# AdaptiveCity/deepdish

Measured on AMD Instinct MI355X. Metric: end-to-end frames/sec (detect+encode+track) at 640x480, higher is better.
Workload: dtype i8 (reference: uint8); encoder f16; 1 GPU; SSD-MobileNet-v1 uint8-quantised (300x300) + MARS-64x32x3 + deep_sort on synthetic 640x480 BGR frames, ~20 synthetic detections/frame (BASELINE.json configs[1]); streams_per_gpu=3072, worker_threads_per_gpu=2, parallelism=independent streams, 3072 per GPU in 2 worker groups, weights=seeded synthetic (seed 1234)

## Files before the change

### deepdish_amd/_lib.py

```python
import ctypes
import os
from ctypes import c_int, c_int64, c_double, c_float, c_void_p, c_char_p, POINTER

HERE = os.path.dirname(os.path.abspath(__file__))
LIB_PATH = os.environ.get('DD_LIB') or os.path.join(HERE, 'libdeepdish_hip.so')

P = c_void_p


class DeepDishHipError(RuntimeError):
    pass


SIGNATURES = {
    'dd_last_error': [],
    'dd_version': [],
    'dd_ctx_create': [c_int, POINTER(P)],
    'dd_ctx_destroy': [P],
    'dd_ctx_stream': [P, POINTER(P)],
    'dd_ctx_sync': [P],
    'dd_kf_initiate': [P, P, P, P, P, c_int, P],
    'dd_kf_predict': [P, P, P, P, c_int, P],
    'dd_kf_project': [P, P, P, P, c_int, P, P, P],
    'dd_kf_update': [P, P, P, P, P, c_int, P],
    'dd_kf_gate': [P, P, P, P, c_int, P, c_int, c_int, P, P],
    'dd_iou_cost': [P, P, P, c_int, P, c_int, P, P],
    'dd_cosine_nn_cost': [P, P, P, c_int, P, c_int, P, P],
    'dd_euclidean_nn_cost': [P, P, P, c_int, P, c_int, P, P],
    'dd_nms': [P, P, P, c_int, c_double, P, P, P],
    'dd_nms_ssd': [P, P, P, c_int, c_double, P, P, P],
    'dd_lsap_host': [P, c_int, c_int, P, P],
    'dd_pyset_difference_order_host': [P, c_int, P, c_int, P, POINTER(c_int)],
    'dd_tracker_create': [P, c_double, c_double, c_int, c_int, c_int, c_int, c_int, POINTER(P)],
    'dd_tracker_create_metric': [P, c_int, c_double, c_double, c_int, c_int, c_int, c_int, c_int, POINTER(P)],
    'dd_tracker_destroy': [P],
    'dd_tracker_predict': [P],
    'dd_tracker_update': [P, P, P, c_int, c_int],
    'dd_tracker_count': [P, c_int, POINTER(c_int)],
    'dd_tracker_read': [P, c_int, P, P, P],
    'dd_tracker_track_update': [P, c_int64, P, P, c_int],
    'dd_tracker_track_predict': [P, c_int64],
    'dd_tracker_track_set': [P, c_int64, c_int, c_int],
    'dd_tracker_remove': [P, P, c_int],
    'dd_tracker_next_id': [P, POINTER(c_int64)],
    'dd_tracker_last_cost': [P, P, P, c_int, POINTER(c_int), POINTER(c_int)],
    'dd_tracker_last_matches': [P, P, c_int, POINTER(c_int)],
    'dd_crop_resize': [P, P, c_int, c_int, P, c_int, c_int, c_int, P, P, P],
    'dd_crop_resize_f64': [P, P, c_int, c_int, P, c_int, c_int, c_int, P, P, P],
    'dd_fake_encode': [P, P, c_int, c_int, P, P],
    'dd_resize_lanczos': [P, P, c_int, c_int, c_int, c_int, P, c_int, c_int, P],
    'dd_resize_lanczos_batch': [P, P, c_int, c_int, c_int, c_int, c_int, P, c_int, c_int, P],
    'dd_resize_bilinear': [P, P, c_int, c_int, c_int, P, c_int, c_int, P],
    'dd_ingest_create': [P, c_int, c_int, c_int, c_int, c_int, c_int, c_int, P],
    'dd_ingest_destroy': [P],
    'dd_ingest_host_slot': [P, c_int, P, P],
    'dd_ingest_submit': [P, c_int],
    'dd_ingest_wait_uploaded': [P, c_int],
    'dd_ingest_acquire': [P, c_int, P, P],
    'dd_ingest_release': [P, c_int, P],
    'dd_mog2_create': [P, c_int, c_int, c_int, c_int, c_double, c_int, POINTER(P)],
    'dd_mog2_destroy': [P],
    'dd_mog2_state': [P, c_int, P, P, P, P],
    'dd_mog2_apply': [P, P, c_double, P, P, P],
    'dd_mask_box_count': [P, P, c_int, c_int, c_int, P, P, c_int, P, P],
    'dd_net_create': [P, P, c_int, P, c_int64, c_int, POINTER(P)],
    'dd_net_create_shared': [P, P, c_int, P, c_int64, c_int, POINTER(P)],
    'dd_net_activation_bytes': [P, POINTER(c_int64)],
    'dd_net_destroy': [P],
    'dd_net_forward': [P, P, c_int, P],
    'dd_net_output': [P, c_int, POINTER(P), POINTER(c_int), POINTER(c_int), POINTER(c_int), POINTER(c_int),
                      POINTER(c_int)],
    'dd_net_use_graph': [P, c_int],
    'dd_net_input_size': [P, POINTER(c_int), POINTER(c_int)],
    'dd_net_max_batch': [P, POINTER(c_int)],
    'dd_net_last_batch': [P, POINTER(c_int)],
    'dd_net_read': [P, c_int, c_int, P, c_int, P],
    'dd_net_profile': [P, c_int],
    'dd_net_profile_read': [P, P, c_int, POINTER(c_int)],
    'dd_net_op_launches': [P, P, c_int, POINTER(c_int)],
    'dd_ssd_postprocess': [P, P, P, c_int, c_int, c_int, c_float, c_float, P, P, P, P, P],
    'dd_ssd_decode': [P, P, P, c_int, c_int, c_float, P, P, P, P, c_int, P],
    'dd_ssd_postprocess_decoded': [P, P, P, P, P, c_int, c_int, c_float, c_float, P, P, P, P, c_int, P],
    'dd_ssd_regular_nms_decoded': [P, P, P, c_int, c_int, c_int, c_int, c_int, c_int, c_float, c_float, P, P, P, P, c_int, P],
    'dd_ssd_postprocess_regular': [P, P, P, c_int, c_int, c_int, c_int, c_float, c_float, P, P, P, P, c_int, P],
    'dd_ssd_postprocess_regular_u8': [P, P, P, c_int, P, P, P, c_int, c_int, c_int, c_int, c_float, c_float, P, P, P, P, c_int, P],
    'dd_net_ssd_heads_u8': [P, POINTER(P), POINTER(P), POINTER(c_int), POINTER(P), P, POINTER(c_int), POINTER(c_int)],
    'dd_net_ssd_decode': [P, P, c_int, c_float, c_int],
    'dd_net_ssd_decoded': [P, POINTER(P), POINTER(P), POINTER(P), POINTER(P)],
    'dd_net_ssd_decoded_read': [P, c_int, P, P, P, P],
    'dd_net_yolo_decode': [P, c_int],
    'dd_net_yolo_decoded': [P, P, P, P, P],
    'dd_net_yolo_decoded_read': [P, c_int, P, P, P],
    'dd_ssd_detections': [P, P, P, P, c_int, c_int, c_double, c_double, c_double, c_double, P, P, P, P, P],
    'dd_yolov5_decode': [P, P, c_int, c_int, c_float, c_float, c_float, P, P, P, c_int, P, P],
    'dd_pipeline_create': [P, c_int, c_int, c_int, P, P, c_int, c_int, P, c_char_p, c_char_p, c_double, c_double,
                           c_double, c_int, c_int, P, c_int, c_int, POINTER(P)],
    'dd_pipeline_destroy': [P],
    'dd_pipeline_detector_adaptor': [P, c_int],
    'dd_pipeline_ssd_options': [P, c_int, c_float, c_float],
    'dd_pipeline_ssd_regular_nms': [P, c_int],
    'dd_pipeline_detector_skip_frames': [P, c_int],
    'dd_pipeline_metric': [P, c_int],
    'dd_pipeline_step': [P, P, P, P, P, P],
    'dd_pipeline_step2': [P, P, P, P, P, P, P],
    'dd_pipeline_background_subtraction': [P, c_double, c_int],
    'dd_pipeline_motion_mask': [P, P, c_int, POINTER(ctypes.c_longlong)],
    'dd_pipeline_counts': [P, P],
    'dd_pipeline_tracker': [P, c_int, POINTER(P)],
    'dd_pipeline_stage_seconds': [P, P, POINTER(ctypes.c_longlong)],
    'dd_pipeline_stage_gpu_ms': [P, P, POINTER(ctypes.c_longlong)],
    'dd_pipeline_detector_stream': [P, POINTER(P)],
    'dd_pipeline_detections': [P, c_int, P, P, P, c_int, POINTER(c_int)],
    'dd_counts_accumulate': [P, P, P, c_int, P],
}
_RESTYPE = {'dd_last_error': c_char_p}

_lib = None
MISSING = []


def lib():
    global _lib
    if _lib is not None:
        return _lib
    if not os.path.exists(LIB_PATH):
        raise DeepDishHipError(
            'libdeepdish_hip.so is missing (%s): build it with `python -m deepdish_amd.build`; '
            'there is no CPU fallback' % LIB_PATH)
    try:
        import torch
    except ImportError:
        pass
    l = ctypes.CDLL(LIB_PATH)
    for name, args in SIGNATURES.items():
        try:
            fn = getattr(l, name)
        except AttributeError:
            MISSING.append(name)
            continue
        fn.argtypes = args
        fn.restype = _RESTYPE.get(name, c_int)
    _lib = l
    return l


def check(rc, what=''):
    if rc != 0:
        msg = lib().dd_last_error()
        raise DeepDishHipError('%s failed (%d): %s' % (what or 'libdeepdish_hip call', rc,
                                                      msg.decode() if msg else '?'))
```

### deepdish_amd/csrc/mars_pair.hip

```cpp
#include "mars_tail.h"

namespace {

typedef _Float16 h8 __attribute__((ext_vector_type(8)));
typedef float f4 __attribute__((ext_vector_type(4)));
typedef unsigned u4 __attribute__((ext_vector_type(4)));

__device__ __forceinline__ float elu(float v) {
    float e = __builtin_amdgcn_exp2f(v * 1.44269504088896340736f);
    e = __builtin_amdgcn_fmed3f(e, 0.f, 1.f);
    return __builtin_amdgcn_fmed3f(v, e - 1.f, 3.0e38f);
}

__device__ __forceinline__ void lds_fill16(const _Float16 *g, char *lds_wave_base) {
#if defined(__HIP_DEVICE_COMPILE__)
    __builtin_amdgcn_global_load_lds(g, lds_wave_base, 16, 0, 0);
#endif
}

__device__ __forceinline__ int frag_row(int a, int fr) { return (fr >> 2) * 8 + (a & 1) * 4 + (fr & 3); }

constexpr int PZ_B = 3072;
constexpr int PT64_B = 18 * 1024;
constexpr int PT32_B = 33 * 1024;
constexpr int PPLAIN_B = 16 * 1024;
constexpr int PRAW_B = 8 * 1024;
constexpr int pair_off_in(bool) { return PZ_B; }
constexpr int pair_off_h(bool first) { return PZ_B + 2 * (first ? PT32_B : PT64_B); }
constexpr int pair_off_res(bool first) { return pair_off_h(first) + 2 * PT64_B; }
constexpr int pair_off_raw(bool first) { return pair_off_res(first) + (first ? 2 : 3) * PPLAIN_B; }
constexpr int pair_off_const(bool first) { return pair_off_raw(first) + (first ? 2 * PRAW_B : 0); }
constexpr int pair_lds_bytes(bool first) { return pair_off_const(first) + 5 * 64 * 4; }

template <bool FIRST>
__global__ __launch_bounds__(512, 2) void mars_pair64_k(const MarsPairP P) {
    constexpr int OFF_IN = pair_off_in(FIRST), OFF_H = pair_off_h(FIRST), OFF_RES = pair_off_res(FIRST), OFF_RAW = pair_off_raw(FIRST),
                  OFF_C = pair_off_const(FIRST);
    constexpr int TIN_B = FIRST ? PT32_B : PT64_B, NRES = FIRST ? 2 : 3;
    extern __shared__ __attribute__((aligned(16))) char smem[];
    const int tid = threadIdx.x, lane = tid & 63;
    const int wave = __builtin_amdgcn_readfirstlane(tid >> 6);
    const int stage = wave >> 2, half = wave & 1, q = (wave >> 1) & 1;
    const int fr = lane & 15, fq = lane >> 4, j = fr >> 3, x = fr & 7;

    for (int i = tid * 16; i < OFF_C; i += 512 * 16) *reinterpret_cast<u4 *>(smem + i) = u4{0u, 0u, 0u, 0u};
    float *cst = reinterpret_cast<float *>(smem + OFF_C);
    if (tid < 64) {
        cst[tid] = P.bias_a[tid];
        cst[64 + tid] = P.bias_b[tid];
        cst[128 + tid] = P.aff2[tid];
        cst[192 + tid] = P.aff2[P.cout_pad + tid];
        cst[256 + tid] = (FIRST && P.bias_p) ? P.bias_p[tid] : 0.f;
    }
    __syncthreads();

    h8 wf[9][2][2];
    h8 wp[2];
    const bool a32 = FIRST && stage == 0;
    {
        const _Float16 *w = stage == 0 ? P.wa : P.wb;
        const int kpad = stage == 0 ? P.kpad_a : P.kpad_b;
#pragma unroll
        for (int t = 0; t < 9; ++t)
#pragma unroll
            for (int ks = 0; ks < 2; ++ks)
#pragma unroll
                for (int a = 0; a < 2; ++a) {
                    const size_t row = (size_t)(half * 32 + frag_row(a, fr)) * kpad;
                    wf[t][ks][a] = a32 ? *reinterpret_cast<const h8 *>(w + row + t * 32 + fq * 8)
                                       : *reinterpret_cast<const h8 *>(w + row + t * 64 + ks * 32 + fq * 8);
                }
#pragma unroll
        for (int a = 0; a < 2; ++a)
            wp[a] = FIRST ? *reinterpret_cast<const h8 *>(P.wp + (size_t)(half * 32 + frag_row(a, fr)) * P.kpad_p + fq * 8) : wf[0][0][a];
    }
#if defined(__HIP_DEVICE_COMPILE__)
#pragma unroll
    for (int t = 0; t < 9; ++t)
#pragma unroll
        for (int ks = 0; ks < 2; ++ks)
#pragma unroll
            for (int a = 0; a < 2; ++a) asm volatile("" ::"v"(wf[t][ks][a]));
    asm volatile("" ::"v"(wp[0]), "v"(wp[1]));
#endif

    const int n0 = blockIdx.x, nstep = gridDim.x;
    const int Kc = (P.n_img - n0 + nstep - 1) / nstep;

    const _Float16 *src[5];
    size_t stp[5];
    int n_dma;
    if constexpr (FIRST) {
        const int par = lane >> 5, pl = (lane >> 3) & 3, col = 2 * (lane & 7) + par;
#pragma unroll
        for (int h = 0; h < 4; ++h) {
            const int r = wave + 8 * h < 31 ? wave + 8 * h : 30;
            src[h] = col < 15 ? P.in + ((size_t)n0 * 31 + r) * 15 * P.cs_in + (size_t)col * P.cs_in + P.coff_in + pl * 8 : P.zero;
            stp[h] = col < 15 ? (size_t)nstep * 31 * 15 * P.cs_in : 0;
        }
        const int jr = lane >> 5, xx = lane & 7;
        src[4] = P.in2 + ((size_t)n0 * 31 + 2 * (2 * wave + jr)) * 15 * P.cs_in2 + (size_t)(2 * xx) * P.cs_in2 + P.coff_in2 + pl * 8;
        stp[4] = (size_t)nstep * 31 * 15 * P.cs_in2;
        n_dma = 5;
    } else {
        const int pl = lane >> 3, xx = lane & 7;
#pragma unroll
        for (int h = 0; h < 2; ++h) {
            src[h] = P.in + (((size_t)n0 * 16 + wave + 8 * h) * 8 + xx) * P.cs_in + P.coff_in + pl * 8;
            stp[h] = (size_t)nstep * 128 * P.cs_in;
            src[2 + h] = P.res + (((size_t)n0 * 16 + wave + 8 * h) * 8 + xx) * P.cs_res + P.coff_res + pl * 8;
            stp[2 + h] = (size_t)nstep * 128 * P.cs_res;
        }
        src[4] = P.zero; stp[4] = 0;
        n_dma = 4;
    }
    (void)n_dma;
    int dq = 0;
    auto issue = [&]() {
        char *T = smem + OFF_IN + (dq & 1) * TIN_B;
        if constexpr (FIRST) {
#pragma unroll
            for (int h = 0; h < 4; ++h) lds_fill16(src[h], T + ((wave + 8 * h < 31 ? wave + 8 * h : 30) + 1) * 1024);
            lds_fill16(src[4], smem + OFF_RAW + (dq & 1) * PRAW_B + wave * 1024);
        } else {
#pragma unroll
            for (int h = 0; h < 2; ++h) lds_fill16(src[h], T + (wave + 8 * h + 1) * 1024);
            const int rs = dq % 3;
#pragma unroll
            for (int h = 0; h < 2; ++h) lds_fill16(src[2 + h], smem + OFF_RES + rs * PPLAIN_B + (wave + 8 * h) * 1024);
        }
        ++dq;
        const bool more = dq < Kc;
#pragma unroll
        for (int h = 0; h < 5; ++h) src[h] += more ? stp[h] : 0;
    };

    const int co = half * 32 + fq * 8;
    const unsigned lo64 = (unsigned)((j * 64 + fq * 8 + x) * 16);
    const unsigned lo32 = (unsigned)((2 * j * 64 + fq * 8 + x) * 16);
    const f4 ba0 = *reinterpret_cast<const f4 *>(cst + (stage ? 64 : 0) + co), ba1 = *reinterpret_cast<const f4 *>(cst + (stage ? 64 : 0) + co + 4);

    issue();
    for (int c = 0; c <= Kc; ++c) {
#if defined(__HIP_DEVICE_COMPILE__)
        if (stage == 0 || c < 2) asm volatile("s_waitcnt vmcnt(0) lgkmcnt(0)" ::: "memory");
        else asm volatile("s_waitcnt vmcnt(8) lgkmcnt(0)" ::: "memory");
        __builtin_amdgcn_s_barrier();
        asm volatile("" ::: "memory");
#endif
        issue();
        const int cc = stage == 0 ? c : c - 1;
        if (cc < 0 || cc >= Kc) continue;
        const size_t n = (size_t)(n0 + cc * nstep);
#pragma unroll 1
        for (int f = 0; f < 4; ++f) {
            const int F = 4 * q + f;
            f4 acc[2] = {f4{0.f, 0.f, 0.f, 0.f}, f4{0.f, 0.f, 0.f, 0.f}};
            h8 X[4];
            if (a32) {
                const unsigned tb = (unsigned)(OFF_IN + (cc & 1) * PT32_B + 4 * F * 1024) + lo32;
                const unsigned bL = x == 0 ? ((tb + 512u - 16u) & 255u) : tb + 512u - 16u, bC = tb, bR = tb + 512u;
                const unsigned pb = (unsigned)(OFF_RAW + (cc & 1) * PRAW_B) + (unsigned)(((2 * F + j) * 32 + fq * 8 + x) * 16);
                f4 accp[2] = {f4{0.f, 0.f, 0.f, 0.f}, f4{0.f, 0.f, 0.f, 0.f}};
#if defined(__HIP_DEVICE_COMPILE__)
#define DD_RD(u_) do { if constexpr ((u_) < 9) { constexpr int dy_ = (u_) / 3, dx_ = (u_) - dy_ * 3;                                               \
                           asm volatile("ds_read_b128 %0, %1 offset:%2" : "=&v"(X[(u_) & 3]) : "v"(dx_ == 0 ? bL : dx_ == 1 ? bC : bR), "n"(dy_ * 1024) : "memory"); } \
                       else asm volatile("ds_read_b128 %0, %1" : "=&v"(X[(u_) & 3]) : "v"(pb) : "memory"); } while (0)
#define DD_UNIT(u_) do { if constexpr ((u_) + 3 < 10) DD_RD(((u_) + 3) % 10);                                                                      \
                         asm volatile("s_waitcnt lgkmcnt(%1)" : "+v"(X[(u_) & 3]) : "n"((u_) + 3 < 10 ? 3 : 9 - (u_)));                           \
                         if constexpr ((u_) < 9) { _Pragma("unroll") for (int a = 0; a < 2; ++a) acc[a] = __builtin_amdgcn_mfma_f32_16x16x32_f16(wf[(u_) % 9][0][a], X[(u_) & 3], acc[a], 0, 0, 0); } \
                         else { _Pragma("unroll") for (int a = 0; a < 2; ++a) accp[a] = __builtin_amdgcn_mfma_f32_16x16x32_f16(wp[a], X[(u_) & 3], accp[a], 0, 0, 0); } } while (0)
                DD_RD(0); DD_RD(1); DD_RD(2);
                DD_UNIT(0); DD_UNIT(1); DD_UNIT(2); DD_UNIT(3); DD_UNIT(4); DD_UNIT(5); DD_UNIT(6); DD_UNIT(7); DD_UNIT(8); DD_UNIT(9);
#undef DD_UNIT
#undef DD_RD
#endif
                const f4 c0 = *reinterpret_cast<const f4 *>(cst + 256 + co), c1 = *reinterpret_cast<const f4 *>(cst + 256 + co + 4);
                h8 sk;
#pragma unroll
                for (int i = 0; i < 4; ++i) { sk[i] = (_Float16)(accp[0][i] + c0[i]); sk[4 + i] = (_Float16)(accp[1][i] + c1[i]); }
                *reinterpret_cast<h8 *>(smem + OFF_RES + (cc & 1) * PPLAIN_B + ((2 * F + j) * 64 + (half * 4 + fq) * 8 + x) * 16) = sk;
            } else {
                const unsigned tb = (unsigned)((stage == 0 ? OFF_IN + (cc & 1) * PT64_B : OFF_H + (cc & 1) * PT64_B) + 2 * F * 1024) + lo64;
                const unsigned bL = x == 0 ? ((tb - 16u) & 255u) : tb - 16u, bC = tb, bR = x == 7 ? ((tb + 16u) & 255u) : tb + 16u;
#if defined(__HIP_DEVICE_COMPILE__)
#define DD_RD(u_) do { constexpr int t_ = (u_) >> 1, ks_ = (u_) & 1, dy_ = t_ / 3, dx_ = t_ - dy_ * 3;                                             \
                       asm volatile("ds_read_b128 %0, %1 offset:%2" : "=&v"(X[(u_) & 3]) : "v"(dx_ == 0 ? bL : dx_ == 1 ? bC : bR), "n"(dy_ * 1024 + ks_ * 512) : "memory"); } while (0)
#define DD_UNIT(u_) do { if constexpr ((u_) + 3 < 18) DD_RD(((u_) + 3) % 18);                                                                      \
                         asm volatile("s_waitcnt lgkmcnt(%1)" : "+v"(X[(u_) & 3]) : "n"((u_) + 3 < 18 ? 3 : 17 - (u_)));                          \
                         _Pragma("unroll") for (int a = 0; a < 2; ++a) acc[a] = __builtin_amdgcn_mfma_f32_16x16x32_f16(wf[(u_) >> 1][(u_) & 1][a], X[(u_) & 3], acc[a], 0, 0, 0); } while (0)
                DD_RD(0); DD_RD(1); DD_RD(2);
                DD_UNIT(0); DD_UNIT(1); DD_UNIT(2); DD_UNIT(3); DD_UNIT(4); DD_UNIT(5); DD_UNIT(6); DD_UNIT(7); DD_UNIT(8);
                DD_UNIT(9); DD_UNIT(10); DD_UNIT(11); DD_UNIT(12); DD_UNIT(13); DD_UNIT(14); DD_UNIT(15); DD_UNIT(16); DD_UNIT(17);
#undef DD_UNIT
#undef DD_RD
#endif
            }
            float v[8];
#pragma unroll
            for (int i = 0; i < 4; ++i) { v[i] = acc[0][i] + ba0[i]; v[4 + i] = acc[1][i] + ba1[i]; }
            if (stage == 0) {
                h8 o;
#pragma unroll
                for (int i = 0; i < 8; ++i) o[i] = (_Float16)elu(v[i]);
                *reinterpret_cast<h8 *>(smem + OFF_H + (cc & 1) * PT64_B + ((2 * F + j + 1) * 64 + (half * 4 + fq) * 8 + x) * 16) = o;
            } else {
                const int rs = FIRST ? (cc & 1) : cc % 3;
                const h8 rv = *reinterpret_cast<const h8 *>(smem + OFF_RES + rs * PPLAIN_B + ((2 * F + j) * 64 + (half * 4 + fq) * 8 + x) * 16);
#pragma unroll
                for (int i = 0; i < 8; ++i) v[i] += (float)rv[i];
                const size_t m = (n * 16 + 2 * F + j) * 8 + x;
                h8 o;
#pragma unroll
                for (int i = 0; i < 8; ++i) o[i] = (_Float16)v[i];
                *reinterpret_cast<h8 *>(P.out + m * P.cs_out + P.coff_out + co) = o;
                const f4 s0 = *reinterpret_cast<const f4 *>(cst + 128 + co), s1 = *reinterpret_cast<const f4 *>(cst + 128 + co + 4);
                const f4 t0 = *reinterpret_cast<const f4 *>(cst + 192 + co), t1 = *reinterpret_cast<const f4 *>(cst + 192 + co + 4);
                h8 o2;
#pragma unroll
                for (int i = 0; i < 4; ++i) { o2[i] = (_Float16)elu(s0[i] * v[i] + t0[i]); o2[4 + i] = (_Float16)elu(s1[i] * v[4 + i] + t1[i]); }
                *reinterpret_cast<h8 *>(P.out2 + m * P.cs_out2 + P.coff_out2 + co) = o2;
            }
        }
    }
#if defined(__HIP_DEVICE_COMPILE__)
    asm volatile("s_waitcnt vmcnt(0)" ::: "memory");
#endif
}

template <bool FIRST>
int launch_pair(hipStream_t s, int device, const MarsPairP &P) {
    constexpr int lds = pair_lds_bytes(FIRST);
    static_assert(lds <= 160 * 1024, "LDS budget");
    static DevOnce once;
    const int rc = once.run(device, [&]() -> int {
        DD_HIP(hipFuncSetAttribute(reinterpret_cast<const void *>(&mars_pair64_k<FIRST>), hipFuncAttributeMaxDynamicSharedMemorySize, lds));
        return DD_OK;
    });
    if (rc != DD_OK) return rc;
    const int n_cu = dd_cu_count(device);
    const int grid = P.n_img < n_cu ? P.n_img : n_cu;
    hipLaunchKernelGGL((mars_pair64_k<FIRST>), dim3(grid), dim3(512), lds, s, P);
    DD_LAUNCH_CHECK();
    return DD_OK;
}

}

int mars_pair64_launch(hipStream_t s, int device, const MarsPairP &P, bool first) {
    DD_REQUIRE(P.n_img > 0 && P.in && P.wa && P.wb && P.bias_a && P.bias_b && P.out && P.out2 && P.aff2 && P.zero && (first ? (P.in2 && P.wp) : P.res != nullptr), DD_E_ARG,
               "mars_pair64: bad argument");
    return first ? launch_pair<true>(s, device, P) : launch_pair<false>(s, device, P);
}
```

### deepdish_amd/csrc/mars_tail.h

```cpp
#pragma once
#include "common.h"

struct MarsWsP {
    const _Float16 *in;  int cs_in, coff_in;
    const _Float16 *in2; int cs_in2, coff_in2;
    const _Float16 *w;   int kpad;
    const _Float16 *w2;  int kpad2;
    const float *bias, *bias2;
    const _Float16 *res; int cs_res, coff_res;
    _Float16 *out;  int cs_out, coff_out;
    _Float16 *out2; int cs_out2, coff_out2;
    const float *aff2; int cout_pad;
    const _Float16 *zero;
    int n_img;
};

enum { MARS_WS_S1 = 0, MARS_WS_S1_RES = 1, MARS_WS_S2_PROJ = 2 };

int mars_ws128_launch(hipStream_t s, int device, const MarsWsP &P, int mode, int act, bool out2);

struct MarsPairP {
    const _Float16 *in;  int cs_in, coff_in;
    const _Float16 *in2; int cs_in2, coff_in2;
    const _Float16 *wa;  int kpad_a; const float *bias_a;
    const _Float16 *wp;  int kpad_p; const float *bias_p;
    const _Float16 *wb;  int kpad_b; const float *bias_b;
    const _Float16 *res; int cs_res, coff_res;
    _Float16 *out;  int cs_out, coff_out;
    _Float16 *out2; int cs_out2, coff_out2;
    const float *aff2; int cout_pad;
    const _Float16 *zero;
    int n_img;
};
int mars_pair64_launch(hipStream_t s, int device, const MarsPairP &P, bool first);
```

### deepdish_amd/csrc/mars_tail.hip

```cpp
#include "mars_tail.h"
#include <vector>

namespace {

typedef _Float16 h8 __attribute__((ext_vector_type(8)));
typedef float f4 __attribute__((ext_vector_type(4)));
typedef unsigned u4 __attribute__((ext_vector_type(4)));

enum { ACT_NONE = 0, ACT_ELU = 2 };

__device__ __forceinline__ float elu(float v) {
    float e = __builtin_amdgcn_exp2f(v * 1.44269504088896340736f);
    e = __builtin_amdgcn_fmed3f(e, 0.f, 1.f);
    return __builtin_amdgcn_fmed3f(v, e - 1.f, 3.0e38f);
}

__device__ __forceinline__ void lds_fill16(const _Float16 *g, char *lds_wave_base) {
#if defined(__HIP_DEVICE_COMPILE__)
    __builtin_amdgcn_global_load_lds(g, lds_wave_base, 16, 0, 0);
#endif
}

__device__ __forceinline__ int frag_row(int a, int fr) { return (fr >> 2) * 8 + (a & 1) * 4 + (fr & 3); }

// ... 1 lines not shown
__device__ unsigned long long dd_mars_stamps[256 * 8 * 8];
#define DD_STAMP(k) do { const unsigned long long t_ = __builtin_amdgcn_s_memtime(); st_acc[k] += t_ - st_last; st_last = t_; } while (0)
#else
#define DD_STAMP(k) do { } while (0)
#endif

constexpr int WS_LEAD = 2, WS_NB = WS_LEAD + 2, WS_NBR = WS_LEAD + 3;
constexpr int ws_tile_bytes(int mode) { return mode == MARS_WS_S2_PROJ ? 17 * 68 * 16 : 10 * 72 * 16; }
constexpr int ws_zero_bytes(int mode) { return mode == MARS_WS_S2_PROJ ? 0 : 7680; }
constexpr int WS_RES_BYTES = 8 * 72 * 16, WS_PRJ_BYTES = 4096;
constexpr int ws_xw_bytes(int mode) { return mode == MARS_WS_S2_PROJ ? 4096 : 2048; }
constexpr int ws_off_tiles(int mode) { return ws_zero_bytes(mode); }
constexpr int ws_off_aux(int mode) { return ws_off_tiles(mode) + WS_NB * ws_tile_bytes(mode); }
constexpr int ws_off_xchg(int mode) {
    return ws_off_aux(mode) + (mode == MARS_WS_S1_RES ? WS_NBR * WS_RES_BYTES : mode == MARS_WS_S2_PROJ ? WS_NB * WS_PRJ_BYTES : 0);
}
constexpr int ws_off_const(int mode) { return ws_off_xchg(mode) + 2 * 8 * ws_xw_bytes(mode); }
constexpr int ws_lds_bytes(int mode) { return ws_off_const(mode) + 3 * 128 * 4; }

template <int MODE, int ACT, bool OUT2>
__global__ __launch_bounds__(512, 2) void mars_ws128_k(const MarsWsP P) {
    constexpr bool S2 = MODE == MARS_WS_S2_PROJ, RES = MODE == MARS_WS_S1_RES;
    constexpr int LEAD = WS_LEAD, NB = WS_NB, NBR = WS_NBR;
    constexpr int TILE_B = ws_tile_bytes(MODE), XW_B = ws_xw_bytes(MODE);
    constexpr int OFF_T = ws_off_tiles(MODE), OFF_A = ws_off_aux(MODE), OFF_X = ws_off_xchg(MODE), OFF_C = ws_off_const(MODE);
    constexpr int KS = S2 ? 1 : 2, CIN = S2 ? 64 : 128;
    [[maybe_unused]] constexpr int N_DMA = S2 ? 3 : RES ? 2 : 1;
    [[maybe_unused]] constexpr int N_ST = S2 ? 2 : (RES && OUT2) ? 2 : 1;
    extern __shared__ __attribute__((aligned(16))) char smem[];
    const int tid = threadIdx.x, lane = tid & 63;
    const int wave = __builtin_amdgcn_readfirstlane(tid >> 6);
    const int cg = wave & 3, kh = wave >> 2;
    const int fr = lane & 15, fq = lane >> 4, yy = fr >> 2, x = fr & 3;

    for (int i = tid * 16; i < OFF_A; i += 512 * 16) *reinterpret_cast<u4 *>(smem + i) = u4{0u, 0u, 0u, 0u};
    float *cst = reinterpret_cast<float *>(smem + OFF_C);
    if (tid < 128) {
        cst[tid] = P.bias[tid];
        if constexpr (S2) cst[128 + tid] = P.bias2 ? P.bias2[tid] : 0.f;
        if constexpr (RES && OUT2) { cst[128 + tid] = P.aff2[tid]; cst[256 + tid] = P.aff2[P.cout_pad + tid]; }
    }
    __syncthreads();

    h8 wf[9][KS][2];
#pragma unroll
    for (int t = 0; t < 9; ++t)
#pragma unroll
        for (int ks = 0; ks < KS; ++ks)
#pragma unroll
            for (int a = 0; a < 2; ++a)
                wf[t][ks][a] = *reinterpret_cast<const h8 *>(P.w + (size_t)(cg * 32 + frag_row(a, fr)) * P.kpad + t * CIN + kh * (CIN / 2) + ks * 32 + fq * 8);
    h8 wp[2];
    if constexpr (S2) {
#pragma unroll
        for (int a = 0; a < 2; ++a) wp[a] = *reinterpret_cast<const h8 *>(P.w2 + (size_t)(cg * 32 + frag_row(a, fr)) * P.kpad2 + kh * 32 + fq * 8);
    }

#if defined(__HIP_DEVICE_COMPILE__)
#pragma unroll
    for (int t = 0; t < 9; ++t)
#pragma unroll
        for (int ks = 0; ks < KS; ++ks)
#pragma unroll
            for (int a = 0; a < 2; ++a) asm volatile("" ::"v"(wf[t][ks][a]));
    if constexpr (S2) asm volatile("" ::"v"(wp[0]), "v"(wp[1]));
#endif

    const int n0 = blockIdx.x, nstep = gridDim.x;
    const int Kc = (P.n_img - n0 + nstep - 1) / nstep;

    int dq = 0, dq_slot = 0, dq_rslot = 0;
    const _Float16 *src_a, *src_b, *src_c;
    size_t step_a, step_b, step_c;
    if constexpr (!S2) {
        src_a = P.in + (size_t)n0 * 32 * P.cs_in + ((wave * 4 + (lane & 3)) * P.cs_in + P.coff_in + (lane >> 2) * 8);
        src_b = RES ? P.res + (size_t)n0 * 32 * P.cs_res + ((wave * 4 + (lane & 3)) * P.cs_res + P.coff_res + (lane >> 2) * 8) : P.zero;
        src_c = P.zero;
        step_a = (size_t)nstep * 32 * P.cs_in; step_b = (size_t)nstep * 32 * P.cs_res; step_c = 0;
    } else {
        const int par = lane >> 5, pl = (lane >> 2) & 7, col = 2 * (lane & 3) + par;
        src_a = P.in + (size_t)n0 * 128 * P.cs_in + ((wave * 8 + col) * P.cs_in + P.coff_in + pl * 8);
        src_b = src_a + (size_t)64 * P.cs_in;
        const int ch = (wave & 3) * 64 + lane;
        src_c = P.in2 + (size_t)n0 * 128 * P.cs_in2 + ((2 * ((ch >> 2) & 7) * 8 + 2 * (ch & 3)) * P.cs_in2 + P.coff_in2 + (ch >> 5) * 8);
        step_a = step_b = (size_t)nstep * 128 * P.cs_in; step_c = (size_t)nstep * 128 * P.cs_in2;
    }
    auto issue = [&]() {
        char *T = smem + OFF_T + dq_slot * TILE_B;
        if constexpr (!S2) {
            lds_fill16(src_a, T + (wave + 1) * 72 * 16);
            if constexpr (RES) lds_fill16(src_b, smem + OFF_A + dq_rslot * WS_RES_BYTES + wave * 72 * 16);
        } else {
            lds_fill16(src_a, T + wave * 68 * 16);
            lds_fill16(src_b, T + (wave + 8) * 68 * 16);
            lds_fill16(src_c, smem + OFF_A + dq_slot * WS_PRJ_BYTES + (wave & 3) * 1024);
        }
        ++dq;
        const bool more = dq < Kc;
        src_a += more ? step_a : 0;
        if constexpr (RES || S2) src_b += more ? step_b : 0;
        if constexpr (S2) src_c += more ? step_c : 0;
        dq_slot = dq_slot + 1 == NB ? 0 : dq_slot + 1;
        dq_rslot = dq_rslot + 1 == NBR ? 0 : dq_rslot + 1;
    };

    const unsigned lo = S2 ? (unsigned)((2 * yy * 68 + (kh * 4 + fq) * 4 + x) * 16) : (unsigned)((yy * 72 + (kh * 8 + fq) * 4 + x) * 16);
    const unsigned lo_prj = (unsigned)(((kh * 4 + fq) * 32 + yy * 4 + x) * 16);
    const unsigned lo_res = (unsigned)(((4 * kh + yy) * 72 + (cg * 4 + fq) * 4 + x) * 16);
    const int co = cg * 32 + fq * 8;
    const f4 b0 = *reinterpret_cast<const f4 *>(cst + co), b1 = *reinterpret_cast<const f4 *>(cst + co + 4);

    f4 keep[S2 ? 4 : 2];
    int slot = 0, rslot_prev = 0, rslot = 0;

    auto epilogue = [&](int cprev) {
        const char *Xp = smem + OFF_X + ((cprev & 1) * 8 + (wave ^ 4)) * XW_B + lane * 16;
        const size_t n = (size_t)(n0 + cprev * nstep);
        const size_t m = (n * 8 + 4 * kh + yy) * 4 + x;
        float v[8];
        {
            const f4 o0 = *reinterpret_cast<const f4 *>(Xp), o1 = *reinterpret_cast<const f4 *>(Xp + 1024);
#pragma unroll
            for (int i = 0; i < 4; ++i) { v[i] = keep[0][i] + o0[i] + b0[i]; v[4 + i] = keep[1][i] + o1[i] + b1[i]; }
        }
        if constexpr (ACT == ACT_ELU) {
#pragma unroll
            for (int i = 0; i < 8; ++i) v[i] = elu(v[i]);
        }
        if constexpr (RES) {
            const h8 rv = *reinterpret_cast<const h8 *>(smem + OFF_A + rslot_prev * WS_RES_BYTES + lo_res);
#pragma unroll
            for (int i = 0; i < 8; ++i) v[i] += (float)rv[i];
        }
        h8 o;
#pragma unroll
        for (int i = 0; i < 8; ++i) o[i] = (_Float16)v[i];
        *reinterpret_cast<h8 *>(P.out + m * P.cs_out + P.coff_out + co) = o;
        if constexpr (RES && OUT2) {
            const f4 s0 = *reinterpret_cast<const f4 *>(cst + 128 + co), s1 = *reinterpret_cast<const f4 *>(cst + 128 + co + 4);
            const f4 t0 = *reinterpret_cast<const f4 *>(cst + 256 + co), t1 = *reinterpret_cast<const f4 *>(cst + 256 + co + 4);
            h8 o2;
#pragma unroll
            for (int i = 0; i < 4; ++i) { o2[i] = (_Float16)elu(s0[i] * v[i] + t0[i]); o2[4 + i] = (_Float16)elu(s1[i] * v[4 + i] + t1[i]); }
            *reinterpret_cast<h8 *>(P.out2 + m * P.cs_out2 + P.coff_out2 + co) = o2;
        }
        if constexpr (S2) {
            const f4 o0 = *reinterpret_cast<const f4 *>(Xp + 2048), o1 = *reinterpret_cast<const f4 *>(Xp + 3072);
            const f4 c0 = *reinterpret_cast<const f4 *>(cst + 128 + co), c1 = *reinterpret_cast<const f4 *>(cst + 128 + co + 4);
            h8 o2;
#pragma unroll
            for (int i = 0; i < 4; ++i) { o2[i] = (_Float16)(keep[2][i] + o0[i] + c0[i]); o2[4 + i] = (_Float16)(keep[3][i] + o1[i] + c1[i]); }
            *reinterpret_cast<h8 *>(P.out2 + m * P.cs_out2 + P.coff_out2 + co) = o2;
        }
    };

#ifdef DD_MARS_STAMPS
    unsigned long long st_acc[8] = {0, 0, 0, 0, 0, 0, 0, 0}, st_last = __builtin_amdgcn_s_memtime();
    const unsigned long long st_begin = st_last;
#endif
    static_assert(LEAD == 2, "the counted waits below are written for two crops of look-ahead");
    for (int ci = 0; ci < LEAD; ++ci) issue();
    DD_STAMP(0);
    for (int c = 0; c <= Kc; ++c) {
#if defined(__HIP_DEVICE_COMPILE__)
        if (kh == 0 || c == 0) {
            if (c <= 1) asm volatile("s_waitcnt vmcnt(%0) lgkmcnt(0)" ::"i"(N_DMA) : "memory");
            else if (c == 2) asm volatile("s_waitcnt vmcnt(%0) lgkmcnt(0)" ::"i"(N_DMA + N_ST) : "memory");
            else asm volatile("s_waitcnt vmcnt(%0) lgkmcnt(0)" ::"i"(N_DMA + 2 * N_ST) : "memory");
// ... 66 lines not shown
#endif
            DD_STAMP(3);
            issue();
            DD_STAMP(1);
            if (c > 0) epilogue(c - 1);
            DD_STAMP(4);
#pragma unroll
            for (int i = 0; i < (S2 ? 4 : 2); ++i) keep[i] = kn[i];
        } else {
            issue();
            DD_STAMP(1);
            if (c > 0) epilogue(c - 1);
            DD_STAMP(4);
#if defined(__HIP_DEVICE_COMPILE__)
            if (c == 0) asm volatile("s_waitcnt vmcnt(%0) lgkmcnt(0)" ::"i"(N_DMA) : "memory");
            else if (c == 1) asm volatile("s_waitcnt vmcnt(%0) lgkmcnt(0)" ::"i"(N_DMA + N_ST) : "memory");
            else asm volatile("s_waitcnt vmcnt(%0) lgkmcnt(0)" ::"i"(N_DMA + 2 * N_ST) : "memory");
            __builtin_amdgcn_s_barrier();
            asm volatile("" ::: "memory");
#endif
            DD_STAMP(3);
            if (c < Kc) compute(keep);
            DD_STAMP(5);
        }
        slot = slot + 1 == NB ? 0 : slot + 1;
        rslot_prev = rslot;
        rslot = rslot + 1 == NBR ? 0 : rslot + 1;
    }
#if defined(__HIP_DEVICE_COMPILE__)
    asm volatile("s_waitcnt vmcnt(0)" ::: "memory");
#endif
#ifdef DD_MARS_STAMPS
    if (lane == 0) {
        unsigned long long *d = dd_mars_stamps + ((size_t)blockIdx.x * 8 + wave) * 8;
        for (int k = 0; k < 6; ++k) d[k] = st_acc[k];
        d[6] = __builtin_amdgcn_s_memtime() - st_begin;
        d[7] = (unsigned long long)Kc;
    }
#endif
}

template <int MODE, int ACT, bool OUT2>
int launch_one(hipStream_t s, int device, const MarsWsP &P) {
    constexpr int lds = ws_lds_bytes(MODE);
    static_assert(lds <= 160 * 1024, "LDS budget");
    static DevOnce once;
    const int rc = once.run(device, [&]() -> int {
        DD_HIP(hipFuncSetAttribute(reinterpret_cast<const void *>(&mars_ws128_k<MODE, ACT, OUT2>), hipFuncAttributeMaxDynamicSharedMemorySize, lds));
        return DD_OK;
    });
    if (rc != DD_OK) return rc;
    const int n_cu = dd_cu_count(device);
    const int grid = P.n_img < n_cu ? P.n_img : n_cu;
    hipLaunchKernelGGL((mars_ws128_k<MODE, ACT, OUT2>), dim3(grid), dim3(512), lds, s, P);
    DD_LAUNCH_CHECK();
#ifdef DD_MARS_STAMPS
    {
        static std::vector<unsigned long long> h(256 * 8 * 8);
        DD_HIP(hipStreamSynchronize(s));
        DD_HIP(hipMemcpyFromSymbol(h.data(), HIP_SYMBOL(dd_mars_stamps), h.size() * 8));
        for (int half = 0; half < 2; ++half) {
            double a[7] = {0, 0, 0, 0, 0, 0, 0};
            int nw = 0;
            for (int b = 0; b < grid; ++b)
                for (int w = half * 4; w < half * 4 + 4; ++w, ++nw) {
                    const unsigned long long *d = h.data() + ((size_t)b * 8 + w) * 8;
                    for (int k = 0; k < 7; ++k) a[k] += (double)d[k] / (double)(k == 0 || k == 6 ? 1 : d[7] + 1);
                }
            fprintf(stderr, "mars_ws128_k<%d,%d,%d> K half %d: prologue DMAs %.0f | per step: issue %.0f, wait %.0f, barrier %.0f, epilogue %.0f, compute %.0f | loop total %.0f cycles, %d steps\n",
                    MODE, ACT, (int)OUT2, half, a[0] / nw, a[1] / nw, a[2] / nw, a[3] / nw, a[4] / nw, a[5] / nw, a[6] / nw, (int)h[7] + 1);
        }
    }
#endif
    return DD_OK;
}

}

int mars_ws128_launch(hipStream_t s, int device, const MarsWsP &P, int mode, int act, bool out2) {
    DD_REQUIRE(P.n_img > 0 && P.in && P.w && P.bias && P.out && P.zero, DD_E_ARG, "mars_ws128: bad argument");
    DD_REQUIRE((long long)P.n_img * 128 * (P.cs_in > P.cs_out ? P.cs_in : P.cs_out) < (1ll << 40), DD_E_CAPACITY, "mars_ws128: batch of %d", P.n_img);
    if (mode == MARS_WS_S2_PROJ) {
        DD_REQUIRE(P.in2 && P.w2 && P.out2 && act == ACT_ELU, DD_E_ARG, "mars_ws128: stride-2 form needs the projection operands and ELU");
        return launch_one<MARS_WS_S2_PROJ, ACT_ELU, false>(s, device, P);
    }
    if (mode == MARS_WS_S1) {
        DD_REQUIRE(!P.res && !P.out2, DD_E_ARG, "mars_ws128: plain form with a residual or a second output");
        return act == ACT_ELU ? launch_one<MARS_WS_S1, ACT_ELU, false>(s, device, P) : launch_one<MARS_WS_S1, ACT_NONE, false>(s, device, P);
    }
    DD_REQUIRE(mode == MARS_WS_S1_RES && P.res && act == ACT_NONE && (!out2 || (P.out2 && P.aff2)), DD_E_ARG, "mars_ws128: residual form");
    return out2 ? launch_one<MARS_WS_S1_RES, ACT_NONE, true>(s, device, P) : launch_one<MARS_WS_S1_RES, ACT_NONE, false>(s, device, P);
}
```

### deepdish_amd/csrc/net_priv.h

```cpp
#pragma once
#include <map>
#include <utility>
#include <vector>
#include "common.h"

struct TensorDesc { int buf, h, w, c, cs, coff, dtype, pad; };

struct dd_net {
    dd_ctx *ctx = nullptr;
    int max_batch = 0;
    std::vector<int32_t> prog;
    std::vector<TensorDesc> tensors;
    std::vector<int64_t> buf_elems;
    std::vector<void *> bufs;
    std::vector<int> buf_dtype;
    int n_ops = 0, ops_off = 0;
    void *arena = nullptr;
    int64_t arena_bytes = 0;
    char *d_weights = nullptr;
    int64_t weight_bytes = 0;
    int in_h = 0, in_w = 0, out_tensor = -1;
    bool profile = false;
    int last_batch = 0;
    DevBuf slab;
    bool ssd_dec = false, yolo_dec = false;
    int dec_anchors = 0; float dec_thr = 0.f;
    float *d_anchors = nullptr, *dec_boxes = nullptr, *dec_score = nullptr, *dec_keys = nullptr; int *dec_cls = nullptr;
    bool slab_moved = false;
    _Float16 *d_zero = nullptr;
    bool use_glds = true;
    bool use_rw = true;
    int tile_mode = 0;
    std::vector<hipEvent_t> events;
    std::vector<int32_t> op_launch;
    struct GraphEntry { int calls = 0; hipGraph_t graph = nullptr; hipGraphExec_t exec = nullptr; };
    bool use_graph = false;
    std::map<std::pair<const void *, int>, GraphEntry> graphs;
};

int netq_run_op(dd_net *net, int op_index, const int32_t *o, const uint8_t *input, int nimg, hipStream_t s, int *handled);
int netq_run_front(dd_net *net, const int32_t *o0, const int32_t *o1, const int32_t *o2, const uint8_t *input, int nimg, hipStream_t s, int *ran);
int netq_run_mid(dd_net *net, const int32_t *o3, const int32_t *o4, int nimg, hipStream_t s, int *ran);
int netq_prepare(dd_net *net);
```

### deepdish_amd/csrc/nets.hip

```cpp
#include <algorithm>
#include <cmath>
#include <cstdlib>
#include <map>
#include <string>
#include "common.h"
#include "ssd_dev.h"
#include "net_priv.h"
#include "mars_tail.h"

namespace {

typedef _Float16 h8 __attribute__((ext_vector_type(8)));
typedef _Float16 h4 __attribute__((ext_vector_type(4)));
typedef float f4 __attribute__((ext_vector_type(4)));

enum { OP_INPUT = 1, OP_CONV = 2, OP_DWCONV = 3, OP_MAXPOOL = 4, OP_UPSAMPLE = 5, OP_FC = 6, OP_L2NORM = 7, OP_STEM = 8, OP_DWPW = 9 };
enum { ACT_NONE = 0, ACT_RELU6 = 1, ACT_ELU = 2, ACT_SILU = 3, ACT_RELU = 4, ACT_SIGMOID = 5 };
enum { EPI_F16 = 0, EPI_F32 = 1, EPI_SSD_HEAD = 2, EPI_YOLO = 3 };
enum { OPK_DEFAULT = 0, OPK_FOLDED = 1, OPK_POOL_ROWS = 2, OPK_POOL_ROWS_STEM = 3, OPK_RES_UNIT = 4, OPK_SSD_FRONT = 5, OPK_C64_ROWS = 6, OPK_S2_ROWS = 7, OPK_CONV_WS = 8, OPK_WS_DW = 9, OPK_DWPW_ROWS = 10, OPK_SSD_HEAD_DEC = 11, OPK_RES_PAIR = 12, OPK_YOLO_HEAD_DEC = 13, OPK_MARS_WS = 14, OPK_FOLDED_PREV = 15, OPK_MARS_PAIR = 16, OPK_C64_STRIPS = 18, OPK_Q_FRONT = 19, OPK_Q_MID = 20, OPK_STEM_WIDE = 23 };
enum { DT_F16 = 0, DT_F32 = 1, DT_U8 = 2 };

constexpr int OP_WORDS = 48;
constexpr int TENSOR_WORDS = 8;

// ... 83 lines not shown
        const int n = m / hw, p = m - n * hw;
        const int A = P.p[5];
        float *dst = static_cast<float *>(P.out) + ((size_t)n * P.p[1] + P.p[2] + (size_t)p * A) * P.p[3];
#pragma unroll
        for (int r = 0; r < 4; ++r)
            if (co + r < P.cout) dst[co + r] = v[r];
        return;
    }
    if (P.res) {
        const h4 rv = *reinterpret_cast<const h4 *>(P.res + (size_t)m * P.cs_res + P.coff_res + co);
#pragma unroll
        for (int r = 0; r < 4; ++r) v[r] += (float)rv[r];
    }
    if (P.epi == EPI_F32) {
        if (P.post_aff) {
            const f4 sc = *reinterpret_cast<const f4 *>(P.aff2 + co);
            const f4 sh = *reinterpret_cast<const f4 *>(P.aff2 + P.cout_pad + co);
#pragma unroll
            for (int r = 0; r < 4; ++r) v[r] = sc[r] * v[r] + sh[r];
        }
#pragma unroll
        for (int r = 0; r < 4; ++r)
            if (co + r >= P.cout) v[r] = 0.f;
        *reinterpret_cast<f4 *>(static_cast<float *>(P.out) + (size_t)m * P.cs_out + P.coff_out + co) = f4{v[0], v[1], v[2], v[3]};
        return;
    }
#pragma unroll
    for (int r = 0; r < 4; ++r)
        if (co + r >= P.cout) v[r] = 0.f;
    {
        h4 o;
#pragma unroll
        for (int r = 0; r < 4; ++r) o[r] = (_Float16)v[r];
        *reinterpret_cast<h4 *>(static_cast<_Float16 *>(P.out) + (size_t)m * P.cs_out + P.coff_out + co) = o;
    }
    if (P.out2) {
        const f4 sc = *reinterpret_cast<const f4 *>(P.aff2 + co);
        const f4 sh = *reinterpret_cast<const f4 *>(P.aff2 + P.cout_pad + co);
        h4 o;
#pragma unroll
        for (int r = 0; r < 4; ++r) {
            const float t = co + r < P.cout ? apply_act(sc[r] * v[r] + sh[r], ACT_ELU) : 0.f;
            o[r] = (_Float16)t;
        }
        *reinterpret_cast<h4 *>(P.out2 + (size_t)m * P.cs_out2 + P.coff_out2 + co) = o;
    }
}

typedef unsigned u4v_t __attribute__((ext_vector_type(4)));
template <int HI>
__device__ __forceinline__ float fma_mix_f16(unsigned x, unsigned w, float acc) {
#if defined(__HIP_DEVICE_COMPILE__)
    if (HI) asm("v_fma_mix_f32 %0, %1, %2, %0 op_sel:[1,1,0] op_sel_hi:[1,1,0]" : "+v"(acc) : "v"(x), "v"(w));
    else asm("v_fma_mix_f32 %0, %1, %2, %0 op_sel:[0,0,0] op_sel_hi:[1,1,0]" : "+v"(acc) : "v"(x), "v"(w));
#endif
    return acc;
}
__device__ __forceinline__ void dw_tap(float (&acc)[8], const h8 &x, const h8 &w) {
    const u4v_t xv = __builtin_bit_cast(u4v_t, x), wv = __builtin_bit_cast(u4v_t, w);
#pragma unroll
    for (int i = 0; i < 8; ++i)
        acc[i] = (i & 1) ? fma_mix_f16<1>(xv[i >> 1], wv[i >> 1], acc[i]) : fma_mix_f16<0>(xv[i >> 1], wv[i >> 1], acc[i]);
}

struct Epi8 { f4 b0, b1, s0, s1, t0, t1; };

__device__ __forceinline__ Epi8 epi8_load(const ConvP &P, int co) {
    Epi8 E;
    E.b0 = *reinterpret_cast<const f4 *>(P.bias + co);
    E.b1 = *reinterpret_cast<const f4 *>(P.bias + co + 4);
    E.s0 = E.s1 = E.t0 = E.t1 = f4{0.f, 0.f, 0.f, 0.f};
    if (P.out2) {
        E.s0 = *reinterpret_cast<const f4 *>(P.aff2 + co);
        E.s1 = *reinterpret_cast<const f4 *>(P.aff2 + co + 4);
        E.t0 = *reinterpret_cast<const f4 *>(P.aff2 + P.cout_pad + co);
        E.t1 = *reinterpret_cast<const f4 *>(P.aff2 + P.cout_pad + co + 4);
    }
    return E;
}

#ifndef DD_EPI_NT
#define DD_EPI_NT true
#endif
template <int ACT = -1, bool BIAS = true, int EF = -1, bool NT = DD_EPI_NT, bool TAIL = true>
__device__ __forceinline__ void conv_epilogue_f16x8(const ConvP &P, const Epi8 &E, int m, int co, float v[8], const h8 *res_pre = nullptr) {
    const int act = ACT < 0 ? P.act : ACT;
    const bool has_res = EF < 0 ? P.res != nullptr : EF >= 1, has_out2 = EF < 0 ? P.out2 != nullptr : EF == 1;
#pragma unroll
    for (int r = 0; r < 4; ++r) {
        v[r] = apply_act(BIAS ? v[r] + E.b0[r] : v[r], act);
        v[4 + r] = apply_act(BIAS ? v[4 + r] + E.b1[r] : v[4 + r], act);
    }
    if (has_res) {
        const h8 rv = res_pre ? *res_pre : *reinterpret_cast<const h8 *>(P.res + (size_t)m * P.cs_res + P.coff_res + co);
#pragma unroll
        for (int r = 0; r < 8; ++r) v[r] += (float)rv[r];
    }
    const bool tail = TAIL && co + 8 > P.cout;
    h8 o;
#pragma unroll
    for (int r = 0; r < 8; ++r) o[r] = (_Float16)v[r];
    if (tail) {
#pragma unroll
        for (int r = 0; r < 8; ++r)
            if (co + r >= P.cout) o[r] = (_Float16)0.f;
    }
    h8 *dst = reinterpret_cast<h8 *>(static_cast<_Float16 *>(P.out) + (size_t)m * P.cs_out + P.coff_out + co);
    if constexpr (NT) __builtin_nontemporal_store(o, dst);
    else *dst = o;
    if (has_out2) {
        h8 o2;
#pragma unroll
        for (int r = 0; r < 8; ++r) {
            const float sc = r < 4 ? E.s0[r] : E.s1[r - 4], sh = r < 4 ? E.t0[r] : E.t1[r - 4];
            o2[r] = (_Float16)apply_act(sc * v[r] + sh, ACT_ELU);
        }
        if (tail) {
#pragma unroll
            for (int r = 0; r < 8; ++r)
                if (co + r >= P.cout) o2[r] = (_Float16)0.f;
        }
        *reinterpret_cast<h8 *>(P.out2 + (size_t)m * P.cs_out2 + P.coff_out2 + co) = o2;
    }
}

template <int ACT = -1>
__device__ __forceinline__ void conv_epilogue_f16x8(const ConvP &P, int m, int co, float v[8]) {
    const Epi8 E = epi8_load(P, co);
    conv_epilogue_f16x8<ACT>(P, E, m, co, v);
}

template <int ACT, int BM, int BN, int T>
__device__ __forceinline__ void conv_finish_rows(const ConvP &P, const float *ot, int m0, int n0) {
    constexpr int OROW = BN + 4, G = BN / 8;
    static_assert(T % G == 0, "a thread keeps its channel group over the row loop");
    const int g = threadIdx.x % G, co = n0 + g * 8;
    if (co >= P.cout_pad) return;
    const Epi8 E = epi8_load(P, co);
    for (int pl = threadIdx.x / G; pl < BM; pl += T / G) {
        const int m = m0 + pl;
        if (m >= P.m) break;
        const f4 lo = *reinterpret_cast<const f4 *>(ot + pl * OROW + g * 8);
        const f4 hi = *reinterpret_cast<const f4 *>(ot + pl * OROW + g * 8 + 4);
        float v[8] = {lo[0], lo[1], lo[2], lo[3], hi[0], hi[1], hi[2], hi[3]};
        conv_epilogue_f16x8<ACT>(P, E, m, co, v);
    }
}

template <int WM, int WN, int MI, int NI>
__device__ __forceinline__ void conv_finish(const ConvP &P, f4 (&acc)[NI][MI], _Float16 *lds, int m0, int n0, int hw) {
    constexpr int T = WM * WN * 64;
    constexpr int BM = WM * MI * 16, BN = WN * NI * 16;
    const int tid = threadIdx.x, lane = tid & 63, wave = tid >> 6;
    const int wm = wave / WN, wn = wave % WN;
    const int fr = lane & 15, fq = lane >> 4;
    if (P.epi == EPI_F16 && P.splitk == 1) {
        constexpr int OROW = BN + 4;
        float *ot = reinterpret_cast<float *>(lds);
#pragma unroll
        for (int b = 0; b < MI; ++b)
#pragma unroll
            for (int a = 0; a < NI; ++a)
                *reinterpret_cast<f4 *>(ot + ((wm * MI + b) * 16 + fr) * OROW + (wn * NI + a) * 16 + fq * 4) = acc[a][b];
        __syncthreads();
        switch (P.act) {
            case ACT_NONE: conv_finish_rows<ACT_NONE, BM, BN, T>(P, ot, m0, n0); break;
            case ACT_RELU6: conv_finish_rows<ACT_RELU6, BM, BN, T>(P, ot, m0, n0); break;
            case ACT_ELU: conv_finish_rows<ACT_ELU, BM, BN, T>(P, ot, m0, n0); break;
            case ACT_SILU: conv_finish_rows<ACT_SILU, BM, BN, T>(P, ot, m0, n0); break;
            default: conv_finish_rows<-1, BM, BN, T>(P, ot, m0, n0);
        }
        return;
    }
    if (P.epi == EPI_SSD_HEAD && P.splitk == 1) {
        constexpr int OROW = BN + 4;
        float *ot = reinterpret_cast<float *>(lds);
#pragma unroll
        for (int b = 0; b < MI; ++b)
#pragma unroll
            for (int a = 0; a < NI; ++a)
                *reinterpret_cast<f4 *>(ot + ((wm * MI + b) * 16 + fr) * OROW + (wn * NI + a) * 16 + fq * 4) = acc[a][b];
        __syncthreads();
        const int A = P.p[5];
        typedef float f4u __attribute__((ext_vector_type(4), aligned(4)));
        constexpr int LPP = BN / 4, PPW = 64 / LPP;
        const int lc = (lane % LPP) * 4, lp = lane / LPP;
        const int ch = n0 + lc;
        const int nlive = min(4, max(0, P.cout - ch));
        f4 bias = f4{0.f, 0.f, 0.f, 0.f};
        for (int q = 0; q < nlive; ++q) bias[q] = P.bias[ch + q];
        for (int pl = wave * PPW + lp; pl < BM; pl += WM * WN * PPW) {
            const int m = m0 + pl;
// ... 1183 lines not shown
            fill_pre(2 * r + 3); fill_pre(2 * r + 4);
            if constexpr (RAW_SEP) { fill_raw(2 * r + 1); fill_raw(2 * r + 2); }
            auto conv2 = [&](const _Float16 *ringp, int slot0, int mask, const h8 (&w)[9][2], f4 (&acc)[2][2]) {
                h8 X[2][3];
                auto rd = [&](int i, h8 (&x)[3]) {
                    const _Float16 *rs = ringp + ((slot0 + i) & mask) * RU_SLOT + offC;
                    x[0] = *reinterpret_cast<const h8 *>(rs - 8);
                    x[1] = *reinterpret_cast<const h8 *>(rs);
                    x[2] = *reinterpret_cast<const h8 *>(rs + 8);
                };
                rd(0, X[0]);
#pragma unroll
                for (int i = 0; i < 4; ++i) {
                    h8 (&x)[3] = X[i & 1];
#if defined(__HIP_DEVICE_COMPILE__)
                    asm volatile("" : "+v"(x[0]), "+v"(x[1]), "+v"(x[2]));
                    __builtin_amdgcn_sched_barrier(0);
#endif
                    if (i + 1 < 4) rd(i + 1, X[(i + 1) & 1]);
#if defined(__HIP_DEVICE_COMPILE__)
                    __builtin_amdgcn_sched_barrier(0);
#endif
#pragma unroll
                    for (int dx = 0; dx < 3; ++dx)
#pragma unroll
                        for (int cr = 0; cr < 2; ++cr) {
                            const int dy = i - cr;
                            if (dy < 0 || dy > 2) continue;
#pragma unroll
                            for (int a = 0; a < 2; ++a)
                                acc[cr][a] = __builtin_amdgcn_mfma_f32_16x16x32_f16(w[dy * 3 + dx][a], x[dx], acc[cr][a], 0, 0, 0);
                        }
#if defined(__HIP_DEVICE_COMPILE__)
                    __builtin_amdgcn_sched_barrier(0);
#endif
                }
            };
            {
                f4 acc[2][2] = {{bA0, bA1}, {bA0, bA1}};
                conv2(pre, 2 * r, RU_PRE_SLOTS - 1, wA, acc);
#pragma unroll
                for (int cr = 0; cr < 2; ++cr) {
                    const int y = 2 * r + cr;
                    const bool live = y < H && fr < W;
                    h8 o;
#pragma unroll
                    for (int q = 0; q < 4; ++q) {
                        o[q] = (_Float16)apply_act(acc[cr][0][q], actA);
                        o[4 + q] = (_Float16)apply_act(acc[cr][1][q], actA);
                    }
                    u4v_t ou = __builtin_bit_cast(u4v_t, o);
                    ou &= live ? 0xFFFFFFFFu : 0u;
                    *reinterpret_cast<u4v_t *>(h1 + (y & (RU_H1_SLOTS - 1)) * RU_SLOT + offC) = ou;
                }
            }
            {
                f4 acc[2][2] = {{EB.b0, EB.b1}, {EB.b0, EB.b1}};
                conv2(h1, 2 * r - 2, RU_H1_SLOTS - 1, wB, acc);
                h8 rv0 = RAW_SEP ? *reinterpret_cast<const h8 *>(rawr + ((2 * r - 1) & (RU_RAW_SLOTS - 1)) * RU_SLOT + offC)
                                 : *reinterpret_cast<const h8 *>(pre + ((2 * r) & (RU_PRE_SLOTS - 1)) * RU_SLOT + offC);
#if defined(__HIP_DEVICE_COMPILE__)
                asm volatile("s_waitcnt vmcnt(0)" ::: "memory");
#endif
#pragma unroll
                for (int cr = 0; cr < 2; ++cr) {
                    const int y = 2 * r - 1 + cr;
                    if (cr == 1) rv0 = RAW_SEP ? *reinterpret_cast<const h8 *>(rawr + (y & (RU_RAW_SLOTS - 1)) * RU_SLOT + offC)
                                               : *reinterpret_cast<const h8 *>(pre + ((y + 1) & (RU_PRE_SLOTS - 1)) * RU_SLOT + offC);
                    if ((unsigned)y >= (unsigned)H || fr >= W) continue;
                    float o[8];
#pragma unroll
                    for (int q = 0; q < 4; ++q) { o[q] = acc[cr][0][q]; o[4 + q] = acc[cr][1][q]; }
                    conv_epilogue_f16x8<ACT_NONE, false, 1, true, false>(PB, EB, (n * H + y) * W + fr, fq * 8, o, &rv0);
                }
            }
        }
    }
}

constexpr int RP_X_SLOTS = 8;
constexpr int rp_pair_halves() { return 6 * 8 + (RU_PRE_SLOTS + 2 * RU_H1_SLOTS + 2 * RP_X_SLOTS) * RU_SLOT; }

template <int ACT_A>
__global__ __launch_bounds__(512, 2) void res_pair_rows_k(const ConvP P1A, const ConvP P1B, const ConvP P2A, const ConvP P2B, const int n_img) {
    extern __shared__ __attribute__((aligned(16))) _Float16 lds[];
    const int tid = threadIdx.x, lane = tid & 63;
    const int wave = __builtin_amdgcn_readfirstlane(tid >> 6);
    const int pair = wave & 3, role = wave >> 2;
    const int fr = lane & 15, fq = lane >> 4;
    _Float16 *pbase = lds + (size_t)pair * rp_pair_halves();
    _Float16 *pre = pbase + 8;
    _Float16 *h1a = pre + RU_PRE_SLOTS * RU_SLOT + 8;
    _Float16 *xo = h1a + RU_H1_SLOTS * RU_SLOT + 8;
    _Float16 *xo2 = xo + RP_X_SLOTS * RU_SLOT + 8;
    _Float16 *h1b = xo2 + RP_X_SLOTS * RU_SLOT + 8;
    const h8 zero8 = {(_Float16)0.f, (_Float16)0.f, (_Float16)0.f, (_Float16)0.f, (_Float16)0.f, (_Float16)0.f, (_Float16)0.f, (_Float16)0.f};
    for (int i = (role * 64 + lane) * 8; i < rp_pair_halves(); i += 128 * 8) *reinterpret_cast<h8 *>(pbase + i) = zero8;

    const _Float16 *wa_p = role ? P2A.w : P1A.w, *wb_p = role ? P2B.w : P1B.w;
    const int kpa = role ? P2A.kpad : P1A.kpad, kpb = role ? P2B.kpad : P1B.kpad;
    h8 wA[9][2], wB[9][2];
#pragma unroll
    for (int t = 0; t < 9; ++t)
#pragma unroll
        for (int a = 0; a < 2; ++a) {
            wA[t][a] = *reinterpret_cast<const h8 *>(wa_p + (size_t)rw_weight_row(a, fr) * kpa + t * 32 + fq * 8);
            wB[t][a] = *reinterpret_cast<const h8 *>(wb_p + (size_t)rw_weight_row(a, fr) * kpb + t * 32 + fq * 8);
        }
    const float *ba_p = role ? P2A.bias : P1A.bias, *bb_p = role ? P2B.bias : P1B.bias, *af_p = role ? P2B.aff2 : P1B.aff2;
    const int cpad = role ? P2B.cout_pad : P1B.cout_pad;
    const f4 bA0 = *reinterpret_cast<const f4 *>(ba_p + fq * 8), bA1 = *reinterpret_cast<const f4 *>(ba_p + fq * 8 + 4);
    Epi8 EB;
    EB.b0 = *reinterpret_cast<const f4 *>(bb_p + fq * 8); EB.b1 = *reinterpret_cast<const f4 *>(bb_p + fq * 8 + 4);
    EB.s0 = *reinterpret_cast<const f4 *>(af_p + fq * 8); EB.s1 = *reinterpret_cast<const f4 *>(af_p + fq * 8 + 4);
    EB.t0 = *reinterpret_cast<const f4 *>(af_p + cpad + fq * 8); EB.t1 = *reinterpret_cast<const f4 *>(af_p + cpad + fq * 8 + 4);
    const int H = P1A.H, W = P1A.W;
    const int offC = (fq * 16 + fr) * 8;
    const int actA = ACT_A < 0 ? P1A.act : ACT_A;
    _Float16 *inr = role ? xo2 : pre, *h1r = role ? h1b : h1a, *resr = role ? xo : pre;

    const int n0 = blockIdx.x * 4 + pair, nstep = gridDim.x * 4;
    const int K = n0 < n_img ? (n_img - n0 + nstep - 1) / nstep : 0;
    const int base4 = blockIdx.x * 4;
    const int Kmax = base4 < n_img ? (n_img - base4 + nstep - 1) / nstep : 0;
    const int GA = 16 * K, Gall = 16 * Kmax + 2;
    auto fill_pre = [&](int s) {
        const int kk = (s + 1) >> 5, y = ((s + 1) & 31) - 1;
        const bool ok = kk < K && y >= 0 && fr < W;
        const _Float16 *src = P1A.in + ((size_t)(n0 + (ok ? kk : 0) * nstep) * H * W + (size_t)(ok ? y : 0) * W + fr) * P1A.cs_in + P1A.coff_in + fq * 8;
        lds_fill16(ok ? src : P1A.zero, pre + ((s + 1) & (RU_PRE_SLOTS - 1)) * RU_SLOT);
    };
#if defined(__HIP_DEVICE_COMPILE__)
    asm volatile("s_waitcnt lgkmcnt(0)" ::: "memory");
    __builtin_amdgcn_s_barrier();
    asm volatile("" ::: "memory");
#endif
    if (role == 0 && K > 0) { fill_pre(-1); fill_pre(0); fill_pre(1); fill_pre(2); fill_pre(3); fill_pre(4); }
#if defined(__HIP_DEVICE_COMPILE__)
    asm volatile("s_waitcnt vmcnt(0)" ::: "memory");
#endif
    auto conv2 = [&](const _Float16 *ringp, int slot0, int mask, const h8 (&w)[9][2], f4 (&acc)[2][2]) {
        h8 X[2][3];
        auto rd = [&](int i, h8 (&x)[3]) {
            const _Float16 *rs = ringp + ((slot0 + i) & mask) * RU_SLOT + offC;
            x[0] = *reinterpret_cast<const h8 *>(rs - 8);
            x[1] = *reinterpret_cast<const h8 *>(rs);
            x[2] = *reinterpret_cast<const h8 *>(rs + 8);
        };
        rd(0, X[0]);
#pragma unroll
        for (int i = 0; i < 4; ++i) {
            h8 (&x)[3] = X[i & 1];
#if defined(__HIP_DEVICE_COMPILE__)
            asm volatile("" : "+v"(x[0]), "+v"(x[1]), "+v"(x[2]));
            __builtin_amdgcn_sched_barrier(0);
#endif
            if (i + 1 < 4) rd(i + 1, X[(i + 1) & 1]);
#if defined(__HIP_DEVICE_COMPILE__)
            __builtin_amdgcn_sched_barrier(0);
#endif
#pragma unroll
            for (int dx = 0; dx < 3; ++dx)
#pragma unroll
                for (int cr = 0; cr < 2; ++cr) {
                    const int dy = i - cr;
                    if (dy < 0 || dy > 2) continue;
#pragma unroll
                    for (int a = 0; a < 2; ++a)
                        acc[cr][a] = __builtin_amdgcn_mfma_f32_16x16x32_f16(w[dy * 3 + dx][a], x[dx], acc[cr][a], 0, 0, 0);
                }
#if defined(__HIP_DEVICE_COMPILE__)
            __builtin_amdgcn_sched_barrier(0);
#endif
        }
    };
    f4 accC[2][2];
    int grC = -1;
    auto b_store = [&]() {
#pragma unroll
        for (int cr = 0; cr < 2; ++cr) {
            const int s = 2 * grC - 1 + cr;
            const int kk = (s + 1) >> 5, y = ((s + 1) & 31) - 1;
            if (y < 0 || fr >= W) continue;
            float o[8];
#pragma unroll
            for (int q = 0; q < 4; ++q) { o[q] = accC[cr][0][q]; o[4 + q] = accC[cr][1][q]; }
            const h8 rv = *reinterpret_cast<const h8 *>(resr + ((s + 1) & (RU_PRE_SLOTS - 1)) * RU_SLOT + offC);
            conv_epilogue_f16x8<ACT_NONE, false, 1, true, false>(P2B, EB, ((n0 + kk * nstep) * H + y) * W + fr, fq * 8, o, &rv);
        }
    };
    for (int g = 0; g < Gall; ++g) {
        const int gr = role ? g - 2 : g;
        const bool active = role ? (gr >= 0 && gr < GA) : (K > 0 && gr <= GA);
        if (grC >= 0) { b_store(); grC = -1; }
        if (active) {
            if (role == 0) { fill_pre(2 * gr + 5); fill_pre(2 * gr + 6); }
            {
                f4 acc[2][2] = {{bA0, bA1}, {bA0, bA1}};
                conv2(inr, 2 * gr, RU_PRE_SLOTS - 1, wA, acc);
#pragma unroll
                for (int cr = 0; cr < 2; ++cr) {
                    const int s = 2 * gr + cr;
                    const bool live = ((s + 1) & 31) != 0 && fr < W;
                    h8 o;
#pragma unroll
                    for (int q = 0; q < 4; ++q) {
                        o[q] = (_Float16)apply_act(acc[cr][0][q], actA);
                        o[4 + q] = (_Float16)apply_act(acc[cr][1][q], actA);
                    }
                    u4v_t ou = __builtin_bit_cast(u4v_t, o);
                    ou &= live ? 0xFFFFFFFFu : 0u;
                    *reinterpret_cast<u4v_t *>(h1r + (s & (RU_H1_SLOTS - 1)) * RU_SLOT + offC) = ou;
                }
            }
            {
                f4 acc[2][2] = {{EB.b0, EB.b1}, {EB.b0, EB.b1}};
                conv2(h1r, 2 * gr - 2, RU_H1_SLOTS - 1, wB, acc);
                h8 rv[2];
#pragma unroll
                for (int cr = 0; cr < 2; ++cr) rv[cr] = *reinterpret_cast<const h8 *>(resr + ((2 * gr + cr) & (RU_PRE_SLOTS - 1)) * RU_SLOT + offC);
                if (role == 0) {
#pragma unroll
                    for (int cr = 0; cr < 2; ++cr) {
                        const int s = 2 * gr - 1 + cr;
                        const bool live = ((s + 1) & 31) != 0 && fr < W;
                        float v[8];
#pragma unroll
                        for (int q = 0; q < 4; ++q) { v[q] = acc[cr][0][q]; v[4 + q] = acc[cr][1][q]; }
#pragma unroll
                        for (int q = 0; q < 8; ++q) v[q] += (float)rv[cr][q];
                        h8 o, o2;
#pragma unroll
                        for (int q = 0; q < 8; ++q) o[q] = (_Float16)v[q];
#pragma unroll
                        for (int q = 0; q < 8; ++q) {
                            const float sc = q < 4 ? EB.s0[q] : EB.s1[q - 4], sh = q < 4 ? EB.t0[q] : EB.t1[q - 4];
                            o2[q] = (_Float16)apply_act(sc * v[q] + sh, ACT_ELU);
                        }
                        u4v_t ou = __builtin_bit_cast(u4v_t, o), ou2 = __builtin_bit_cast(u4v_t, o2);
                        ou &= live ? 0xFFFFFFFFu : 0u;
                        ou2 &= live ? 0xFFFFFFFFu : 0u;
                        *reinterpret_cast<u4v_t *>(xo + ((s + 1) & (RP_X_SLOTS - 1)) * RU_SLOT + offC) = ou;
                        *reinterpret_cast<u4v_t *>(xo2 + ((s + 1) & (RP_X_SLOTS - 1)) * RU_SLOT + offC) = ou2;
                    }
#if defined(__HIP_DEVICE_COMPILE__)
                    asm volatile("s_waitcnt vmcnt(2)" ::: "memory");
#endif
                } else {
#pragma unroll
                    for (int cr = 0; cr < 2; ++cr) { accC[cr][0] = acc[cr][0]; accC[cr][1] = acc[cr][1]; }
                    grC = gr;
                }
            }
        }
#if defined(__HIP_DEVICE_COMPILE__)
        asm volatile("s_waitcnt lgkmcnt(0)" ::: "memory");
        __builtin_amdgcn_s_barrier();
        asm volatile("" ::: "memory");
#endif
    }
    if (grC >= 0) b_store();
#if defined(__HIP_DEVICE_COMPILE__)
    asm volatile("s_waitcnt vmcnt(0)" ::: "memory");
#endif
}

constexpr int C64_PITCH = 704, C64_SLOTS = 11, C64_RES_SLOTS = 4, C64_LEAD = 3;
constexpr int c64_wave_halves() { return C64_SLOTS * C64_PITCH + C64_RES_SLOTS * 512; }

template <int ACT, int EF, bool STRIP = false>
__global__ __launch_bounds__(256, 2) void conv3x3_c64_rows_k(const ConvP P, const int n_img) {
// ... 1725 lines not shown
            const int split = force_split > 0 ? force_split : nimg >= 1536 ? 1 : nimg >= 768 ? 2 : 4;
            const int n_units = nimg * split;
            const int grid = std::min(dd_ceil_div(n_units, 4), 2 * 256);
            if (stem) hipLaunchKernelGGL((conv3x3_pool_rows_k<ACT_ELU, true>), dim3((unsigned)grid), dim3(256), ring_bytes, s, P, n_units, split | (dbg << 8));
            else hipLaunchKernelGGL((conv3x3_pool_rows_k<ACT_ELU, false>), dim3((unsigned)grid), dim3(256), ring_bytes, s, P, n_units, split | (dbg << 8));
            DD_LAUNCH_CHECK();
            return DD_OK;
        }
    } else {
        spatial_tile(P.ho, P.wo, 1, RW_MAX_PATCH, P);
    }
    const int npix = (P.th + 2) * (P.tw + 2);
    DD_REQUIRE(npix <= RW_MAX_PATCH, DD_E_ARG, "conv3x3_rw: patch of %d pixels", npix);
    DD_REQUIRE(pool || !P.src8 || (P.tw == 32 && P.act == ACT_SILU && !P.res && !P.out2), DD_E_ARG, "conv3x3_rw: an input op was folded into a launch that cannot take it");
    const size_t lds_bytes = (size_t)4 * ((npix * 16 + 255) & ~255) + (pool ? (size_t)P.th * P.tw * 32 * sizeof(_Float16) : 0);
    const int total = nimg * P.tiles_x * P.tiles_y;
    const int grid = std::min(total, 2 * 256);
    if (pool) {
        static DevOnce once;
        const int rc = once.run(device, [&]() -> int {
            DD_HIP(hipFuncSetAttribute(reinterpret_cast<const void *>(&conv3x3_rw_k<2, 32, ACT_ELU, true>),
                                       hipFuncAttributeMaxDynamicSharedMemorySize, (int)lds_bytes));
            return DD_OK;
        });
        if (rc != DD_OK) return rc;
    }
    if (pool) {
        hipLaunchKernelGGL((conv3x3_rw_k<2, 32, ACT_ELU, true>), dim3((unsigned)grid), dim3(256), lds_bytes, s, P, total);
        DD_LAUNCH_CHECK();
        return DD_OK;
    }
#define DD_RW(TW_, ACT_, EF_) hipLaunchKernelGGL((conv3x3_rw_k<2, TW_, ACT_, false, EF_>), dim3((unsigned)grid), dim3(256), lds_bytes, s, P, total)
    const int ef = (!P.res && !P.out2) ? 0 : (P.res && P.out2) ? 1 : -1;
    if (P.tw == 32 && P.act == ACT_ELU && ef == 0) DD_RW(32, ACT_ELU, 0);
    else if (P.tw == 32 && P.act == ACT_SILU && P.src8 && ef == 0)
        hipLaunchKernelGGL((conv3x3_rw_k<2, 32, ACT_SILU, false, 0, true>), dim3((unsigned)grid), dim3(256), lds_bytes, s, P, total);
    else if (P.tw == 32 && P.act == ACT_SILU) DD_RW(32, ACT_SILU, -1);
    else if (P.tw == 15 && P.act == ACT_ELU && ef == 0) DD_RW(15, ACT_ELU, 0);
    else if (P.tw == 15 && P.act == ACT_NONE && ef == 1) DD_RW(15, ACT_NONE, 1);
    else DD_RW(0, -1, -1);
#undef DD_RW
    DD_LAUNCH_CHECK();
    return DD_OK;
}

bool res_unit_fusable(const ConvP &A, const ConvP &B, int nimg) {
    static const bool off = getenv("DD_RES_UNIT_UNFUSED") && atoi(getenv("DD_RES_UNIT_UNFUSED")) != 0;
    static const int min_img = getenv("DD_RES_UNIT_MIN") ? atoi(getenv("DD_RES_UNIT_MIN")) : 512;
    auto plain = [](const ConvP &P) {
        return P.kh == 3 && P.kw == 3 && P.stride == 1 && P.pad_t == 1 && P.pad_l == 1 && P.cin == 32 && P.cout == 32 && P.cout_pad == 32 &&
               P.epi == EPI_F16 && P.W == 15 && P.wo == 15 && P.H == P.ho && P.splitk <= 1;
    };
    return !off && nimg >= min_img && plain(A) && plain(B) && A.act == ACT_ELU && !A.res && !A.out2 && !A.coff_out &&
           B.act == ACT_NONE && B.res && B.out2 && B.in == static_cast<const _Float16 *>(A.out) && !B.coff_in && B.cs_in == A.cs_out && B.H == A.H;
}

int launch_res_unit(hipStream_t s, const ConvP &A, const ConvP &B, int nimg, int device) {
    const bool raw_sep = !(B.res == A.in && B.cs_res == A.cs_in && B.coff_res == A.coff_in);
    const size_t lds_bytes = (size_t)4 * ru_wave_halves(raw_sep) * sizeof(_Float16);
    static DevOnce once;
    const int rc = once.run(device, [&]() -> int {
        DD_HIP(hipFuncSetAttribute(reinterpret_cast<const void *>(&res_unit_rows_k<ACT_ELU, true>),
                                   hipFuncAttributeMaxDynamicSharedMemorySize, (int)(4 * ru_wave_halves(true) * sizeof(_Float16))));
        return DD_OK;
    });
    if (rc != DD_OK) return rc;
    const int grid = std::min(dd_ceil_div(nimg, 4), 2 * 256);
    if (raw_sep) hipLaunchKernelGGL((res_unit_rows_k<ACT_ELU, true>), dim3((unsigned)grid), dim3(256), lds_bytes, s, A, B, nimg);
    else hipLaunchKernelGGL((res_unit_rows_k<ACT_ELU, false>), dim3((unsigned)grid), dim3(256), lds_bytes, s, A, B, nimg);
    DD_LAUNCH_CHECK();
    return DD_OK;
}

bool res_pair_fusable(const ConvP &A1, const ConvP &B1, const ConvP &A2, const ConvP &B2, int nimg) {
    static const bool off = getenv("DD_RES_PAIR_OFF") && atoi(getenv("DD_RES_PAIR_OFF")) != 0;
    static const int min_img = getenv("DD_RES_PAIR_MIN") ? atoi(getenv("DD_RES_PAIR_MIN")) : 1024;
    return !off && nimg >= min_img && A1.H == 31 && A1.W == 15 &&
           B1.res == A1.in && B1.cs_res == A1.cs_in && B1.coff_res == A1.coff_in &&
           A2.in == static_cast<const _Float16 *>(B1.out2) && A2.cs_in == B1.cs_out2 && !A2.coff_in && !B1.coff_out2 &&
           B2.res == static_cast<const _Float16 *>(B1.out) && B2.cs_res == B1.cs_out && B2.coff_res == B1.coff_out &&
           A2.H == A1.H && A2.W == A1.W && A1.act == ACT_ELU && A2.act == ACT_ELU;
}

int launch_res_pair(hipStream_t s, const ConvP &A1, const ConvP &B1, const ConvP &A2, const ConvP &B2, int nimg, int device) {
    constexpr size_t lds_bytes = (size_t)4 * rp_pair_halves() * sizeof(_Float16);
    static DevOnce once;
    const int rc = once.run(device, [&]() -> int {
        DD_HIP(hipFuncSetAttribute(reinterpret_cast<const void *>(&res_pair_rows_k<ACT_ELU>), hipFuncAttributeMaxDynamicSharedMemorySize, (int)lds_bytes));
        return DD_OK;
    });
    if (rc != DD_OK) return rc;
    const int grid = std::min(dd_ceil_div(nimg, 4), 256);
    hipLaunchKernelGGL((res_pair_rows_k<ACT_ELU>), dim3((unsigned)grid), dim3(512), lds_bytes, s, A1, B1, A2, B2, nimg);
    DD_LAUNCH_CHECK();
    return DD_OK;
}

bool s2_rows_eligible(const ConvP &P, int nimg, int max_batch) {
    static const bool off = getenv("DD_S2_ROWS_OFF") && atoi(getenv("DD_S2_ROWS_OFF")) != 0;
    static const int min_img = getenv("DD_S2_ROWS_MIN") ? atoi(getenv("DD_S2_ROWS_MIN")) : 512;
    return !off && nimg >= min_img && P.kh == 3 && P.kw == 3 && P.stride == 2 && P.pad_t == 1 && P.pad_l == 1 && P.cin == 32 && P.cout == 64 &&
           P.cout_pad == 64 && P.kpad >= 288 && P.epi == EPI_F16 && P.W == 15 && P.H == 31 && P.ho == 16 && P.wo == 8 && P.splitk <= 1 &&
           P.act == ACT_ELU && !P.res && !P.out2 && (long long)dd_ceil_div(max_batch * P.ho * P.wo, 64) >= 256;
}

int launch_conv3x3_s2_rows(hipStream_t s, const ConvP &P, int nimg, int device) {
    constexpr size_t lds_bytes = (size_t)4 * S2_SLOTS * S2_PITCH * sizeof(_Float16);
    static DevOnce once;
    const int rc = once.run(device, [&]() -> int {
        DD_HIP(hipFuncSetAttribute(reinterpret_cast<const void *>(&conv3x3_s2_rows_k<ACT_ELU>), hipFuncAttributeMaxDynamicSharedMemorySize, (int)lds_bytes));
        return DD_OK;
    });
    if (rc != DD_OK) return rc;
    const int grid = std::min(dd_ceil_div(nimg, 4), 2 * 256);
    hipLaunchKernelGGL((conv3x3_s2_rows_k<ACT_ELU>), dim3((unsigned)grid), dim3(256), lds_bytes, s, P, nimg);
    DD_LAUNCH_CHECK();
    return DD_OK;
}

bool c64_strips_eligible(const ConvP &P, int nimg, int max_batch) {
    static const bool off = getenv("DD_C64_STRIPS_OFF") && atoi(getenv("DD_C64_STRIPS_OFF")) != 0;
    static const int min_items = getenv("DD_C64_STRIPS_MIN") ? atoi(getenv("DD_C64_STRIPS_MIN")) : 1024;
    return !off && P.kh == 3 && P.kw == 3 && P.stride == 1 && P.pad_t == 1 && P.pad_l == 1 && P.cin == 64 && P.cout == 64 &&
           P.cout_pad == 64 && P.kpad == 576 && P.epi == EPI_F16 && P.W > 8 && P.W % 8 == 0 && P.wo == P.W && P.H == P.ho && P.H % 2 == 0 &&
           P.splitk <= 1 && P.act == ACT_SILU && !P.out2 && (!P.res || (P.cs_res % 8 == 0 && P.coff_res % 8 == 0)) &&
           P.cs_in % 8 == 0 && P.coff_in % 8 == 0 && (long long)nimg * (P.W >> 3) >= min_items &&
           (long long)dd_ceil_div(max_batch * P.ho * P.wo, 64) >= 256;
}

int launch_conv3x3_c64_strips(hipStream_t s, const ConvP &P, int nimg, int device) {
    constexpr size_t lds_bytes = (size_t)4 * c64_wave_halves() * sizeof(_Float16);
    static DevOnce once;
    const int rc = once.run(device, [&]() -> int {
        DD_HIP(hipFuncSetAttribute(reinterpret_cast<const void *>(&conv3x3_c64_rows_k<ACT_SILU, 0, true>), hipFuncAttributeMaxDynamicSharedMemorySize, (int)lds_bytes));
        DD_HIP(hipFuncSetAttribute(reinterpret_cast<const void *>(&conv3x3_c64_rows_k<ACT_SILU, 2, true>), hipFuncAttributeMaxDynamicSharedMemorySize, (int)lds_bytes));
        return DD_OK;
    });
    if (rc != DD_OK) return rc;
    const long long items = (long long)nimg * (P.W >> 3);
    DD_REQUIRE(items * P.H * 8 < (1LL << 31), DD_E_CAPACITY, "conv3x3_c64 strips: %lld items exceed 32-bit pixel indexing", items);
    const int grid = (int)std::min<long long>((items + 1) / 2, 2 * 256);
    if (P.res) hipLaunchKernelGGL((conv3x3_c64_rows_k<ACT_SILU, 2, true>), dim3((unsigned)grid), dim3(256), lds_bytes, s, P, (int)items);
    else hipLaunchKernelGGL((conv3x3_c64_rows_k<ACT_SILU, 0, true>), dim3((unsigned)grid), dim3(256), lds_bytes, s, P, (int)items);
    DD_LAUNCH_CHECK();
    return DD_OK;
}

bool c64_rows_eligible(const ConvP &P, int nimg, int max_batch) {
    static const bool off = getenv("DD_C64_ROWS_OFF") && atoi(getenv("DD_C64_ROWS_OFF")) != 0;
    static const int min_img = getenv("DD_C64_ROWS_MIN") ? atoi(getenv("DD_C64_ROWS_MIN")) : 512;
    return !off && nimg >= min_img && P.kh == 3 && P.kw == 3 && P.stride == 1 && P.pad_t == 1 && P.pad_l == 1 && P.cin == 64 && P.cout == 64 &&
           P.cout_pad == 64 && P.kpad == 576 && P.epi == EPI_F16 && P.W == 8 && P.wo == 8 && P.H == P.ho && P.H % 2 == 0 && P.splitk <= 1 &&
           ((P.act == ACT_ELU && !P.res && !P.out2) || (P.act == ACT_NONE && P.res && P.out2 && P.cs_res % 8 == 0 && P.coff_res % 8 == 0)) &&
           (long long)dd_ceil_div(max_batch * P.ho * P.wo, 64) >= 256;
}

int launch_conv3x3_c64_rows(hipStream_t s, const ConvP &P, int nimg, int device) {
    constexpr size_t lds_bytes = (size_t)4 * c64_wave_halves() * sizeof(_Float16);
    static DevOnce once;
    const int rc = once.run(device, [&]() -> int {
        DD_HIP(hipFuncSetAttribute(reinterpret_cast<const void *>(&conv3x3_c64_rows_k<ACT_ELU, 0>), hipFuncAttributeMaxDynamicSharedMemorySize, (int)lds_bytes));
        DD_HIP(hipFuncSetAttribute(reinterpret_cast<const void *>(&conv3x3_c64_rows_k<ACT_NONE, 1>), hipFuncAttributeMaxDynamicSharedMemorySize, (int)lds_bytes));
        return DD_OK;
    });
    if (rc != DD_OK) return rc;
    const int grid = std::min(dd_ceil_div(nimg, 2), 2 * 256);
    if (P.res) hipLaunchKernelGGL((conv3x3_c64_rows_k<ACT_NONE, 1>), dim3((unsigned)grid), dim3(256), lds_bytes, s, P, nimg);
    else hipLaunchKernelGGL((conv3x3_c64_rows_k<ACT_ELU, 0>), dim3((unsigned)grid), dim3(256), lds_bytes, s, P, nimg);
    DD_LAUNCH_CHECK();
    return DD_OK;
}

bool ssd_front_fusable(const ConvP &S, const ConvP &P, int nimg) {
    static const bool off = getenv("DD_SSD_FRONT_UNFUSED") && atoi(getenv("DD_SSD_FRONT_UNFUSED")) != 0;
    static const int min_img = getenv("DD_SSD_FRONT_MIN") ? atoi(getenv("DD_SSD_FRONT_MIN")) : 16;
    return !off && nimg >= min_img && S.stride == 2 && S.cout == 32 && S.cout_pad == 32 && S.act == ACT_RELU6 && (S.W * 3) % 4 == 0 &&
// ... 221 lines not shown
        DD_HIP(hipFuncSetAttribute(reinterpret_cast<const void *>(&dwpw_big_k<STRIDE, -1, -1>),
                                   hipFuncAttributeMaxDynamicSharedMemorySize, 160 * 1024));
        return DD_OK;
    });
    if (rc != DD_OK) return rc;
    const dim3 grid((unsigned)(dd_ceil_div(P.total_quads, DWB_BM / 2) * (P.cout_pad / DWB_BN)));
    if (relu6) hipLaunchKernelGGL((dwpw_big_k<STRIDE, ACT_RELU6, ACT_RELU6>), grid, dim3(512), lds_bytes, s, P);
    else hipLaunchKernelGGL((dwpw_big_k<STRIDE, -1, -1>), grid, dim3(512), lds_bytes, s, P);
    DD_LAUNCH_CHECK();
    return DD_OK;
}


bool mars_ws_on() {
    static const bool on = !(getenv("DD_MARS_WS") && atoi(getenv("DD_MARS_WS")) == 0);
    return on;
}
bool mars_ws_s1_eligible(const ConvP &P) {
    return mars_ws_on() && P.kh == 3 && P.kw == 3 && P.stride == 1 && P.pad_t == 1 && P.pad_l == 1 && P.H == 8 && P.W == 4 && P.ho == 8 && P.wo == 4 &&
           P.cin == 128 && P.cout == 128 && P.cout_pad == 128 && P.kpad >= 1152 && P.epi == EPI_F16 && P.cs_in % 8 == 0 && P.coff_in % 8 == 0 &&
           P.cs_out % 8 == 0 && P.coff_out % 8 == 0 &&
           ((P.act == ACT_ELU && !P.res && !P.out2) || (P.act == ACT_NONE && P.res && P.cs_res % 8 == 0 && P.coff_res % 8 == 0 && (!P.out2 || (P.cs_out2 % 8 == 0 && P.coff_out2 % 8 == 0))));
}
bool mars_ws_s2_eligible(const ConvP &P) {
    return mars_ws_on() && P.kh == 3 && P.kw == 3 && P.stride == 2 && P.pad_t == 0 && P.pad_l == 0 && P.H == 16 && P.W == 8 && P.ho == 8 && P.wo == 4 &&
           P.cin == 64 && P.cout == 128 && P.cout_pad == 128 && P.kpad >= 576 && P.epi == EPI_F16 && P.act == ACT_ELU && !P.res && !P.out2 &&
           P.cs_in % 8 == 0 && P.coff_in % 8 == 0 && P.cs_out % 8 == 0 && P.coff_out % 8 == 0;
}
bool mars_proj_follows(const dd_net *net, int i, const ConvP &P) {
    const int32_t *q = net->prog.data() + net->ops_off + (size_t)(i + 1) * OP_WORDS;
    if (q[0] != OP_CONV || q[5] != 1 || q[6] != 1 || q[7] != 2 || q[8] != 0 || q[9] != 0 || q[10] != 64 || q[11] != 128 || q[12] != 128 ||
        q[14] != ACT_NONE || q[15] != EPI_F16 || q[3] >= 0 || q[4] >= 0 || q[13] < 64 || q[1] < 0 || q[2] < 0) return false;
    const TensorDesc &qs = net->tensors[q[1]], &qd = net->tensors[q[2]];
    return qs.h == 16 && qs.w == 8 && qd.h == 8 && qd.w == 4 && qs.cs % 8 == 0 && qs.coff % 8 == 0 && qd.cs % 8 == 0 && qd.coff % 8 == 0 && qd.dtype == DT_F16;
}
int mars_pair_match(const dd_net *net, int i, int nimg, MarsPairP &Q, bool &first) {
    void *const *bufs = net->bufs.data();
    static const bool off = getenv("DD_MARS_PAIR") && atoi(getenv("DD_MARS_PAIR")) == 0;
    static const int min_crops = getenv("DD_MARS_PAIR_MIN") ? atoi(getenv("DD_MARS_PAIR_MIN")) : 256;
    if (off || nimg < min_crops) return 0;
    auto op = [&](int k) { return net->prog.data() + net->ops_off + (size_t)k * OP_WORDS; };
    auto W = [&](const int32_t *o, int word) { return net->d_weights + (size_t)(uint32_t)o[word]; };
    auto conv3 = [&](const int32_t *o, int stride, int cin, int act) {
        return o[0] == OP_CONV && o[5] == 3 && o[6] == 3 && o[7] == stride && o[10] == cin && o[11] == 64 && o[12] == 64 && o[14] == act && o[15] == EPI_F16 &&
               o[8] == 1 && o[9] == 1 && o[13] >= 9 * cin && o[1] >= 0 && o[2] >= 0 && !o[29];
    };
    auto t16x8 = [&](int t, int c) { const TensorDesc &d = net->tensors[t]; return d.h == 16 && d.w == 8 && d.c == c && d.cs % 8 == 0 && d.coff % 8 == 0 && d.dtype == DT_F16; };
    auto t31x15 = [&](int t) { const TensorDesc &d = net->tensors[t]; return d.h == 31 && d.w == 15 && d.c == 32 && d.cs % 8 == 0 && d.coff % 8 == 0 && d.dtype == DT_F16; };
    memset(&Q, 0, sizeof(Q));
    const int32_t *a = op(i);
    int nb;
    if (i + 2 < net->n_ops && a[30] == 3 && conv3(a, 2, 32, ACT_ELU) && a[3] < 0 && a[4] < 0 && t31x15(a[1]) && t16x8(a[2], 64)) {
        const int32_t *p = op(i + 1);
        if (!(p[30] == 4 && p[0] == OP_CONV && p[5] == 1 && p[6] == 1 && p[7] == 2 && p[8] == 0 && p[9] == 0 && p[10] == 32 && p[11] == 64 && p[12] == 64 &&
              p[14] == ACT_NONE && p[15] == EPI_F16 && p[3] < 0 && p[4] < 0 && p[13] >= 32 && p[1] >= 0 && p[2] >= 0 && t31x15(p[1]) && t16x8(p[2], 64))) return 0;
        first = true; nb = i + 2;
        const TensorDesc &ti = net->tensors[a[1]], &tr = net->tensors[p[1]];
        Q.in = reinterpret_cast<const _Float16 *>(bufs[ti.buf]); Q.cs_in = ti.cs; Q.coff_in = ti.coff;
        Q.in2 = reinterpret_cast<const _Float16 *>(bufs[tr.buf]); Q.cs_in2 = tr.cs; Q.coff_in2 = tr.coff;
        Q.wp = reinterpret_cast<const _Float16 *>(W(p, 16)); Q.kpad_p = p[13]; Q.bias_p = reinterpret_cast<const float *>(W(p, 17));
        const int32_t *b = op(nb);
        if (b[3] != p[2]) return 0;
    } else if (i + 1 < net->n_ops && a[30] == 4 && conv3(a, 1, 64, ACT_ELU) && a[3] < 0 && a[4] < 0 && t16x8(a[1], 64) && t16x8(a[2], 64)) {
        first = false; nb = i + 1;
        const TensorDesc &ti = net->tensors[a[1]];
        Q.in = reinterpret_cast<const _Float16 *>(bufs[ti.buf]); Q.cs_in = ti.cs; Q.coff_in = ti.coff;
        const int32_t *b = op(nb);
        if (b[3] < 0 || !t16x8(b[3], 64)) return 0;
        const TensorDesc &tr = net->tensors[b[3]];
        Q.res = reinterpret_cast<const _Float16 *>(bufs[tr.buf]); Q.cs_res = tr.cs; Q.coff_res = tr.coff;
    } else return 0;
    const int32_t *b = op(nb);
    if (!(conv3(b, 1, 64, ACT_NONE) && b[1] == a[2] && b[3] >= 0 && b[4] >= 0 && b[19] && t16x8(b[2], 64) && t16x8(b[4], 64))) return 0;
    Q.wa = reinterpret_cast<const _Float16 *>(W(a, 16)); Q.kpad_a = a[13]; Q.bias_a = reinterpret_cast<const float *>(W(a, 17));
    Q.wb = reinterpret_cast<const _Float16 *>(W(b, 16)); Q.kpad_b = b[13]; Q.bias_b = reinterpret_cast<const float *>(W(b, 17));
    const TensorDesc &to = net->tensors[b[2]], &t2 = net->tensors[b[4]];
    Q.out = reinterpret_cast<_Float16 *>(bufs[to.buf]); Q.cs_out = to.cs; Q.coff_out = to.coff;
    Q.out2 = reinterpret_cast<_Float16 *>(bufs[t2.buf]); Q.cs_out2 = t2.cs; Q.coff_out2 = t2.coff;
    Q.aff2 = reinterpret_cast<const float *>(W(b, 18)); Q.cout_pad = b[12];
    Q.zero = net->d_zero; Q.n_img = nimg;
    return nb - i + 1;
}

MarsWsP mars_ws_params(const ConvP &P, int nimg) {
    MarsWsP Q;
    memset(&Q, 0, sizeof(Q));
    Q.in = P.in; Q.cs_in = P.cs_in; Q.coff_in = P.coff_in;
    Q.w = P.w; Q.kpad = P.kpad; Q.bias = P.bias;
    Q.res = P.res; Q.cs_res = P.cs_res; Q.coff_res = P.coff_res;
    Q.out = static_cast<_Float16 *>(P.out); Q.cs_out = P.cs_out; Q.coff_out = P.coff_out;
    Q.out2 = P.out2; Q.cs_out2 = P.cs_out2; Q.coff_out2 = P.coff_out2; Q.aff2 = P.aff2; Q.cout_pad = P.cout_pad;
    Q.zero = P.zero; Q.n_img = nimg;
    return Q;
}

}

extern "C" {

static int net_create(dd_ctx *ctx, const int32_t *program_host, int n_words, const void *weights_host,
                      int64_t n_weight_bytes, int max_batch, dd_net **out, bool share);
int dd_net_destroy(dd_net *n);

int dd_net_create(dd_ctx *ctx, const int32_t *program_host, int n_words, const void *weights_host,
                  int64_t n_weight_bytes, int max_batch, dd_net **out) {
    return net_create(ctx, program_host, n_words, weights_host, n_weight_bytes, max_batch, out, false);
}

int dd_net_create_shared(dd_ctx *ctx, const int32_t *program_host, int n_words, const void *weights_host,
                         int64_t n_weight_bytes, int max_batch, dd_net **out) {
    return net_create(ctx, program_host, n_words, weights_host, n_weight_bytes, max_batch, out, true);
}

static int net_create(dd_ctx *ctx, const int32_t *program_host, int n_words, const void *weights_host,
                      int64_t n_weight_bytes, int max_batch, dd_net **out, bool share) {
    DD_REQUIRE(ctx && program_host && weights_host && out && max_batch > 0 && n_words >= 8, DD_E_ARG,
               "dd_net_create: bad argument");
    DD_REQUIRE(program_host[0] == 0x314E4444, DD_E_ARG, "dd_net_create: bad program magic");
    const int nt = program_host[1], nb = program_host[2], no = program_host[3];
    DD_REQUIRE(n_words == 8 + nt * TENSOR_WORDS + nb * 2 + no * OP_WORDS, DD_E_ARG, "dd_net_create: program size mismatch");
    dd_net *n = new dd_net();
    struct Guard { dd_net *n; ~Guard() { if (n) (void)dd_net_destroy(n); } } guard{n};
    n->ctx = ctx;
    n->max_batch = max_batch;
    n->prog.assign(program_host, program_host + n_words);
    n->in_h = program_host[4];
    n->in_w = program_host[5];
    n->out_tensor = program_host[6];
    const int32_t *p = program_host + 8;
    for (int i = 0; i < nt; ++i, p += TENSOR_WORDS) n->tensors.push_back(TensorDesc{p[0], p[1], p[2], p[3], p[4], p[5], p[6], p[7]});
    DD_HIP(hipSetDevice(ctx->device));
    if (share) {
        const int32_t *ops = p + (size_t)nb * 2;
        std::vector<int> first(nb, -1), last(nb, -1);
        for (int t = 0; t < nt; ++t) DD_REQUIRE(n->tensors[t].buf >= 0 && n->tensors[t].buf < nb, DD_E_ARG, "dd_net_create_shared: tensor %d names buffer %d of %d", t, n->tensors[t].buf, nb);
        for (int i = 0; i < no; ++i)
            DD_REQUIRE((ops + (size_t)i * OP_WORDS)[0] < 16, DD_E_ARG, "dd_net_create_shared: uint8 programs keep one buffer per tensor (their borders are set once)");
        std::vector<int> gs(no), ge(no);
        for (int i = 0; i < no;) {
            int j = i;
            while (j + 1 < no && (ops + (size_t)j * OP_WORDS)[30] != 0) ++j;
            for (int k = i; k <= j; ++k) { gs[k] = i; ge[k] = j; }
            i = j + 1;
        }
        auto touch2 = [&](int t, int i) {
            if (t < 0 || t >= nt) return;
            const int b = n->tensors[t].buf;
            first[b] = first[b] < 0 ? gs[i] : std::min(first[b], gs[i]);
            last[b] = std::max(last[b], ge[i]);
        };
        for (int i = 0; i < no; ++i) {
            const int32_t *o = ops + (size_t)i * OP_WORDS;
            touch2(o[1], i); touch2(o[2], i); touch2(o[3], i); touch2(o[4], i);
        }
        if (n->out_tensor >= 0) last[n->tensors[n->out_tensor].buf] = no;
        std::vector<size_t> bytes(nb), off(nb, 0);
        size_t arena = 0;
        std::vector<int> order(nb);
        for (int b = 0; b < nb; ++b) { order[b] = b; bytes[b] = ((size_t)p[2 * b] * max_batch * dtype_size(p[2 * b + 1] & 0xff) + 256 + 255) & ~(size_t)255; }
        std::stable_sort(order.begin(), order.end(), [&](int a, int b) { return first[a] < first[b]; });
        std::vector<int> placed;
        for (int b : order) {
            if (first[b] < 0) { first[b] = 0; last[b] = no; }
            size_t at = 0;
            for (bool moved = true; moved;) {
                moved = false;
// ... 78 lines not shown

int dd_net_input_size(dd_net *n, int *h_host, int *w_host) {
    DD_REQUIRE(n && h_host && w_host, DD_E_ARG, "dd_net_input_size: NULL argument");
    *h_host = n->in_h; *w_host = n->in_w;
    return DD_OK;
}

int dd_net_max_batch(dd_net *n, int *out_host) {
    DD_REQUIRE(n && out_host, DD_E_ARG, "dd_net_max_batch: NULL argument");
    *out_host = n->max_batch;
    return DD_OK;
}

int dd_net_output(dd_net *n, int tensor, void **dev_ptr, int *h, int *w, int *c, int *cs, int *dtype) {
    DD_REQUIRE(n, DD_E_ARG, "dd_net_output: NULL net");
    const int t = tensor < 0 ? n->out_tensor : tensor;
    DD_REQUIRE(t >= 0 && t < (int)n->tensors.size(), DD_E_ARG, "dd_net_output: tensor %d out of range", t);
    const TensorDesc &d = n->tensors[t];
    if (dev_ptr) *dev_ptr = static_cast<char *>(n->bufs[d.buf]) + (size_t)d.coff * dtype_size(d.dtype);
    if (h) *h = d.h;
    if (w) *w = d.w;
    if (c) *c = d.c;
    if (cs) *cs = d.cs;
    if (dtype) *dtype = d.dtype;
    return DD_OK;
}

int dd_net_profile(dd_net *n, int enable) {
    DD_REQUIRE(n, DD_E_ARG, "dd_net_profile: NULL net");
    DD_DEVICE(n->ctx);
    if (enable && n->events.empty()) {
        n->events.resize(n->n_ops + 2);
        for (auto &e : n->events) DD_HIP(hipEventCreate(&e));
    }
    n->profile = enable != 0;
    return DD_OK;
}

int dd_net_profile_read(dd_net *n, float *ms_host, int cap, int *n_ops_host) {
    DD_REQUIRE(n && ms_host && n_ops_host, DD_E_ARG, "dd_net_profile_read: NULL argument");
    DD_DEVICE(n->ctx);
    DD_REQUIRE(n->profile && !n->events.empty(), DD_E_STATE, "dd_net_profile_read: profiling is off");
    DD_REQUIRE(cap >= n->n_ops, DD_E_ARG, "dd_net_profile_read: cap %d < %d ops", cap, n->n_ops);
    DD_HIP(hipEventSynchronize(n->events[n->n_ops + 1]));
    float empty = 0.f;
    DD_HIP(hipEventElapsedTime(&empty, n->events[n->n_ops], n->events[n->n_ops + 1]));
    for (int i = 0; i < n->n_ops; ++i) {
        DD_HIP(hipEventElapsedTime(&ms_host[i], n->events[i], n->events[i + 1]));
        ms_host[i] = ms_host[i] > empty ? ms_host[i] - empty : 0.f;
    }
    *n_ops_host = n->n_ops;
    return DD_OK;
}

int dd_net_op_launches(dd_net *n, int32_t *codes_host, int cap, int *n_ops_host) {
    DD_REQUIRE(n && codes_host && n_ops_host, DD_E_ARG, "dd_net_op_launches: NULL argument");
    DD_REQUIRE(cap >= n->n_ops, DD_E_ARG, "dd_net_op_launches: cap %d < %d ops", cap, n->n_ops);
    for (int i = 0; i < n->n_ops; ++i) codes_host[i] = i < (int)n->op_launch.size() ? n->op_launch[i] : OPK_DEFAULT;
    *n_ops_host = n->n_ops;
    return DD_OK;
}

int dd_net_read(dd_net *n, int tensor, int n_img, void *dst, int dst_on_device, void *stream) {
    DD_REQUIRE(n && dst && n_img >= 0 && n_img <= n->max_batch, DD_E_ARG, "dd_net_read: bad argument");
    DD_DEVICE(n->ctx);
    const int t = tensor < 0 ? n->out_tensor : tensor;
    DD_REQUIRE(t >= 0 && t < (int)n->tensors.size(), DD_E_ARG, "dd_net_read: tensor %d out of range", t);
    const TensorDesc &d = n->tensors[t];
    DD_REQUIRE(!n->arena || t == n->out_tensor, DD_E_STATE, "dd_net_read: tensor %d of an engine whose buffers share memory by lifetime "
               "(dd_net_create_shared): only the output tensor outlives the forward", t);
    DD_REQUIRE(d.coff == 0, DD_E_ARG, "dd_net_read: tensor %d is a channel slice", t);
    for (int i = 0; i < n->n_ops && i < (int)n->op_launch.size(); ++i) {
        const int32_t *o = n->prog.data() + n->ops_off + (size_t)i * OP_WORDS;
        DD_REQUIRE(!(o[2] == t && n->op_launch[i] == OPK_SSD_HEAD_DEC), DD_E_STATE,
                   "dd_net_read: tensor %d (the SSD head matrix) was not written: the head layers decoded in their epilogue "
                   "(dd_net_ssd_decode); read dd_net_ssd_decoded instead", t);
        DD_REQUIRE(!(o[2] == t && n->op_launch[i] == OPK_YOLO_HEAD_DEC), DD_E_STATE,
                   "dd_net_read: tensor %d (the Detect matrix) was not written: the head layers reduced their rows in their epilogue "
                   "(dd_net_yolo_decode); read dd_net_yolo_decoded instead", t);
        DD_REQUIRE(!((o[2] == t || o[4] == t) && n->op_launch[i] == OPK_FOLDED), DD_E_STATE,
                   "dd_net_read: tensor %d was not written by the last forward (op %d ran inside the next op's launch at this batch "
                   "size and its output stayed on chip); run a smaller batch or a program compiled without the fusion flags", t, i);
    }
    hipStream_t s = dd_pick_stream(n->ctx, stream);
    const size_t bytes = d.pad ? (size_t)n_img * (d.h + 2) * (d.w + 2) * d.cs
                               : (size_t)n_img * d.h * d.w * d.cs * dtype_size(d.dtype);
    if (!bytes) return DD_OK;
    DD_HIP(hipMemcpyAsync(dst, n->bufs[d.buf], bytes, dst_on_device ? hipMemcpyDeviceToDevice : hipMemcpyDeviceToHost, s));
    if (!dst_on_device) DD_HIP(hipStreamSynchronize(s));
    return DD_OK;
}

static int net_run_ops(dd_net *net, const uint8_t *input, int nimg, hipStream_t s);

int dd_net_use_graph(dd_net *net, int enable) {
    DD_REQUIRE(net, DD_E_ARG, "dd_net_use_graph: NULL net");
    DD_DEVICE(net->ctx);
    net->use_graph = enable != 0;
    if (!net->use_graph) net_drop_graphs(net);
    return DD_OK;
}

int dd_net_ssd_decode(dd_net *net, const float *anchors_host, int n_anchors, float score_thr, int enable) {
    DD_REQUIRE(net, DD_E_ARG, "dd_net_ssd_decode: NULL net");
    DD_DEVICE(net->ctx);
    net_drop_graphs(net);
    if (!enable) { net->ssd_dec = false; return DD_OK; }
    DD_REQUIRE(anchors_host && n_anchors > 0, DD_E_ARG, "dd_net_ssd_decode: anchors missing");
    int heads = 0;
    for (int i = 0; i < net->n_ops; ++i) {
        const int32_t *o = net->prog.data() + net->ops_off + (size_t)i * OP_WORDS;
        if (o[0] == OP_CONV && o[15] == EPI_SSD_HEAD) {
            DD_REQUIRE(o[18] && o[21] == n_anchors && 4 + o[20] <= 96, DD_E_ARG,
                       "dd_net_ssd_decode: head op %d has no per-anchor weight copy, or %d anchors / %d classes do not fit", i, o[21], o[20]);
            ++heads;
        }
        if (o[0] == 20) {
            DD_REQUIRE(o[21] == n_anchors, DD_E_ARG, "dd_net_ssd_decode: the program decodes %d anchors, %d given", o[21], n_anchors);
            ++heads;
        }
    }
    DD_REQUIRE(heads > 0, DD_E_ARG, "dd_net_ssd_decode: the program has no SSD head");
    if (net->dec_anchors != n_anchors) {
        for (void *q : {(void *)net->d_anchors, (void *)net->dec_boxes, (void *)net->dec_score, (void *)net->dec_keys, (void *)net->dec_cls}) (void)hipFree(q);
        net->d_anchors = net->dec_boxes = net->dec_score = net->dec_keys = nullptr; net->dec_cls = nullptr; net->dec_anchors = 0;
        const size_t per = (size_t)net->max_batch * n_anchors;
        DD_HIP(hipMalloc(&net->d_anchors, (size_t)n_anchors * 4 * sizeof(float)));
        DD_HIP(hipMalloc(&net->dec_boxes, per * 4 * sizeof(float)));
        DD_HIP(hipMalloc(&net->dec_score, per * sizeof(float)));
        DD_HIP(hipMalloc(&net->dec_keys, per * sizeof(float)));
        DD_HIP(hipMalloc(&net->dec_cls, per * sizeof(int)));
        net->dec_anchors = n_anchors;
    }
    DD_HIP(hipMemcpy(net->d_anchors, anchors_host, (size_t)n_anchors * 4 * sizeof(float), hipMemcpyHostToDevice));
    net->dec_thr = score_thr;
    net->ssd_dec = true;
    return DD_OK;
}

int dd_net_yolo_decode(dd_net *net, int enable) {
    DD_REQUIRE(net, DD_E_ARG, "dd_net_yolo_decode: NULL net");
    DD_DEVICE(net->ctx);
    net_drop_graphs(net);
    if (!enable) { net->yolo_dec = false; return DD_OK; }
    DD_REQUIRE(!net->ssd_dec, DD_E_STATE, "dd_net_yolo_decode: the SSD decode is on for this network");
    int heads = 0, rows = 0;
    for (int i = 0; i < net->n_ops; ++i) {
        const int32_t *o = net->prog.data() + net->ops_off + (size_t)i * OP_WORDS;
        if (o[0] == OP_CONV && o[15] == EPI_YOLO) {
            DD_REQUIRE(o[18] && !o[19] && o[20] >= 6 && o[20] <= 96, DD_E_ARG,
                       "dd_net_yolo_decode: head op %d has no per-anchor weight copy, or %d columns per row do not fit", i, o[20]);
            DD_REQUIRE(rows == 0 || rows == o[21], DD_E_ARG, "dd_net_yolo_decode: heads disagree on the rows per image");
            rows = o[21];
            ++heads;
        }
    }
    DD_REQUIRE(heads > 0 && rows > 0, DD_E_ARG, "dd_net_yolo_decode: the program has no YOLOv5 Detect head");
    if (net->dec_anchors != rows || !net->dec_boxes) {
        for (void *q : {(void *)net->d_anchors, (void *)net->dec_boxes, (void *)net->dec_score, (void *)net->dec_keys, (void *)net->dec_cls}) (void)hipFree(q);
        net->d_anchors = net->dec_boxes = net->dec_score = net->dec_keys = nullptr; net->dec_cls = nullptr; net->dec_anchors = 0;
        const size_t per = (size_t)net->max_batch * rows;
        DD_HIP(hipMalloc(&net->dec_boxes, per * 4 * sizeof(float)));
        DD_HIP(hipMalloc(&net->dec_score, per * sizeof(float)));
        DD_HIP(hipMalloc(&net->dec_cls, per * sizeof(int)));
        net->dec_anchors = rows;
    }
    net->yolo_dec = true;
    return DD_OK;
}

int dd_net_yolo_decoded(dd_net *net, float **boxes, float **conf, int **classes, int *rows) {
    DD_REQUIRE(net && net->yolo_dec, DD_E_STATE, "dd_net_yolo_decoded: dd_net_yolo_decode is off");
    if (boxes) *boxes = net->dec_boxes;
    if (conf) *conf = net->dec_score;
    if (classes) *classes = net->dec_cls;
    if (rows) *rows = net->dec_anchors;
    return DD_OK;
}

int dd_net_yolo_decoded_read(dd_net *net, int n, float *boxes_host, float *conf_host, int *classes_host) {
    DD_REQUIRE(net && net->yolo_dec && n >= 0 && n <= net->max_batch, DD_E_STATE, "dd_net_yolo_decoded_read: decode is off or n out of range");
    DD_DEVICE(net->ctx);
    DD_HIP(hipStreamSynchronize(net->ctx->stream));
    const size_t per = (size_t)n * net->dec_anchors;
    if (boxes_host) DD_HIP(hipMemcpy(boxes_host, net->dec_boxes, per * 4 * sizeof(float), hipMemcpyDeviceToHost));
    if (conf_host) DD_HIP(hipMemcpy(conf_host, net->dec_score, per * sizeof(float), hipMemcpyDeviceToHost));
    if (classes_host) DD_HIP(hipMemcpy(classes_host, net->dec_cls, per * sizeof(int), hipMemcpyDeviceToHost));
    return DD_OK;
}


int dd_net_ssd_decoded(dd_net *net, float **boxes, float **scores, int **classes, float **keys) {
    DD_REQUIRE(net && net->ssd_dec, DD_E_STATE, "dd_net_ssd_decoded: dd_net_ssd_decode is off");
    if (boxes) *boxes = net->dec_boxes;
    if (scores) *scores = net->dec_score;
    if (classes) *classes = net->dec_cls;
    if (keys) *keys = net->dec_keys;
    return DD_OK;
}

int dd_net_ssd_heads_u8(dd_net *net, const uint8_t **box_q, const uint8_t **cls_q, int *cls_stride, const uint8_t **lut, float *quant4_host,
                        int *n_anchors, int *n_classes) {
    DD_REQUIRE(net && box_q && cls_q && cls_stride && lut && quant4_host && n_anchors && n_classes, DD_E_ARG, "dd_net_ssd_heads_u8: NULL argument");
    DD_REQUIRE(!net->arena, DD_E_STATE, "dd_net_ssd_heads_u8: the engine's buffers share memory by lifetime (dd_net_create_shared): the head "
               "tensors do not outlive the forward");
    for (int i = 0; i < net->n_ops; ++i) {
        const int32_t *o = net->prog.data() + net->ops_off + (size_t)i * OP_WORDS;
        if (o[0] != 20) continue;
        DD_REQUIRE(o[1] >= 0 && o[1] < (int)net->tensors.size() && o[3] >= 0 && o[3] < (int)net->tensors.size(), DD_E_ARG, "dd_net_ssd_heads_u8: head tensors out of range");
        const TensorDesc &tb = net->tensors[o[1]], &tc = net->tensors[o[3]];
        DD_REQUIRE(tb.cs == 4 && tb.h == o[21] && tc.h == o[21] && tb.w == 1 && tc.w == 1 && o[20] <= tc.cs && !tb.pad && !tc.pad && !tb.coff && !tc.coff, DD_E_ARG,
                   "dd_net_ssd_heads_u8: head tensors of %d anchors are not [anchors][4] / [anchors][>= %d] bytes", o[21], o[20]);
        *box_q = static_cast<const uint8_t *>(net->bufs[tb.buf]); *cls_q = static_cast<const uint8_t *>(net->bufs[tc.buf]);
        *cls_stride = tc.cs; *n_anchors = o[21]; *n_classes = o[20];
        *lut = reinterpret_cast<const uint8_t *>(net->d_weights + (size_t)(uint32_t)o[16]);
        const float *of = reinterpret_cast<const float *>(o);
        for (int q = 0; q < 4; ++q) quant4_host[q] = of[32 + q];
        return DD_OK;
    }
    DD_REQUIRE(false, DD_E_ARG, "dd_net_ssd_heads_u8: the program has no uint8 SSD head");
}

int dd_net_ssd_decoded_read(dd_net *net, int n, float *boxes_host, float *scores_host, int *classes_host, float *keys_host) {
    DD_REQUIRE(net && net->ssd_dec && n >= 0 && n <= net->max_batch, DD_E_STATE, "dd_net_ssd_decoded_read: decode is off or n out of range");
    DD_DEVICE(net->ctx);
    hipStream_t s = net->ctx->stream;
    DD_HIP(hipStreamSynchronize(s));
    const size_t per = (size_t)n * net->dec_anchors;
    if (!per) return DD_OK;
    if (boxes_host) DD_HIP(hipMemcpy(boxes_host, net->dec_boxes, per * 4 * sizeof(float), hipMemcpyDeviceToHost));
    if (scores_host) DD_HIP(hipMemcpy(scores_host, net->dec_score, per * sizeof(float), hipMemcpyDeviceToHost));
    if (classes_host) DD_HIP(hipMemcpy(classes_host, net->dec_cls, per * sizeof(int), hipMemcpyDeviceToHost));
    if (keys_host) DD_HIP(hipMemcpy(keys_host, net->dec_keys, per * sizeof(float), hipMemcpyDeviceToHost));
    return DD_OK;
}

int dd_net_forward(dd_net *net, const uint8_t *input, int nimg, void *stream) {
    DD_REQUIRE(net && input && nimg >= 0, DD_E_ARG, "dd_net_forward: bad argument");
    DD_DEVICE(net->ctx);
    DD_REQUIRE(nimg <= net->max_batch, DD_E_CAPACITY, "dd_net_forward: batch %d > max_batch %d", nimg, net->max_batch);
    if (nimg == 0) return DD_OK;
    net->last_batch = nimg;
    hipStream_t s = dd_pick_stream(net->ctx, stream);
    auto eager = [&]() -> int {
        const int rc = net_run_ops(net, input, nimg, s);
        if (net->slab_moved) { net->slab_moved = false; net_drop_graphs(net); }
        return rc;
    };
    if (!net->use_graph || net->profile) return eager();
    if (net->graphs.size() > 256) net_drop_graphs(net);
    dd_net::GraphEntry &g = net->graphs[std::make_pair(static_cast<const void *>(input), nimg)];
    if (g.exec) { DD_HIP(hipGraphLaunch(g.exec, s)); return DD_OK; }
    if (g.calls++ == 0) return eager();
    DD_HIP(hipStreamBeginCapture(s, hipStreamCaptureModeThreadLocal));
    const int rc = net_run_ops(net, input, nimg, s);
    hipGraph_t graph = nullptr;
    const hipError_t e = hipStreamEndCapture(s, &graph);
    if (rc != DD_OK) { if (graph) (void)hipGraphDestroy(graph); return rc; }
    DD_HIP(e);
    g.graph = graph;
    DD_HIP(hipGraphInstantiate(&g.exec, graph, nullptr, nullptr, 0));
    DD_HIP(hipGraphLaunch(g.exec, s));
    return DD_OK;
}

static int net_run_ops(dd_net *net, const uint8_t *input, int nimg, hipStream_t s) {
    auto base = [&](int t) -> char * {
        const TensorDesc &d = net->tensors[t];
        return static_cast<char *>(net->bufs[d.buf]);
    };
    net->op_launch.assign((size_t)net->n_ops, OPK_DEFAULT);
    ConvP stem_p;
    bool stem_pending = false;
    bool wide_pending = false, wide_ready = false;
    bool input_pending = false;
    float input_mean = 0.f, input_scale = 1.f;
    int input_op = -1;
    ConvP unit_a;
    bool unit_pending = false;
    ConvP pw_p;
    bool pw_pending = false;
    bool proj_done = false;
    MarsPairP pair64;
    bool pair64_first = false;
    int pair_left = 0;
    ConvP pair_a, pair_b;
    bool pair_pending = false;
    int pair_op = -1;
    auto flush_pair = [&]() -> int {
        pair_pending = false;
        net->op_launch[pair_op] = OPK_RES_UNIT;
        return launch_res_unit(s, pair_a, pair_b, nimg, net->ctx->device);
    };
    auto run_ws = [&](ConvP &P) { return P.cin == 256 ? launch_conv_ws<4>(s, P, net->ctx->device) : launch_conv_ws<8>(s, P, net->ctx->device); };
    int first_op = 0;
    bool mid_on = false;
    {
        static const int chunk_env = getenv("DD_Q_FRONT_CHUNK") ? atoi(getenv("DD_Q_FRONT_CHUNK")) : 0;
        auto opw = [&](int k) { return net->prog.data() + net->ops_off + (size_t)k * OP_WORDS; };
        const char *front_env = getenv("DD_Q_FRONT"), *front_min_env = getenv("DD_Q_FRONT_MIN");
        const int front_min = front_min_env ? atoi(front_min_env) : 24;
        {
            const char *mid_env = getenv("DD_Q_MID");
            mid_on = !(mid_env && atoi(mid_env) == 0) && nimg >= front_min;
        }
        if (!(front_env && atoi(front_env) == 0) && chunk_env <= 0 && nimg >= front_min && net->n_ops > 3 && opw(0)[0] == 16 && opw(1)[0] == 19 && opw(2)[0] == 19) {
            if (net->profile) for (int k = 0; k < 3; ++k) DD_HIP(hipEventRecord(net->events[k], s));
            int ran = 0;
            const int rc = netq_run_front(net, opw(0), opw(1), opw(2), input, nimg, s, &ran);
            if (rc != DD_OK) return rc;
            if (ran) { first_op = 3; net->op_launch[0] = OPK_FOLDED; net->op_launch[1] = OPK_FOLDED; net->op_launch[2] = OPK_Q_FRONT; }
        }
        if (first_op == 0 && chunk_env > 0 && nimg > chunk_env && net->n_ops > 3 && opw(0)[0] == 16 && opw(1)[0] == 19 && opw(2)[0] == 19 && opw(1)[1] == opw(0)[2] && opw(2)[1] == opw(1)[2]) {
            const TensorDesc &t2 = net->tensors[opw(2)[2]];
            const size_t img_out = (size_t)(t2.h + 2) * (t2.w + 2) * t2.cs;
            void *&out_buf = net->bufs[t2.buf];
            void *const out_base = out_buf;
            if (net->profile) for (int k = 0; k < 3; ++k) DD_HIP(hipEventRecord(net->events[k], s));
            for (int c0 = 0; c0 < nimg; c0 += chunk_env) {
                const int nc = std::min(chunk_env, nimg - c0);
                out_buf = static_cast<char *>(out_base) + (size_t)c0 * img_out;
                for (int k = 0; k < 3; ++k) {
                    int handled = 0;
                    const int rc = netq_run_op(net, k, opw(k), input + (size_t)c0 * net->in_h * net->in_w * 3, nc, s, &handled);
                    if (rc != DD_OK || !handled) { out_buf = out_base; return rc != DD_OK ? rc : DD_E_ARG; }
                }
            }
            out_buf = out_base;
            first_op = 3;
        }
    }
    for (int i = first_op; i < net->n_ops; ++i) {
        if (net->profile) DD_HIP(hipEventRecord(net->events[i], s));
        const int32_t *o = net->prog.data() + net->ops_off + (size_t)i * OP_WORDS;
        const float *of = reinterpret_cast<const float *>(o);
        const int kind = o[0], src = o[1], dst = o[2], res = o[3], dst2 = o[4];
        const TensorDesc *ts = src >= 0 ? &net->tensors[src] : nullptr;
        const TensorDesc *td = dst >= 0 ? &net->tensors[dst] : nullptr;
        DD_REQUIRE(!input_pending || (kind == OP_CONV && i == input_op + 1), DD_E_STATE, "dd_net_forward: input op %d was folded into an op that did not take it", input_op);
        if (mid_on && kind == 19 && i + 1 < net->n_ops && net->prog[net->ops_off + (size_t)(i + 1) * OP_WORDS] == 19) {
            const int32_t *o4 = net->prog.data() + net->ops_off + (size_t)(i + 1) * OP_WORDS;
            if (net->profile) DD_HIP(hipEventRecord(net->events[i + 1], s));
            int ran = 0;
            const int rc = netq_run_mid(net, o, o4, nimg, s, &ran);
            if (rc != DD_OK) return rc;
            if (ran) { net->op_launch[i] = OPK_FOLDED; net->op_launch[i + 1] = OPK_Q_MID; ++i; continue; }
        }
        DD_REQUIRE((!wide_pending || kind == OP_CONV) && (!wide_ready || kind == OP_MAXPOOL), DD_E_STATE, "dd_net_forward: op %d does not take the first layer folded into it", i);
        if (pair_pending && kind != OP_CONV) { const int rc = flush_pair(); if (rc != DD_OK) return rc; }
        if (pw_pending && kind != OP_DWCONV) {
            pw_pending = false; net->op_launch[i - 1] = OPK_CONV_WS;
            const int rc = run_ws(pw_p);
            if (rc != DD_OK) return rc;
        }
        if (unit_pending && kind != OP_CONV) {
            unit_pending = false; net->op_launch[i - 1] = OPK_DEFAULT;
            const int rc = launch_conv3x3_rw(s, unit_a, nimg, false, net->ctx->device);
            if (rc != DD_OK) return rc;
        }
        if (stem_pending && !(kind == OP_CONV && o[29]) && kind != OP_DWPW) {
            stem_pending = false; net->op_launch[i - 1] = OPK_DEFAULT;
            const int rc = launch_stem(s, stem_p, nimg);
            if (rc != DD_OK) return rc;
        }
        switch (kind) {
            case OP_INPUT: {
                const int s2d = o[5];
                const int m = nimg * td->h * td->w;
                if (s2d && o[30] && !o[6] && td->cs == 32 && !td->coff && i + 1 < net->n_ops && net->use_rw) {
                    const int32_t *q = net->prog.data() + net->ops_off + (size_t)(i + 1) * OP_WORDS;
                    static const bool off = getenv("DD_FOCUS_UNFUSED") && atoi(getenv("DD_FOCUS_UNFUSED")) != 0;
                    if (!off && q[0] == OP_CONV && q[1] == dst && q[5] == 3 && q[6] == 3 && q[7] == 1 && q[8] == 1 && q[9] == 1 && q[10] == 32 &&
                        q[12] == 32 && q[14] == ACT_SILU && q[15] == EPI_F16 && q[3] < 0 && q[4] < 0 && !q[29] && td->w % 32 == 0) {
                        input_pending = true; input_mean = of[32]; input_scale = of[33]; input_op = i;
                        net->op_launch[i] = OPK_FOLDED;
                        break;
                    }
                }
                if (s2d && td->cs >= 16 && td->cs % 8 == 0) {
                    const int cpp = td->cs / 8;
                    DD_REQUIRE((long long)m * cpp < (1ll << 31), DD_E_CAPACITY, "dd_net_forward: %d x %d input chunks", m, cpp);
                    hipLaunchKernelGGL(input_s2d_chunks_k, dim3(dd_ceil_div(m * cpp, 256)), dim3(256), 0, s, input, net->in_h, net->in_w, o[6],
                                       of[32], of[33], m * cpp, cpp, reinterpret_cast<_Float16 *>(base(dst)) + td->coff, td->cs);
                } else
                hipLaunchKernelGGL(input_k, dim3(dd_ceil_div(m, 256)), dim3(256), 0, s, input, net->in_h, net->in_w, o[6],
                                   of[32], of[33], s2d, m, reinterpret_cast<_Float16 *>(base(dst)) + td->coff, td->cs);
                DD_LAUNCH_CHECK();
                break;
            }
            case OP_CONV: {
#define DD_NO_PENDING() DD_REQUIRE(!unit_pending && !pair_pending && !stem_pending && !pw_pending && !input_pending, DD_E_STATE, \
                                   "dd_net_forward: op %d is folded into a neighbouring launch while an earlier op's launch is still held back", i)
                if (proj_done) { DD_NO_PENDING(); proj_done = false; net->op_launch[i] = OPK_FOLDED_PREV; break; }
                if (pair_left > 0) {
                    DD_NO_PENDING();
                    if (--pair_left > 0) { net->op_launch[i] = OPK_FOLDED; break; }
                    const int rc = mars_pair64_launch(s, net->ctx->device, pair64, pair64_first);
                    if (rc != DD_OK) return rc;
                    net->op_launch[i] = OPK_MARS_PAIR;
                    break;
                }
                if (o[30] == 3 || o[30] == 4) {
                    const int n_ops = mars_pair_match(net, i, nimg, pair64, pair64_first);
                    if (n_ops) { DD_NO_PENDING(); pair_left = n_ops - 1; net->op_launch[i] = OPK_FOLDED; break; }
                }
#undef DD_NO_PENDING
                ConvP P;
                memset(&P, 0, sizeof(P));
                P.in = reinterpret_cast<const _Float16 *>(base(src)); P.H = ts->h; P.W = ts->w; P.cs_in = ts->cs;
                P.coff_in = ts->coff; P.cin = o[10];
                P.kh = o[5]; P.kw = o[6]; P.stride = o[7]; P.pad_t = o[8]; P.pad_l = o[9];
                P.cout = o[11]; P.cout_pad = o[12]; P.kpad = o[13]; P.act = o[14]; P.epi = o[15];
                P.w = reinterpret_cast<const _Float16 *>(net->d_weights + (size_t)(uint32_t)o[16]);
                P.bias = reinterpret_cast<const float *>(net->d_weights + (size_t)(uint32_t)o[17]);
                P.ho = o[26]; P.wo = o[27]; P.m = nimg * P.ho * P.wo;
                P.out = base(dst); P.cs_out = td->cs; P.coff_out = td->coff;
                if (res >= 0) {
                    const TensorDesc &tr = net->tensors[res];
                    P.res = reinterpret_cast<const _Float16 *>(base(res)); P.cs_res = tr.cs; P.coff_res = tr.coff;
                }
                if (dst2 >= 0) {
                    const TensorDesc &t2 = net->tensors[dst2];
                    P.out2 = reinterpret_cast<_Float16 *>(base(dst2)); P.cs_out2 = t2.cs; P.coff_out2 = t2.coff;
                    P.aff2 = reinterpret_cast<const float *>(net->d_weights + (size_t)(uint32_t)o[18]);
                }
                if (dst2 < 0 && o[19]) {
                    P.aff2 = reinterpret_cast<const float *>(net->d_weights + (size_t)(uint32_t)o[18]);
                    P.post_aff = 1;
                }
                for (int q = 0; q < 6; ++q) P.p[q] = o[20 + q];
                for (int q = 0; q < 8; ++q) P.f[q] = of[32 + q];
                int rc;
                DD_REQUIRE(!o[29] || (net->use_rw && P.kh == 3 && P.stride == 1 && P.cin == 32 && P.cout_pad == 32), DD_E_ARG,
                           "dd_net_forward: fused pooling is only built for the 3x3 32->32 kernel");
                if (unit_pending) {
                    unit_pending = false;
                    if (res_unit_fusable(unit_a, P, nimg)) {
                        P.zero = net->d_zero;
                        if (pair_pending) {
                            if (res_pair_fusable(pair_a, pair_b, unit_a, P, nimg)) {
                                pair_pending = false;
                                rc = launch_res_pair(s, pair_a, pair_b, unit_a, P, nimg, net->ctx->device);
                                if (rc != DD_OK) return rc;
                                net->op_launch[i] = OPK_RES_PAIR;
                                break;
                            }
                            if ((rc = flush_pair()) != DD_OK) return rc;
                        }
                        if (o[30] == 2 && i + 2 < net->n_ops) {
                            pair_a = unit_a; pair_b = P; pair_pending = true; pair_op = i;
                            net->op_launch[i] = OPK_FOLDED;
                            break;
                        }
                        rc = launch_res_unit(s, unit_a, P, nimg, net->ctx->device);
                        if (rc != DD_OK) return rc;
                        net->op_launch[i] = OPK_RES_UNIT;
                        break;
                    }
                    if (pair_pending && (rc = flush_pair()) != DD_OK) return rc;
                    net->op_launch[i - 1] = OPK_DEFAULT;
                    rc = launch_conv3x3_rw(s, unit_a, nimg, false, net->ctx->device);
                    if (rc != DD_OK) return rc;
                }
                if (pair_pending) {
                    const bool next_a = net->use_rw && P.kh == 3 && P.kw == 3 && P.stride == 1 && P.cin == 32 && P.cout_pad == 32 && P.epi == EPI_F16 &&
                                        P.pad_t == 1 && P.pad_l == 1 && o[30] && !o[29] && i + 1 < net->n_ops && nimg >= 160 && !P.res && !P.out2 &&
                                        P.in == static_cast<const _Float16 *>(pair_b.out2);
                    if (!next_a && (rc = flush_pair()) != DD_OK) return rc;
                }
                if (P.epi == EPI_YOLO && net->yolo_dec && o[18] && !o[19]) {
                    DD_REQUIRE(P.p[1] == net->dec_anchors, DD_E_ARG, "dd_net_forward: head of %d rows, decode set up for %d", P.p[1], net->dec_anchors);
                    P.w = reinterpret_cast<const _Float16 *>(net->d_weights + (size_t)(uint32_t)o[18]);
                    P.bias = reinterpret_cast<const float *>(net->d_weights + (size_t)(uint32_t)o[31]);
                    P.zero = net->d_zero;
                    P.dec_boxes = net->dec_boxes; P.dec_score = net->dec_score; P.dec_cls = net->dec_cls;
                    rc = launch_yolo_head_dec(s, P);
                    if (rc != DD_OK) return rc;
                    net->op_launch[i] = OPK_YOLO_HEAD_DEC;
                    break;
                }
                if (P.epi == EPI_SSD_HEAD && net->ssd_dec && o[18] && !o[19]) {
                    DD_REQUIRE(P.p[1] == net->dec_anchors, DD_E_ARG, "dd_net_forward: head of %d anchors, decode set up for %d", P.p[1], net->dec_anchors);
                    P.w = reinterpret_cast<const _Float16 *>(net->d_weights + (size_t)(uint32_t)o[18]);
                    P.bias = reinterpret_cast<const float *>(net->d_weights + (size_t)(uint32_t)o[31]);
                    P.zero = net->d_zero;
                    P.anchors = net->d_anchors; P.dec_boxes = net->dec_boxes; P.dec_score = net->dec_score; P.dec_keys = net->dec_keys;
                    P.dec_cls = net->dec_cls; P.dec_thr = net->dec_thr;
                    rc = launch_ssd_head_dec(s, P);
                    if (rc != DD_OK) return rc;
                    net->op_launch[i] = OPK_SSD_HEAD_DEC;
                    break;
                }
                const bool bk32 = o[28] == 32;
                const bool glds = !bk32 && net->use_glds;
                P.zero = net->d_zero;
                if (net->use_rw && P.kh == 3 && P.kw == 3 && P.stride == 1 && P.cin == 32 && P.cout_pad == 32 &&
                    P.epi == EPI_F16 && P.pad_t == 1 && P.pad_l == 1) {
                    if (input_pending) { input_pending = false; P.src8 = input; P.in_mean = input_mean; P.in_scale = input_scale; }
                    if (o[29]) { P.p[0] = td->h; P.p[1] = td->w; }
                    if (wide_pending) {
                        wide_pending = false;
                        const int32_t *r = o + OP_WORDS;
                        const TensorDesc &tp = net->tensors[r[2]];
                        P.src8 = stem_p.src8; P.in_mean = stem_p.in_mean; P.in_scale = stem_p.in_scale;
                        P.dw_w = stem_p.w; P.dw_bias = stem_p.bias; P.dw_act = stem_p.act;
                        P.out = base(r[2]); P.cs_out = tp.cs; P.coff_out = tp.coff; P.p[0] = tp.h; P.p[1] = tp.w;
                        stem_p = P; wide_ready = true; net->op_launch[i] = OPK_FOLDED;
                        break;
                    }
                    if (stem_pending) {
                        stem_pending = false;
                        if (o[29] && pool_rows_fusable(P, nimg) && stem_p.out == static_cast<const void *>(P.in) && !P.coff_in) {
                            P.src8 = stem_p.src8; P.in_mean = stem_p.in_mean; P.in_scale = stem_p.in_scale;
                            P.dw_w = stem_p.w; P.dw_bias = stem_p.bias; P.dw_act = stem_p.act;
                        } else {
                            net->op_launch[i - 1] = OPK_DEFAULT;
                            rc = launch_stem(s, stem_p, nimg);
                            if (rc != DD_OK) return rc;
                        }
                    }
                    if (o[30] && !o[29] && i + 1 < net->n_ops && nimg >= 160 && !P.res && !P.out2) {
                        if (pair_pending && P.in != static_cast<const _Float16 *>(pair_b.out2) && (rc = flush_pair()) != DD_OK) return rc;
                        unit_a = P; unit_pending = true;
                        net->op_launch[i] = OPK_FOLDED;
                        break;
                    }
                    if (o[29] && pool_rows_fusable(P, nimg)) net->op_launch[i] = P.src8 ? OPK_POOL_ROWS_STEM : OPK_POOL_ROWS;
                    rc = launch_conv3x3_rw(s, P, nimg, o[29] != 0, net->ctx->device);
                } else if (mars_ws_s1_eligible(P)) {
                    const MarsWsP Q = mars_ws_params(P, nimg);
                    net->op_launch[i] = OPK_MARS_WS;
                    rc = mars_ws128_launch(s, net->ctx->device, Q, P.res ? MARS_WS_S1_RES : MARS_WS_S1, P.act, P.out2 != nullptr);
                } else if (o[30] == 3 && i + 1 < net->n_ops && mars_ws_s2_eligible(P) && mars_proj_follows(net, i, P)) {
                    const int32_t *q = net->prog.data() + net->ops_off + (size_t)(i + 1) * OP_WORDS;
                    const TensorDesc &qs = net->tensors[q[1]], &qd = net->tensors[q[2]];
                    MarsWsP Q = mars_ws_params(P, nimg);
                    Q.in2 = reinterpret_cast<const _Float16 *>(base(q[1])); Q.cs_in2 = qs.cs; Q.coff_in2 = qs.coff;
                    Q.w2 = reinterpret_cast<const _Float16 *>(net->d_weights + (size_t)(uint32_t)q[16]); Q.kpad2 = q[13];
                    Q.bias2 = reinterpret_cast<const float *>(net->d_weights + (size_t)(uint32_t)q[17]);
                    Q.out2 = reinterpret_cast<_Float16 *>(base(q[2])); Q.cs_out2 = qd.cs; Q.coff_out2 = qd.coff;
                    net->op_launch[i] = OPK_MARS_WS;
                    rc = mars_ws128_launch(s, net->ctx->device, Q, MARS_WS_S2_PROJ, P.act, false);
                    proj_done = true;
                } else if (s2_rows_eligible(P, nimg, net->max_batch)) {
                    net->op_launch[i] = OPK_S2_ROWS;
                    rc = launch_conv3x3_s2_rows(s, P, nimg, net->ctx->device);
                } else if (c64_rows_eligible(P, nimg, net->max_batch)) {
                    net->op_launch[i] = OPK_C64_ROWS;
                    rc = launch_conv3x3_c64_rows(s, P, nimg, net->ctx->device);
                } else if (c64_strips_eligible(P, nimg, net->max_batch)) {
                    net->op_launch[i] = OPK_C64_STRIPS;
                    rc = launch_conv3x3_c64_strips(s, P, nimg, net->ctx->device);
                } else if (ws_eligible(P) && o[30] && i + 1 < net->n_ops && P.act == ACT_RELU6) {
                    pw_p = P; pw_pending = true; net->op_launch[i] = OPK_FOLDED;
                    break;
                } else if (ws_eligible(P)) {
                    net->op_launch[i] = OPK_CONV_WS;
                    rc = P.cin == 256 ? launch_conv_ws<4>(s, P, net->ctx->device) : launch_conv_ws<8>(s, P, net->ctx->device);
                } else if (P.cout_pad <= 32) {
                    rc = bk32 ? launch_conv<4, 1, 1, 2, 32, false>(s, P, net->slab, net->max_batch, net->ctx->device, &net->slab_moved)
                       : (glds && P.m >= 16384) ? launch_conv<4, 1, 2, 2, 64, true>(s, P, net->slab, net->max_batch, net->ctx->device, &net->slab_moved)
                       : glds ? launch_conv<4, 1, 1, 2, 64, true>(s, P, net->slab, net->max_batch, net->ctx->device, &net->slab_moved)
                              : launch_conv<4, 1, 1, 2, 64, false>(s, P, net->slab, net->max_batch, net->ctx->device, &net->slab_moved);
                } else if (glds && net->tile_mode != 1 && P.m >= 16384 && P.cout_pad >= 128) {
                    const int gy128 = dd_ceil_div(P.cout_pad, 128);
                    const int c128 = dd_ceil_div(dd_ceil_div(P.m, 128) * gy128, 512) * 128;
                    const int c192 = dd_ceil_div(dd_ceil_div(P.m, 192) * gy128, 512) * 192;
                    if (P.epi == EPI_F16 && c192 <= c128 && net->tile_mode != 2)
                        rc = launch_conv<4, 2, 3, 4, 64, true>(s, P, net->slab, net->max_batch, net->ctx->device, &net->slab_moved);
                    else
                        rc = launch_conv<4, 2, 2, 4, 64, true>(s, P, net->slab, net->max_batch, net->ctx->device, &net->slab_moved);
                } else if (glds && net->tile_mode != 1 && P.m >= 16384 && P.cout_pad == 64) {
                    rc = launch_conv<4, 2, 2, 2, 64, true>(s, P, net->slab, net->max_batch, net->ctx->device, &net->slab_moved);
                } else if (glds && net->tile_mode != 1 && P.m >= 4096 && P.cout_pad >= 128) {
                    rc = launch_conv<2, 2, 2, 4, 64, true>(s, P, net->slab, net->max_batch, net->ctx->device, &net->slab_moved);
                } else {
                    rc = bk32 ? launch_conv<2, 2, 2, 2, 32, false>(s, P, net->slab, net->max_batch, net->ctx->device, &net->slab_moved)
                       : glds ? launch_conv<2, 2, 2, 2, 64, true>(s, P, net->slab, net->max_batch, net->ctx->device, &net->slab_moved)
                              : launch_conv<2, 2, 2, 2, 64, false>(s, P, net->slab, net->max_batch, net->ctx->device, &net->slab_moved);
                }
                if (rc != DD_OK) return rc;
                break;
            }
            case OP_STEM: {
                ConvP P;
                memset(&P, 0, sizeof(P));
                P.src8 = input; P.H = net->in_h; P.W = net->in_w; P.in_mean = of[32]; P.in_scale = of[33];
                P.zero = net->d_zero;
                P.kh = P.kw = 3; P.stride = o[7]; P.pad_t = o[8]; P.pad_l = o[9];
                P.cout = o[11]; P.cout_pad = o[12]; P.act = o[14]; P.epi = EPI_F16; P.splitk = 1;
                DD_REQUIRE(P.cout_pad == 32 && (P.stride == 1 || P.stride == 2), DD_E_ARG, "dd_net_forward: stem needs 32 output channels, stride 1 or 2");
                P.w = reinterpret_cast<const _Float16 *>(net->d_weights + (size_t)(uint32_t)o[16]);
                P.bias = reinterpret_cast<const float *>(net->d_weights + (size_t)(uint32_t)o[17]);
                P.ho = td->h; P.wo = td->w; P.m = nimg * P.ho * P.wo;
                P.out = base(dst); P.cs_out = td->cs; P.coff_out = td->coff;
                static const bool unfused = getenv("DD_STEM_UNFUSED") && atoi(getenv("DD_STEM_UNFUSED")) != 0;
                if (o[30] && !unfused && i + 1 < net->n_ops && P.stride == 1 && P.pad_t == 1 && P.pad_l == 1 && P.cout == 32 && P.act == ACT_ELU &&
                    P.W == 32 && (reinterpret_cast<uintptr_t>(input) & 3) == 0) {
                    stem_p = P; stem_pending = true; net->op_launch[i] = OPK_FOLDED;
                    break;
                }
                auto sole_reader = [&](int t, int reader) {
                    if (t < 0 || t == net->out_tensor) return false;
                    for (int k = 0; k < net->n_ops; ++k) {
                        const int32_t *w = net->prog.data() + net->ops_off + (size_t)k * OP_WORDS;
                        for (int a : {w[1], w[3]})
                            if (k != reader && a >= 0 && net->tensors[a].buf == net->tensors[t].buf) return false;
                    }
                    return true;
                };
                const char *wide_env = getenv("DD_STEM_WIDE"), *wide_min_env = getenv("DD_STEM_WIDE_MIN");
                const bool wide_off = wide_env ? atoi(wide_env) == 0 : !STEM_WIDE_DEFAULT;
                const int wide_min = wide_min_env ? atoi(wide_min_env) : STEM_WIDE_MIN_CROPS;
                if (o[30] && !wide_off && nimg >= wide_min && i + 2 < net->n_ops && net->use_rw && stem_wide_geometry(P.H, P.W) && P.stride == 1 &&
                    P.pad_t == 1 && P.pad_l == 1 && P.cout == 32 && P.act == ACT_ELU && !td->coff && (reinterpret_cast<uintptr_t>(input) & 3) == 0) {
                    const int32_t *q = o + OP_WORDS, *r = o + 2 * OP_WORDS;
                    if (q[0] == OP_CONV && q[1] == dst && q[5] == 3 && q[6] == 3 && q[7] == 1 && q[8] == 1 && q[9] == 1 && q[10] == 32 && q[11] == 32 && q[12] == 32 &&
                        q[14] == ACT_ELU && q[15] == EPI_F16 && q[3] < 0 && q[4] < 0 && !q[29] && !q[30] &&
                        r[0] == OP_MAXPOOL && r[1] == q[2] && r[5] == 3 && r[6] <= 1 && r[7] == 2 && r[8] == 0 && r[2] >= 0 && sole_reader(q[2], i + 2) &&
                        net->tensors[r[2]].h == P.H / 2 - 1 && net->tensors[r[2]].w == P.W / 2 - 1 && net->tensors[r[2]].c == 32) {
                        stem_p = P; wide_pending = true; net->op_launch[i] = OPK_FOLDED;
                        break;
                    }
// ... 149 lines not shown
```

### deepdish_amd/engine.py

```python
import ctypes
import numpy as np
import torch

from ._lib import lib, check, P
from .runtime import default_context, ptr
from . import nets


class Net:
    def __init__(self, program, max_batch, context=None, shared=False):
        self.ctx = context or default_context()
        self.program = program
        self.max_batch = int(max_batch)
        words, blob = program.serialize()
        self._words = words
        blob_arr = np.frombuffer(blob, dtype=np.uint8)
        h = P()
        create = lib().dd_net_create_shared if shared else lib().dd_net_create
        check(create(self.ctx.handle, ptr(words), len(words), ptr(blob_arr), len(blob), self.max_batch, ctypes.byref(h)), 'dd_net_create')
        self._h = h
        t = program.tensors[program.out_tensor]
        self.out_shape = (t['h'], t['w'], t['cs'])
        self.out_dtype = {nets.DT_F16: torch.float16, nets.DT_F32: torch.float32, nets.DT_U8: torch.uint8}[t['dtype']]
        self.weight_bytes = len(blob)

    def __del__(self):
        try:
            if self._h:
                lib().dd_net_destroy(self._h)
                self._h = None
        except Exception:
            pass

    def activation_bytes(self):
        v = ctypes.c_int64()
        check(lib().dd_net_activation_bytes(self._h, ctypes.byref(v)), 'dd_net_activation_bytes')
        return v.value

    def use_graph(self, enable=True):
        check(lib().dd_net_use_graph(self._h, int(bool(enable))), 'dd_net_use_graph')

    def ssd_decode(self, anchors, score_thr, enable=True):
        if not enable:
            check(lib().dd_net_ssd_decode(self._h, None, 0, 0.0, 0), 'dd_net_ssd_decode')
            self._dec_anchors = 0
            return
        a = np.ascontiguousarray(anchors, dtype=np.float32)
        check(lib().dd_net_ssd_decode(self._h, ptr(a), len(a), float(score_thr), int(bool(enable))), 'dd_net_ssd_decode')
        self._dec_anchors = len(a) if enable else 0

    def ssd_heads_u8(self):
        box, cls, lut = P(), P(), P()
        stride, na, nc = ctypes.c_int(), ctypes.c_int(), ctypes.c_int()
        quant = np.zeros(4, np.float32)
        check(lib().dd_net_ssd_heads_u8(self._h, ctypes.byref(box), ctypes.byref(cls), ctypes.byref(stride), ctypes.byref(lut), ptr(quant),
                                        ctypes.byref(na), ctypes.byref(nc)), 'dd_net_ssd_heads_u8')
        return dict(box=box.value, cls=cls.value, lut=lut.value, cls_stride=stride.value, n_anchors=na.value, n_classes=nc.value, quant=quant)

    def ssd_decoded(self, n=None):
        n = self._last_n if n is None else n
        A = self._dec_anchors
        out = (np.zeros((n, A, 4), np.float32), np.zeros((n, A), np.float32), np.zeros((n, A), np.int32), np.zeros((n, A), np.float32))
        check(lib().dd_net_ssd_decoded_read(self._h, n, *[ptr(o) for o in out]), 'dd_net_ssd_decoded_read')
        return out

    def yolo_decode(self, enable=True):
        check(lib().dd_net_yolo_decode(self._h, int(bool(enable))), 'dd_net_yolo_decode')
        self._yolo_rows = int(self.program.meta['rows']) if enable else 0

    def yolo_decoded(self, n=None):
        n = self._last_n if n is None else n
        R = self._yolo_rows
        out = (np.zeros((n, R, 4), np.float32), np.zeros((n, R), np.float32), np.zeros((n, R), np.int32))
        check(lib().dd_net_yolo_decoded_read(self._h, n, *[ptr(o) for o in out]), 'dd_net_yolo_decoded_read')
        return out

    def forward(self, images, stream=None):
        if isinstance(images, np.ndarray):
            images = self.ctx.to_device(images, np.uint8)
        n = int(images.shape[0])
        assert images.dtype == torch.uint8 and tuple(images.shape[1:]) == (self.program.in_h, self.program.in_w, 3)
        check(lib().dd_net_forward(self._h, ptr(images), n, stream), 'dd_net_forward')
        self._last_n = n
        return n

    def read(self, n=None, tensor=-1, to_host=True):
        n = self._last_n if n is None else n
        t = self.program.tensors[self.program.out_tensor if tensor < 0 else tensor]
        shape = (t['h'] + 2, t['cs'] // 16, t['w'] + 2, 16) if t.get('q16') else (t['h'], t['w'], t['cs'])
        dt = {nets.DT_F16: torch.float16, nets.DT_F32: torch.float32, nets.DT_U8: torch.uint8}[t['dtype']]
        if to_host:
            out = np.zeros((n,) + shape, dtype={torch.float16: np.float16, torch.float32: np.float32, torch.uint8: np.uint8}[dt])
            check(lib().dd_net_read(self._h, tensor, n, ptr(out), 0, None), 'dd_net_read')
            return out
        out = self.ctx.empty((n,) + shape, dt)
        check(lib().dd_net_read(self._h, tensor, n, ptr(out), 1, None), 'dd_net_read')
        return out

    def output_ptr(self, tensor=-1):
        p = P()
        check(lib().dd_net_output(self._h, tensor, ctypes.byref(p), None, None, None, None, None), 'dd_net_output')
        return p.value
```

### deepdish_amd/profile.py

```python
import ctypes
import numpy as np

from ._lib import lib, check
from .runtime import ptr

PEAK_F16_TFLOPS = 2500.0
PEAK_HBM_GBS = 8000.0
PEAK_I8_TOPS = 5000.0


def last_batch(net):
    n = ctypes.c_int()
    check(lib().dd_net_last_batch(net._h, ctypes.byref(n)), 'dd_net_last_batch')
    return n.value


def net_op_times(net):
    n = len(net.program.ops)
    ms = np.zeros(n, dtype=np.float32)
    cnt = ctypes.c_int()
    check(lib().dd_net_profile_read(net._h, ptr(ms), n, ctypes.byref(cnt)), 'dd_net_profile_read')
    return ms


OPK_FOLDED = 1
OPK_NAMES = {2: 'conv3x3_pool_rows_k', 3: 'conv3x3_pool_rows_k<STEM>', 4: 'res_unit_rows_k', 5: 'ssd_front_k', 6: 'conv3x3_c64_rows_k', 7: 'conv3x3_s2_rows_k', 8: 'conv_ws_k', 9: 'conv_ws_dw_k', 10: 'dwpw_rows_k', 11: 'conv_glds_k<ssd_head_decode>', 12: 'res_pair_rows_k', 13: 'conv_glds_k<yolo_head_decode>', 14: 'mars_ws128_k', 16: 'mars_pair64_k', 17: 'q_dwm_k', 18: 'conv3x3_c64_rows_k<strips>', 19: 'q_front_k', 20: 'q_mid_k', 21: 'q_conv_k<add>', 22: 'q_add_k', 23: 'stem_conv_pool_wide_k'}
OPK_FOLDED_PREV = 15


def net_op_launches(net):
    n = len(net.program.ops)
    codes = np.zeros(n, dtype=np.int32)
    cnt = ctypes.c_int(0)
    check(lib().dd_net_op_launches(net._h, ptr(codes), n, ctypes.byref(cnt)), 'dd_net_op_launches')
    return codes


def launches_of(net, ms, batch):
    out, pend = [], None
    for t, info, code in zip(ms, net.program.info, net_op_launches(net)):
        fl, by = info['flops'] * batch, info['bytes'] * batch + info.get('wbytes', 0)
        if code == OPK_FOLDED:
            if pend is None:
                pend = [float(t), fl, info.get('src_bytes', 0) * batch + info.get('wbytes', 0)]
            else:
                pend[0] += float(t); pend[1] += fl; pend[2] += info.get('wbytes', 0)
            continue
        if code == OPK_FOLDED_PREV and out:
            k0, t0, f0, b0 = out[-1]
            out[-1] = (k0, t0 + float(t), f0 + fl, b0 + by)
            continue
        if pend is not None:
            t, fl, by = float(t) + pend[0], fl + pend[1], by - info.get('src_bytes', 0) * batch + pend[2]
            pend = None
        out.append((OPK_NAMES.get(int(code), info['kernel']), float(t), fl, by))
    return out


def profile_nets(run_once, nets_with_batch, reps=20):
    for _, net, _ in nets_with_batch:
        check(lib().dd_net_profile(net._h, 1), 'dd_net_profile')
    acc = {}
    try:
        for _ in range(reps):
            run_once()
            for name, net, batch in nets_with_batch:
                ms = net_op_times(net)
                b = batch() if callable(batch) else batch
                for kname, t, fl, by in launches_of(net, ms, b):
                    k = acc.setdefault(kname, dict(ms=0.0, flops=0.0, bytes=0.0, launches=0))
                    k['ms'] += t; k['flops'] += fl; k['bytes'] += by; k['launches'] += 1
    finally:
        for _, net, _ in nets_with_batch:
            check(lib().dd_net_profile(net._h, 0), 'dd_net_profile')
    for k in acc.values():
        for f in ('ms', 'flops', 'bytes'):
            k[f] /= reps
        k['launches'] /= reps
    return acc


def pmc_traffic(kernel, streams):
    import json, os
    root = os.path.join(os.path.dirname(os.path.dirname(os.path.abspath(__file__))), 'profiles')
    path = next((p for p in (os.path.join(root, 'r%02d_pmc_traffic_s%d.json' % (r, streams)) for r in (6, 5, 4, 3, 2, 1)) if os.path.exists(p)), None)
    if path is None:
        return None, None
    keys = [part.replace(',', ', ') for part in kernel.split('+')]
    tot_b = tot_n = 0.0
    for k, v in json.load(open(path)).items():
        if any(key in k for key in keys):
            tot_b += (v['hbm_read_bytes_corrected'] + v['hbm_write_bytes']) * v['launches']
            tot_n += v['launches']
    src = 'profiles/%s (rocprofv3 --pmc FETCH_SIZE and WRITE_SIZE passes of `bench.py --groups 1 --streams %d`, committed; not measured in this run)' % (os.path.basename(path), streams)
    return (tot_b / tot_n, src) if tot_n else (None, None)


def dominant_kernel_roofline(pipes, step_group, args, reps=20):
    f0 = args.warmup
    p = pipes[0]
    nets = [('mars', p.enc, lambda: last_batch(p.enc))]
    if p.det is not None:
        nets.append(('ssd', p.det, p.S))
    state = dict(f=f0)

    def run_once():
        step_group(0, state['f'])
        state['f'] = f0 + (state['f'] + 1 - f0) % max(1, args.steps)

    acc = profile_nets(run_once, nets, reps)
    per_kernel = {n: round(v['ms'], 5) for n, v in sorted(acc.items(), key=lambda kv: -kv[1]['ms'])}
    fam = [n for n in ('conv_glds_k', 'conv_ws_k', 'conv_ws_dw_k', 'conv_glds_k<ssd_head_decode>') if n in acc]
    if len(fam) > 1:
        parts = [acc.pop(n) for n in fam]
        acc['+'.join(fam)] = {f: sum(p[f] for p in parts) for f in ('ms', 'flops', 'bytes', 'launches')}
    name, k = max(acc.items(), key=lambda kv: kv[1]['ms'])
    sec = k['ms'] * 1e-3
    avg_us = 1e3 * k['ms'] / max(k['launches'], 1e-9)
# ... 18 lines not shown
```

### include/deepdish_hip.h

```cpp
#ifndef DEEPDISH_HIP_H
#define DEEPDISH_HIP_H

#include <stdint.h>

#ifdef __cplusplus
extern "C" {
#endif

#define DD_OK            0
#define DD_E_ARG        -1
#define DD_E_HIP        -2
#define DD_E_STATE      -3
#define DD_E_CAPACITY   -4

#define DD_FEATURE_DIM 128

typedef struct dd_ctx dd_ctx;
typedef struct dd_tracker dd_tracker;
typedef struct dd_net dd_net;
typedef struct dd_pipeline dd_pipeline;

const char *dd_last_error(void);
int dd_version(void);

// ... 28 lines not shown

int dd_nms_ssd(dd_ctx *ctx, const double *xyxy, const double *scores, int k, double iou_thr,
               int *out_idx, int *out_n, void *stream);

int dd_lsap_host(const double *cost_host, int nr, int nc, int *row_ind_host, int *col_ind_host);

int dd_pyset_difference_order_host(const int *a_host, int na, const int *b_host, int nb, int *out_host,
                                   int *out_n_host);

int dd_tracker_create(dd_ctx *ctx, double max_cosine_distance, double max_iou_distance,
                      int max_age, int n_init, int nn_budget ,
                      int track_capacity, int gallery_capacity, dd_tracker **out);
int dd_tracker_create_metric(dd_ctx *ctx, int metric, double matching_threshold, double max_iou_distance,
                             int max_age, int n_init, int nn_budget ,
                             int track_capacity, int gallery_capacity, dd_tracker **out);
int dd_tracker_destroy(dd_tracker *trk);
int dd_tracker_predict(dd_tracker *trk);
int dd_tracker_update(dd_tracker *trk, const double *tlwh_host, const float *feats,
                      int feats_on_device, int n);
int dd_tracker_count(dd_tracker *trk, int which, int *out_n_host);
int dd_tracker_read(dd_tracker *trk, int which, int64_t *ints6_host, double *means_host,
                    double *covs_host);
int dd_tracker_track_update(dd_tracker *t, int64_t track_id, const double *tlwh_host, const float *feat, int feat_on_device);
int dd_tracker_track_predict(dd_tracker *t, int64_t track_id);
int dd_tracker_track_set(dd_tracker *t, int64_t track_id, int state, int time_since_update);
int dd_tracker_remove(dd_tracker *t, const int64_t *track_ids_host, int n);
int dd_tracker_next_id(dd_tracker *trk, int64_t *out_host);

int dd_tracker_last_cost(dd_tracker *trk, double *app_host, double *iou_host, int cap, int *rows_host, int *cols_host);
int dd_tracker_last_matches(dd_tracker *trk, int *pairs_host, int cap, int *out_m_host);

int dd_crop_resize(dd_ctx *ctx, const uint8_t *frame, int H, int W, const int64_t *boxes_host,
                   int n, int ph, int pw, uint8_t *out, int *valid_host, void *stream);
int dd_crop_resize_f64(dd_ctx *ctx, const uint8_t *frame, int H, int W, const double *boxes_host, int n, int ph,
                       int pw, uint8_t *out, int *valid_host, void *stream);

int dd_fake_encode(dd_ctx *ctx, const uint8_t *patches, int n, int mode, float *out, void *stream);

int dd_resize_lanczos(dd_ctx *ctx, const uint8_t *src, int H, int W, int src_c, int swap_rb,
                      uint8_t *dst, int h, int w, void *stream);
int dd_resize_lanczos_batch(dd_ctx *ctx, const uint8_t *src, int batch, int H, int W, int src_c, int swap_rb,
                            uint8_t *dst, int h, int w, void *stream);
int dd_resize_bilinear(dd_ctx *ctx, const uint8_t *src, int H, int W, int c,
                       uint8_t *dst, int h, int w, void *stream);

typedef struct dd_ingest dd_ingest;
int dd_ingest_create(dd_ctx *ctx, int slots, int n_streams, int src_h, int src_w, int dst_h, int dst_w, int flip,
                     dd_ingest **out);
int dd_ingest_destroy(dd_ingest *g);
int dd_ingest_host_slot(dd_ingest *g, int slot, uint8_t **host_ptr, int64_t *n_bytes);
int dd_ingest_wait_uploaded(dd_ingest *g, int slot);
int dd_ingest_submit(dd_ingest *g, int slot);
int dd_ingest_acquire(dd_ingest *g, int slot, void *consumer_stream, const uint8_t **frames_dev);
int dd_ingest_release(dd_ingest *g, int slot, void *consumer_stream);

typedef struct dd_mog2 dd_mog2;
int dd_mog2_create(dd_ctx *ctx, int n_streams, int height, int width, int history, double var_threshold, int detect_shadows,
                   dd_mog2 **out);
int dd_mog2_destroy(dd_mog2 *m);
int dd_mog2_apply(dd_mog2 *m, const uint8_t *frames, double learning_rate, uint8_t *mask, uint8_t *masked_frames, void *stream);
int dd_mog2_state(dd_mog2 *m, int stream_index, float *weight_host, float *variance_host, float *mean_host, uint8_t *nmodes_host);
int dd_mask_box_count(dd_ctx *ctx, const uint8_t *mask, int n_streams, int height, int width, const int *boxes_xywh_host,
                      const int *box_stream_host, int n_boxes, int *counts_host, void *stream);

int dd_net_create(dd_ctx *ctx, const int32_t *program_host, int n_words, const void *weights_host,
                  int64_t n_weight_bytes, int max_batch, dd_net **out);
int dd_net_create_shared(dd_ctx *ctx, const int32_t *program_host, int n_words, const void *weights_host,
                         int64_t n_weight_bytes, int max_batch, dd_net **out);
int dd_net_activation_bytes(dd_net *net, int64_t *out_host);
int dd_net_destroy(dd_net *net);
int dd_net_forward(dd_net *net, const uint8_t *input, int n, void *stream);
int dd_net_output(dd_net *net, int tensor, void **dev_ptr_host, int *h_host, int *w_host, int *c_host,
                  int *cs_host, int *dtype_host);

int dd_net_use_graph(dd_net *net, int enable);
int dd_net_input_size(dd_net *net, int *h_host, int *w_host);
int dd_net_max_batch(dd_net *net, int *out_host);
int dd_net_last_batch(dd_net *net, int *out_host);
int dd_net_read(dd_net *net, int tensor, int n, void *dst, int dst_on_device, void *stream);

int dd_net_profile(dd_net *net, int enable);
int dd_net_profile_read(dd_net *net, float *ms_host, int cap, int *n_ops_host);
int dd_net_op_launches(dd_net *net, int32_t *codes_host, int cap, int *n_ops_host);

int dd_ssd_postprocess(dd_ctx *ctx, const float *raw, const float *anchors, int n_anchors,
                       int n_classes, int max_det, float score_thr, float iou_thr,
                       float *boxes, float *classes, float *scores, int *count, void *stream);

int dd_ssd_decode(dd_ctx *ctx, const float *raw, const float *anchors, int n_anchors, int n_classes, float score_thr,
                  float *boxes, float *scores, int *classes, float *keys, int batch, void *stream);
int dd_ssd_postprocess_decoded(dd_ctx *ctx, const float *dec_boxes, const float *dec_scores, const int *dec_classes,
                               const float *dec_keys, int n_anchors, int max_det, float score_thr, float iou_thr,
                               float *boxes, float *classes, float *scores, int *count, int batch, void *stream);
int dd_net_ssd_decode(dd_net *net, const float *anchors_host, int n_anchors, float score_thr, int enable);
int dd_net_ssd_decoded(dd_net *net, float **boxes_dev, float **scores_dev, int **classes_dev, float **keys_dev);
int dd_net_ssd_decoded_read(dd_net *net, int n, float *boxes_host, float *scores_host, int *classes_host, float *keys_host);

int dd_ssd_regular_nms_decoded(dd_ctx *ctx, const float *dec_boxes, const float *scores_in, int score_ld, int first_class_col,
                               int n_anchors, int n_classes, int max_det, int detections_per_class, float score_thr, float iou_thr,
                               float *boxes, float *classes, float *scores, int *count, int batch, void *stream);
int dd_ssd_postprocess_regular(dd_ctx *ctx, const float *raw, const float *anchors, int n_anchors, int n_classes, int max_det,
                               int detections_per_class, float score_thr, float iou_thr, float *boxes, float *classes, float *scores,
                               int *count, int batch, void *stream);
int dd_ssd_postprocess_regular_u8(dd_ctx *ctx, const uint8_t *box_q, const uint8_t *cls_q, int cls_stride, const uint8_t *logistic_table,
                                  const float *quant4_host, const float *anchors, int n_anchors, int n_classes, int max_det,
                                  int detections_per_class, float score_thr, float iou_thr, float *boxes, float *classes, float *scores,
                                  int *count, int batch, void *stream);
int dd_net_ssd_heads_u8(dd_net *net, const uint8_t **box_q_dev, const uint8_t **cls_q_dev, int *cls_stride_host,
                        const uint8_t **logistic_table_dev, float *quant4_host, int *n_anchors_host, int *n_classes_host);

int dd_net_yolo_decode(dd_net *net, int enable);
int dd_net_yolo_decoded(dd_net *net, float **boxes, float **conf, int **classes, int *rows);
int dd_net_yolo_decoded_read(dd_net *net, int n, float *boxes_host, float *conf_host, int *classes_host);

int dd_ssd_detections(dd_ctx *ctx, const float *boxes, const float *classes, const float *scores, int batch,
                      int max_det, double confidence, double iou_thr, double img_w, double img_h, double *out_boxes,
                      int *out_cls, double *out_scores, int *out_n, void *stream);

int dd_yolov5_decode(dd_ctx *ctx, const float *raw, int n_rows, int n_cls, float thr,
                     float img_w, float img_h, float *out_boxes, float *out_scores,
                     int *out_cls, int cap, int *out_n, void *stream);

int dd_pipeline_create(dd_ctx *ctx, int n_streams, int frame_h, int frame_w, dd_net *detector,
                       const float *anchors_host, int n_anchors, int n_classes, dd_net *encoder,
                       const char *labels_nl, const char *wanted_nl, double max_cosine_distance,
                       double nms_max_overlap, double max_iou_distance, int max_age, int n_init,
                       const double *line_host, int track_capacity, int gallery_capacity, dd_pipeline **out);
int dd_pipeline_destroy(dd_pipeline *p);
int dd_pipeline_detector_adaptor(dd_pipeline *p, int adaptor);
int dd_pipeline_ssd_options(dd_pipeline *p, int max_detections, float nms_score_threshold, float nms_iou_threshold);
int dd_pipeline_ssd_regular_nms(dd_pipeline *p, int detections_per_class);
int dd_pipeline_detector_skip_frames(dd_pipeline *p, int n);
int dd_pipeline_metric(dd_pipeline *p, int metric);
int dd_pipeline_step(dd_pipeline *p, const uint8_t *frames, const double *inj_boxes_host,
                     const double *inj_scores_host, const int *inj_cls_host, const int *inj_offsets_host);
int dd_pipeline_step2(dd_pipeline *p, const uint8_t *frames, const uint8_t *frames_next, const double *inj_boxes_host,
                      const double *inj_scores_host, const int *inj_cls_host, const int *inj_offsets_host);
int dd_pipeline_detector_stream(dd_pipeline *p, void **stream_out);
int dd_pipeline_background_subtraction(dd_pipeline *p, double ratio, int masking);
int dd_pipeline_motion_mask(dd_pipeline *p, uint8_t *dst, int dst_on_device, long long *rejected_host);
int dd_pipeline_counts(dd_pipeline *p, int64_t *counts_host);
int dd_pipeline_tracker(dd_pipeline *p, int stream, dd_tracker **out);
int dd_pipeline_stage_seconds(dd_pipeline *p, double *out4_host, long long *steps_host);
int dd_pipeline_stage_gpu_ms(dd_pipeline *p, double *out6_host, long long *steps_host);
int dd_pipeline_detections(dd_pipeline *p, int stream, double *boxes_host, double *scores_host, int *classes_host, int cap, int *n_host);

int dd_counts_accumulate(dd_ctx *ctx, int64_t *acc, const int64_t *counts_host, int n, void *stream);

#ifdef __cplusplus
}
#endif
#endif
```

Baseline: 143,700 frames/s.

## Write compact even-pixel skip tensors for MARS stride-2 projections

When a MARS block output is read only by the following stride-2 1x1 projection, the producer kernel now writes just the even pixels into a compact, reader-ordered buffer instead of the full strided tensor. The consumer kernels (pair64 first block and ws128 stride-2 projection) read that compact layout directly. This cuts skip-tensor write and read traffic in the encoder. In exchange those tensors are no longer fully materialised, so dd_net_read rejects them unless keep_tensors is set or the feature is disabled by env var. Graph entries now record which tensors were compacted.

```diff
diff --git a/deepdish_amd/_lib.py b/deepdish_amd/_lib.py
--- a/deepdish_amd/_lib.py
+++ b/deepdish_amd/_lib.py
@@ -78,6 +78,8 @@
     'dd_net_profile': [P, c_int],
     'dd_net_profile_read': [P, P, c_int, POINTER(c_int)],
     'dd_net_op_launches': [P, P, c_int, POINTER(c_int)],
+    'dd_net_keep_tensors': [P, c_int],
+    'dd_net_compact_skips': [P, P],
     'dd_ssd_postprocess': [P, P, P, c_int, c_int, c_int, c_float, c_float, P, P, P, P, P],
     'dd_ssd_decode': [P, P, P, c_int, c_int, c_float, P, P, P, P, c_int, P],
     'dd_ssd_postprocess_decoded': [P, P, P, P, P, c_int, c_int, c_float, c_float, P, P, P, P, c_int, P],
diff --git a/deepdish_amd/csrc/mars_pair.hip b/deepdish_amd/csrc/mars_pair.hip
--- a/deepdish_amd/csrc/mars_pair.hip
+++ b/deepdish_amd/csrc/mars_pair.hip
@@ -99,8 +99,9 @@
             stp[h] = col < 15 ? (size_t)nstep * 31 * 15 * P.cs_in : 0;
         }
         const int jr = lane >> 5, xx = lane & 7;
-        src[4] = P.in2 + ((size_t)n0 * 31 + 2 * (2 * wave + jr)) * 15 * P.cs_in2 + (size_t)(2 * xx) * P.cs_in2 + P.coff_in2 + pl * 8;
-        stp[4] = (size_t)nstep * 31 * 15 * P.cs_in2;
+        src[4] = P.in2_compact ? P.in2 + (size_t)n0 * MARS_SKIP32_HALVES + wave * 512 + lane * 8
+                               : P.in2 + ((size_t)n0 * 31 + 2 * (2 * wave + jr)) * 15 * P.cs_in2 + (size_t)(2 * xx) * P.cs_in2 + P.coff_in2 + pl * 8;
+        stp[4] = P.in2_compact ? (size_t)nstep * MARS_SKIP32_HALVES : (size_t)nstep * 31 * 15 * P.cs_in2;
         n_dma = 5;
     } else {
         const int pl = lane >> 3, xx = lane & 7;
@@ -213,7 +214,8 @@
                 h8 o;
 #pragma unroll
                 for (int i = 0; i < 8; ++i) o[i] = (_Float16)v[i];
-                *reinterpret_cast<h8 *>(P.out + m * P.cs_out + P.coff_out + co) = o;
+                if (!(!FIRST && P.out_compact)) *reinterpret_cast<h8 *>(P.out + m * P.cs_out + P.coff_out + co) = o;
+                else if (j == 0 && (x & 1) == 0) *reinterpret_cast<h8 *>(P.out + n * MARS_SKIP64_HALVES + (((half * 4 + fq) * 8 + F) * 4 + (x >> 1)) * 8) = o;
                 const f4 s0 = *reinterpret_cast<const f4 *>(cst + 128 + co), s1 = *reinterpret_cast<const f4 *>(cst + 128 + co + 4);
                 const f4 t0 = *reinterpret_cast<const f4 *>(cst + 192 + co), t1 = *reinterpret_cast<const f4 *>(cst + 192 + co + 4);
                 h8 o2;
@@ -250,5 +252,7 @@
 int mars_pair64_launch(hipStream_t s, int device, const MarsPairP &P, bool first) {
     DD_REQUIRE(P.n_img > 0 && P.in && P.wa && P.wb && P.bias_a && P.bias_b && P.out && P.out2 && P.aff2 && P.zero && (first ? (P.in2 && P.wp) : P.res != nullptr), DD_E_ARG,
                "mars_pair64: bad argument");
+    DD_REQUIRE(first ? (!P.out_compact && !(P.in2_compact && P.coff_in2)) : (!P.in2_compact && !(P.out_compact && P.coff_out)), DD_E_ARG,
+               "mars_pair64: the first block reads a compact skip tensor, the last one writes one, each a whole buffer");
     return first ? launch_pair<true>(s, device, P) : launch_pair<false>(s, device, P);
 }
diff --git a/deepdish_amd/csrc/mars_tail.h b/deepdish_amd/csrc/mars_tail.h
--- a/deepdish_amd/csrc/mars_tail.h
+++ b/deepdish_amd/csrc/mars_tail.h
@@ -4,6 +4,7 @@
 struct MarsWsP {
     const _Float16 *in;  int cs_in, coff_in;
     const _Float16 *in2; int cs_in2, coff_in2;
+    int in2_compact;
     const _Float16 *w;   int kpad;
     const _Float16 *w2;  int kpad2;
     const float *bias, *bias2;
@@ -19,6 +20,8 @@
 
 int mars_ws128_launch(hipStream_t s, int device, const MarsWsP &P, int mode, int act, bool out2);
 
+enum { MARS_SKIP32_HALVES = 16 * 4 * 8 * 8, MARS_SKIP64_HALVES = 8 * 8 * 4 * 8 };
+
 struct MarsPairP {
     const _Float16 *in;  int cs_in, coff_in;
     const _Float16 *in2; int cs_in2, coff_in2;
@@ -31,5 +34,7 @@
     const float *aff2; int cout_pad;
     const _Float16 *zero;
     int n_img;
+    int in2_compact;
+    int out_compact;
 };
 int mars_pair64_launch(hipStream_t s, int device, const MarsPairP &P, bool first);
diff --git a/deepdish_amd/csrc/mars_tail.hip b/deepdish_amd/csrc/mars_tail.hip
--- a/deepdish_amd/csrc/mars_tail.hip
+++ b/deepdish_amd/csrc/mars_tail.hip
@@ -107,8 +107,10 @@
         src_a = P.in + (size_t)n0 * 128 * P.cs_in + ((wave * 8 + col) * P.cs_in + P.coff_in + pl * 8);
         src_b = src_a + (size_t)64 * P.cs_in;
         const int ch = (wave & 3) * 64 + lane;
-        src_c = P.in2 + (size_t)n0 * 128 * P.cs_in2 + ((2 * ((ch >> 2) & 7) * 8 + 2 * (ch & 3)) * P.cs_in2 + P.coff_in2 + (ch >> 5) * 8);
-        step_a = step_b = (size_t)nstep * 128 * P.cs_in; step_c = (size_t)nstep * 128 * P.cs_in2;
+        src_c = P.in2_compact ? P.in2 + (size_t)n0 * MARS_SKIP64_HALVES + ch * 8
+                              : P.in2 + (size_t)n0 * 128 * P.cs_in2 + ((2 * ((ch >> 2) & 7) * 8 + 2 * (ch & 3)) * P.cs_in2 + P.coff_in2 + (ch >> 5) * 8);
+        step_a = step_b = (size_t)nstep * 128 * P.cs_in;
+        step_c = P.in2_compact ? (size_t)nstep * MARS_SKIP64_HALVES : (size_t)nstep * 128 * P.cs_in2;
     }
     auto issue = [&]() {
         char *T = smem + OFF_T + dq_slot * TILE_B;
@@ -341,6 +343,7 @@
     DD_REQUIRE((long long)P.n_img * 128 * (P.cs_in > P.cs_out ? P.cs_in : P.cs_out) < (1ll << 40), DD_E_CAPACITY, "mars_ws128: batch of %d", P.n_img);
     if (mode == MARS_WS_S2_PROJ) {
         DD_REQUIRE(P.in2 && P.w2 && P.out2 && act == ACT_ELU, DD_E_ARG, "mars_ws128: stride-2 form needs the projection operands and ELU");
+        DD_REQUIRE(!P.in2_compact || !P.coff_in2, DD_E_ARG, "mars_ws128: a compact projection operand is a whole buffer");
         return launch_one<MARS_WS_S2_PROJ, ACT_ELU, false>(s, device, P);
     }
     if (mode == MARS_WS_S1) {
diff --git a/deepdish_amd/csrc/net_priv.h b/deepdish_amd/csrc/net_priv.h
--- a/deepdish_amd/csrc/net_priv.h
+++ b/deepdish_amd/csrc/net_priv.h
@@ -33,7 +33,9 @@
     int tile_mode = 0;
     std::vector<hipEvent_t> events;
     std::vector<int32_t> op_launch;
-    struct GraphEntry { int calls = 0; hipGraph_t graph = nullptr; hipGraphExec_t exec = nullptr; };
+    bool keep_tensors = false;
+    int compact_raw[2] = {-1, -1};
+    struct GraphEntry { int calls = 0; hipGraph_t graph = nullptr; hipGraphExec_t exec = nullptr; int compact_raw[2] = {-1, -1}; };
     bool use_graph = false;
     std::map<std::pair<const void *, int>, GraphEntry> graphs;
 };
diff --git a/deepdish_amd/csrc/nets.hip b/deepdish_amd/csrc/nets.hip
--- a/deepdish_amd/csrc/nets.hip
+++ b/deepdish_amd/csrc/nets.hip
@@ -189,8 +189,8 @@
 #ifndef DD_EPI_NT
 #define DD_EPI_NT true
 #endif
-template <int ACT = -1, bool BIAS = true, int EF = -1, bool NT = DD_EPI_NT, bool TAIL = true>
-__device__ __forceinline__ void conv_epilogue_f16x8(const ConvP &P, const Epi8 &E, int m, int co, float v[8], const h8 *res_pre = nullptr) {
+template <int ACT = -1, bool BIAS = true, int EF = -1, bool NT = DD_EPI_NT, bool TAIL = true, bool RAW_AT = false>
+__device__ __forceinline__ void conv_epilogue_f16x8(const ConvP &P, const Epi8 &E, int m, int co, float v[8], const h8 *res_pre = nullptr, h8 *raw_at = nullptr) {
     const int act = ACT < 0 ? P.act : ACT;
     const bool has_res = EF < 0 ? P.res != nullptr : EF >= 1, has_out2 = EF < 0 ? P.out2 != nullptr : EF == 1;
 #pragma unroll
@@ -212,9 +212,11 @@
         for (int r = 0; r < 8; ++r)
             if (co + r >= P.cout) o[r] = (_Float16)0.f;
     }
-    h8 *dst = reinterpret_cast<h8 *>(static_cast<_Float16 *>(P.out) + (size_t)m * P.cs_out + P.coff_out + co);
-    if constexpr (NT) __builtin_nontemporal_store(o, dst);
-    else *dst = o;
+    h8 *dst = RAW_AT ? raw_at : reinterpret_cast<h8 *>(static_cast<_Float16 *>(P.out) + (size_t)m * P.cs_out + P.coff_out + co);
+    if (!RAW_AT || dst) {
+        if constexpr (NT) __builtin_nontemporal_store(o, dst);
+        else *dst = o;
+    }
     if (has_out2) {
         h8 o2;
 #pragma unroll
@@ -1564,7 +1566,7 @@
 constexpr int rp_pair_halves() { return 6 * 8 + (RU_PRE_SLOTS + 2 * RU_H1_SLOTS + 2 * RP_X_SLOTS) * RU_SLOT; }
 
 template <int ACT_A>
-__global__ __launch_bounds__(512, 2) void res_pair_rows_k(const ConvP P1A, const ConvP P1B, const ConvP P2A, const ConvP P2B, const int n_img) {
+__global__ __launch_bounds__(512, 2) void res_pair_rows_k(const ConvP P1A, const ConvP P1B, const ConvP P2A, const ConvP P2B, const int n_img, const int compact) {
     extern __shared__ __attribute__((aligned(16))) _Float16 lds[];
     const int tid = threadIdx.x, lane = tid & 63;
     const int wave = __builtin_amdgcn_readfirstlane(tid >> 6);
@@ -1668,7 +1670,10 @@
 #pragma unroll
             for (int q = 0; q < 4; ++q) { o[q] = accC[cr][0][q]; o[4 + q] = accC[cr][1][q]; }
             const h8 rv = *reinterpret_cast<const h8 *>(resr + ((s + 1) & (RU_PRE_SLOTS - 1)) * RU_SLOT + offC);
-            conv_epilogue_f16x8<ACT_NONE, false, 1, true, false>(P2B, EB, ((n0 + kk * nstep) * H + y) * W + fr, fq * 8, o, &rv);
+            if (!compact) { conv_epilogue_f16x8<ACT_NONE, false, 1, true, false>(P2B, EB, ((n0 + kk * nstep) * H + y) * W + fr, fq * 8, o, &rv); continue; }
+            h8 *raw = ((y | fr) & 1) ? nullptr
+                    : reinterpret_cast<h8 *>(static_cast<_Float16 *>(P2B.out) + (size_t)(n0 + kk * nstep) * MARS_SKIP32_HALVES + (((y >> 1) * 4 + fq) * 8 + (fr >> 1)) * 8);
+            conv_epilogue_f16x8<ACT_NONE, false, 1, true, false, true>(P2B, EB, ((n0 + kk * nstep) * H + y) * W + fr, fq * 8, o, &rv, raw);
         }
     };
     for (int g = 0; g < Gall; ++g) {
@@ -3560,7 +3565,8 @@
            A2.H == A1.H && A2.W == A1.W && A1.act == ACT_ELU && A2.act == ACT_ELU;
 }
 
-int launch_res_pair(hipStream_t s, const ConvP &A1, const ConvP &B1, const ConvP &A2, const ConvP &B2, int nimg, int device) {
+int launch_res_pair(hipStream_t s, const ConvP &A1, const ConvP &B1, const ConvP &A2, const ConvP &B2, int nimg, int device, bool compact) {
+    DD_REQUIRE(!compact || (!B2.coff_out && B2.cs_out == 32), DD_E_ARG, "res_pair_rows: a compact skip tensor takes a whole 32-channel buffer");
     constexpr size_t lds_bytes = (size_t)4 * rp_pair_halves() * sizeof(_Float16);
     static DevOnce once;
     const int rc = once.run(device, [&]() -> int {
@@ -3569,7 +3575,7 @@
     });
     if (rc != DD_OK) return rc;
     const int grid = std::min(dd_ceil_div(nimg, 4), 256);
-    hipLaunchKernelGGL((res_pair_rows_k<ACT_ELU>), dim3((unsigned)grid), dim3(512), lds_bytes, s, A1, B1, A2, B2, nimg);
+    hipLaunchKernelGGL((res_pair_rows_k<ACT_ELU>), dim3((unsigned)grid), dim3(512), lds_bytes, s, A1, B1, A2, B2, nimg, compact ? 1 : 0);
     DD_LAUNCH_CHECK();
     return DD_OK;
 }
@@ -3957,6 +3963,22 @@
     return nb - i + 1;
 }
 
+bool mars_compact_on() {
+    static const bool on = !(getenv("DD_MARS_COMPACT_SKIP") && atoi(getenv("DD_MARS_COMPACT_SKIP")) == 0);
+    return on;
+}
+bool sole_reader(const dd_net *net, int t, int reader) {
+    if (t < 0 || t == net->out_tensor || net->tensors[t].coff) return false;
+    for (size_t k = 0; k < net->tensors.size(); ++k)
+        if ((int)k != t && net->tensors[k].buf == net->tensors[t].buf) return false;
+    for (int k = 0; k < net->n_ops; ++k) {
+        const int32_t *o = net->prog.data() + net->ops_off + (size_t)k * OP_WORDS;
+        if (o[0] >= 16) return false;
+        if ((o[1] == t || o[3] == t) && k != reader) return false;
+    }
+    return true;
+}
+
 MarsWsP mars_ws_params(const ConvP &P, int nimg) {
     MarsWsP Q;
     memset(&Q, 0, sizeof(Q));
@@ -4201,6 +4223,9 @@
                    "dd_net_read: tensor %d was not written by the last forward (op %d ran inside the next op's launch at this batch "
                    "size and its output stayed on chip); run a smaller batch or a program compiled without the fusion flags", t, i);
     }
+    DD_REQUIRE(t != n->compact_raw[0] && t != n->compact_raw[1], DD_E_STATE,
+               "dd_net_read: tensor %d was not materialised by the last forward (only its even pixels were written, for the stride-2 projection "
+               "that alone reads it); dd_net_keep_tensors before the forward, or DD_MARS_COMPACT_SKIP=0", t);
     hipStream_t s = dd_pick_stream(n->ctx, stream);
     const size_t bytes = d.pad ? (size_t)n_img * (d.h + 2) * (d.w + 2) * d.cs
                                : (size_t)n_img * d.h * d.w * d.cs * dtype_size(d.dtype);
@@ -4211,6 +4236,20 @@
 }
 
 static int net_run_ops(dd_net *net, const uint8_t *input, int nimg, hipStream_t s);
+
+int dd_net_keep_tensors(dd_net *net, int enable) {
+    DD_REQUIRE(net, DD_E_ARG, "dd_net_keep_tensors: NULL net");
+    DD_DEVICE(net->ctx);
+    if (net->keep_tensors != (enable != 0)) net_drop_graphs(net);
+    net->keep_tensors = enable != 0;
+    return DD_OK;
+}
+
+int dd_net_compact_skips(dd_net *net, int32_t *tensors_host) {
+    DD_REQUIRE(net && tensors_host, DD_E_ARG, "dd_net_compact_skips: NULL argument");
+    tensors_host[0] = net->compact_raw[0]; tensors_host[1] = net->compact_raw[1];
+    return DD_OK;
+}
 
 int dd_net_use_graph(dd_net *net, int enable) {
     DD_REQUIRE(net, DD_E_ARG, "dd_net_use_graph: NULL net");
@@ -4369,7 +4408,7 @@
     if (!net->use_graph || net->profile) return eager();
     if (net->graphs.size() > 256) net_drop_graphs(net);
     dd_net::GraphEntry &g = net->graphs[std::make_pair(static_cast<const void *>(input), nimg)];
-    if (g.exec) { DD_HIP(hipGraphLaunch(g.exec, s)); return DD_OK; }
+    if (g.exec) { DD_HIP(hipGraphLaunch(g.exec, s)); net->compact_raw[0] = g.compact_raw[0]; net->compact_raw[1] = g.compact_raw[1]; return DD_OK; }
     if (g.calls++ == 0) return eager();
     DD_HIP(hipStreamBeginCapture(s, hipStreamCaptureModeThreadLocal));
     const int rc = net_run_ops(net, input, nimg, s);
@@ -4378,6 +4417,7 @@
     if (rc != DD_OK) { if (graph) (void)hipGraphDestroy(graph); return rc; }
     DD_HIP(e);
     g.graph = graph;
+    g.compact_raw[0] = net->compact_raw[0]; g.compact_raw[1] = net->compact_raw[1];
     DD_HIP(hipGraphInstantiate(&g.exec, graph, nullptr, nullptr, 0));
     DD_HIP(hipGraphLaunch(g.exec, s));
     return DD_OK;
@@ -4411,6 +4451,50 @@
         net->op_launch[pair_op] = OPK_RES_UNIT;
         return launch_res_unit(s, pair_a, pair_b, nimg, net->ctx->device);
     };
+    const bool compact_ok = mars_compact_on() && !net->keep_tensors;
+    net->compact_raw[0] = net->compact_raw[1] = -1;
+    int compact_reader[2] = {-1, -1};
+    bool compact_taken[2] = {false, false};
+    auto opw_at = [&](int k) { return net->prog.data() + net->ops_off + (size_t)k * OP_WORDS; };
+    auto conv_params = [&](int k, ConvP &P) {
+        const int32_t *o = opw_at(k);
+        const float *of = reinterpret_cast<const float *>(o);
+        const TensorDesc &ts = net->tensors[o[1]], &td = net->tensors[o[2]];
+        memset(&P, 0, sizeof(P));
+        P.in = reinterpret_cast<const _Float16 *>(base(o[1])); P.H = ts.h; P.W = ts.w; P.cs_in = ts.cs;
+        P.coff_in = ts.coff; P.cin = o[10];
+        P.kh = o[5]; P.kw = o[6]; P.stride = o[7]; P.pad_t = o[8]; P.pad_l = o[9];
+        P.cout = o[11]; P.cout_pad = o[12]; P.kpad = o[13]; P.act = o[14]; P.epi = o[15];
+        P.w = reinterpret_cast<const _Float16 *>(net->d_weights + (size_t)(uint32_t)o[16]);
+        P.bias = reinterpret_cast<const float *>(net->d_weights + (size_t)(uint32_t)o[17]);
+        P.ho = o[26]; P.wo = o[27]; P.m = nimg * P.ho * P.wo;
+        P.out = base(o[2]); P.cs_out = td.cs; P.coff_out = td.coff;
+        if (o[3] >= 0) {
+            const TensorDesc &tr = net->tensors[o[3]];
+            P.res = reinterpret_cast<const _Float16 *>(base(o[3])); P.cs_res = tr.cs; P.coff_res = tr.coff;
+        }
+        if (o[4] >= 0) {
+            const TensorDesc &t2 = net->tensors[o[4]];
+            P.out2 = reinterpret_cast<_Float16 *>(base(o[4])); P.cs_out2 = t2.cs; P.coff_out2 = t2.coff;
+            P.aff2 = reinterpret_cast<const float *>(net->d_weights + (size_t)(uint32_t)o[18]);
+        }
+        if (o[4] < 0 && o[19]) {
+            P.aff2 = reinterpret_cast<const float *>(net->d_weights + (size_t)(uint32_t)o[18]);
+            P.post_aff = 1;
+        }
+        for (int q = 0; q < 6; ++q) P.p[q] = o[20 + q];
+        for (int q = 0; q < 8; ++q) P.f[q] = of[32 + q];
+    };
+    auto s2_proj_at = [&](int k) {
+        if (k + 1 >= net->n_ops) return false;
+        const int32_t *o = opw_at(k);
+        if (o[0] != OP_CONV || o[30] != 3 || o[1] < 0 || o[2] < 0) return false;
+        MarsPairP q64; bool f64;
+        if (mars_pair_match(net, k, nimg, q64, f64)) return false;
+        ConvP P;
+        conv_params(k, P);
+        return mars_ws_s2_eligible(P) && mars_proj_follows(net, k, P);
+    };
     auto run_ws = [&](ConvP &P) { return P.cin == 256 ? launch_conv_ws<4>(s, P, net->ctx->device) : launch_conv_ws<8>(s, P, net->ctx->device); };
     int first_op = 0;
     bool mid_on = false;
@@ -4453,10 +4537,15 @@
         if (net->profile) DD_HIP(hipEventRecord(net->events[i], s));
         const int32_t *o = net->prog.data() + net->ops_off + (size_t)i * OP_WORDS;
         const float *of = reinterpret_cast<const float *>(o);
-        const int kind = o[0], src = o[1], dst = o[2], res = o[3], dst2 = o[4];
+        const int kind = o[0], src = o[1], dst = o[2], res = o[3];
         const TensorDesc *ts = src >= 0 ? &net->tensors[src] : nullptr;
         const TensorDesc *td = dst >= 0 ? &net->tensors[dst] : nullptr;
         DD_REQUIRE(!input_pending || (kind == OP_CONV && i == input_op + 1), DD_E_STATE, "dd_net_forward: input op %d was folded into an op that did not take it", input_op);
+        for (int c = 0; c < 2; ++c) {
+            const int t = net->compact_raw[c];
+            DD_REQUIRE(t < 0 || kind >= 16 || (src != t && res != t) || (i == compact_reader[c] && compact_taken[c]), DD_E_STATE,
+                       "dd_net_forward: op %d reads tensor %d, which was written as a compact skip tensor for op %d", i, t, compact_reader[c]);
+        }
         if (mid_on && kind == 19 && i + 1 < net->n_ops && net->prog[net->ops_off + (size_t)(i + 1) * OP_WORDS] == 19) {
             const int32_t *o4 = net->prog.data() + net->ops_off + (size_t)(i + 1) * OP_WORDS;
             if (net->profile) DD_HIP(hipEventRecord(net->events[i + 1], s));
@@ -4521,34 +4610,21 @@
                 }
                 if (o[30] == 3 || o[30] == 4) {
                     const int n_ops = mars_pair_match(net, i, nimg, pair64, pair64_first);
-                    if (n_ops) { DD_NO_PENDING(); pair_left = n_ops - 1; net->op_launch[i] = OPK_FOLDED; break; }
+                    if (n_ops) {
+                        DD_NO_PENDING();
+                        const int last = i + n_ops - 1, t_out = opw_at(last)[2];
+                        if (pair64_first) {
+                            if (net->compact_raw[0] >= 0 && opw_at(i + 1)[1] == net->compact_raw[0]) { pair64.in2_compact = 1; compact_taken[0] = true; }
+                        } else if (compact_ok && s2_proj_at(last + 1) && opw_at(last + 2)[1] == t_out && sole_reader(net, t_out, last + 2) &&
+                                   net->tensors[t_out].cs == 64) {
+                            pair64.out_compact = 1; net->compact_raw[1] = t_out; compact_reader[1] = last + 2;
+                        }
+                        pair_left = n_ops - 1; net->op_launch[i] = OPK_FOLDED; break;
+                    }
                 }
 #undef DD_NO_PENDING
                 ConvP P;
-                memset(&P, 0, sizeof(P));
-                P.in = reinterpret_cast<const _Float16 *>(base(src)); P.H = ts->h; P.W = ts->w; P.cs_in = ts->cs;
-                P.coff_in = ts->coff; P.cin = o[10];
-                P.kh = o[5]; P.kw = o[6]; P.stride = o[7]; P.pad_t = o[8]; P.pad_l = o[9];
-                P.cout = o[11]; P.cout_pad = o[12]; P.kpad = o[13]; P.act = o[14]; P.epi = o[15];
-                P.w = reinterpret_cast<const _Float16 *>(net->d_weights + (size_t)(uint32_t)o[16]);
-                P.bias = reinterpret_cast<const float *>(net->d_weights + (size_t)(uint32_t)o[17]);
-                P.ho = o[26]; P.wo = o[27]; P.m = nimg * P.ho * P.wo;
-                P.out = base(dst); P.cs_out = td->cs; P.coff_out = td->coff;
-                if (res >= 0) {
-                    const TensorDesc &tr = net->tensors[res];
-                    P.res = reinterpret_cast<const _Float16 *>(base(res)); P.cs_res = tr.cs; P.coff_res = tr.coff;
-                }
-                if (dst2 >= 0) {
-                    const TensorDesc &t2 = net->tensors[dst2];
-                    P.out2 = reinterpret_cast<_Float16 *>(base(dst2)); P.cs_out2 = t2.cs; P.coff_out2 = t2.coff;
-                    P.aff2 = reinterpret_cast<const float *>(net->d_weights + (size_t)(uint32_t)o[18]);
-                }
-                if (dst2 < 0 && o[19]) {
-                    P.aff2 = reinterpret_cast<const float *>(net->d_weights + (size_t)(uint32_t)o[18]);
-                    P.post_aff = 1;
-                }
-                for (int q = 0; q < 6; ++q) P.p[q] = o[20 + q];
-                for (int q = 0; q < 8; ++q) P.f[q] = of[32 + q];
+                conv_params(i, P);
                 int rc;
                 DD_REQUIRE(!o[29] || (net->use_rw && P.kh == 3 && P.stride == 1 && P.cin == 32 && P.cout_pad == 32), DD_E_ARG,
                            "dd_net_forward: fused pooling is only built for the 3x3 32->32 kernel");
@@ -4559,7 +4635,13 @@
                         if (pair_pending) {
                             if (res_pair_fusable(pair_a, pair_b, unit_a, P, nimg)) {
                                 pair_pending = false;
-                                rc = launch_res_pair(s, pair_a, pair_b, unit_a, P, nimg, net->ctx->device);
+                                bool compact = false;
+                                if (compact_ok && i + 3 < net->n_ops && P.cs_out == 32 && !P.coff_out) {
+                                    MarsPairP qn; bool first_n = false;
+                                    compact = mars_pair_match(net, i + 1, nimg, qn, first_n) == 3 && first_n && opw_at(i + 2)[1] == dst && sole_reader(net, dst, i + 2);
+                                }
+                                if (compact) { net->compact_raw[0] = dst; compact_reader[0] = i + 2; }
+                                rc = launch_res_pair(s, pair_a, pair_b, unit_a, P, nimg, net->ctx->device, compact);
                                 if (rc != DD_OK) return rc;
                                 net->op_launch[i] = OPK_RES_PAIR;
                                 break;
@@ -4658,6 +4740,7 @@
                     Q.w2 = reinterpret_cast<const _Float16 *>(net->d_weights + (size_t)(uint32_t)q[16]); Q.kpad2 = q[13];
                     Q.bias2 = reinterpret_cast<const float *>(net->d_weights + (size_t)(uint32_t)q[17]);
                     Q.out2 = reinterpret_cast<_Float16 *>(base(q[2])); Q.cs_out2 = qd.cs; Q.coff_out2 = qd.coff;
+                    if (net->compact_raw[1] >= 0 && q[1] == net->compact_raw[1]) { Q.in2_compact = 1; compact_taken[1] = true; }
                     net->op_launch[i] = OPK_MARS_WS;
                     rc = mars_ws128_launch(s, net->ctx->device, Q, MARS_WS_S2_PROJ, P.act, false);
                     proj_done = true;
diff --git a/deepdish_amd/engine.py b/deepdish_amd/engine.py
--- a/deepdish_amd/engine.py
+++ b/deepdish_amd/engine.py
@@ -39,6 +39,9 @@
 
     def use_graph(self, enable=True):
         check(lib().dd_net_use_graph(self._h, int(bool(enable))), 'dd_net_use_graph')
+
+    def keep_tensors(self, enable=True):
+        check(lib().dd_net_keep_tensors(self._h, int(bool(enable))), 'dd_net_keep_tensors')
 
     def ssd_decode(self, anchors, score_thr, enable=True):
         if not enable:
diff --git a/deepdish_amd/profile.py b/deepdish_amd/profile.py
--- a/deepdish_amd/profile.py
+++ b/deepdish_amd/profile.py
@@ -34,6 +34,12 @@
     cnt = ctypes.c_int(0)
     check(lib().dd_net_op_launches(net._h, ptr(codes), n, ctypes.byref(cnt)), 'dd_net_op_launches')
     return codes
+
+
+def net_compact_skips(net):
+    t = np.full(2, -1, dtype=np.int32)
+    check(lib().dd_net_compact_skips(net._h, ptr(t)), 'dd_net_compact_skips')
+    return [int(v) for v in t]
 
 
 def launches_of(net, ms, batch):
diff --git a/include/deepdish_hip.h b/include/deepdish_hip.h
--- a/include/deepdish_hip.h
+++ b/include/deepdish_hip.h
@@ -134,6 +134,8 @@
 int dd_net_profile(dd_net *net, int enable);
 int dd_net_profile_read(dd_net *net, float *ms_host, int cap, int *n_ops_host);
 int dd_net_op_launches(dd_net *net, int32_t *codes_host, int cap, int *n_ops_host);
+int dd_net_keep_tensors(dd_net *net, int enable);
+int dd_net_compact_skips(dd_net *net, int32_t *tensors_host);
 
 int dd_ssd_postprocess(dd_ctx *ctx, const float *raw, const float *anchors, int n_anchors,
                        int n_classes, int max_det, float score_thr, float iou_thr,
```

Measured after the change: 145,500 frames/s (median of 6 runs). 1.2% higher.
